# paTRICK-swk/D3DP

Hardware: AMD Instinct MI355X
Metric: pose-hypotheses/sec (H x clips) at F=243, J=17, H=20, K=10 (higher is better)
Workload: dtype f16x2-split operands on fp16 MFMA, f32 accumulate (fp32-class: meets 1e-3 mm)

## Files before the change

d3dp_amd/csrc/capi_train.hip:

```cpp
#include <optional>

#include "ctx.h"

namespace {

#define TP(cls, call) { Scope ps_(pc, cls, st); LAUNCH_TRY(call); }

const float* mask_ptr(const float* masks, const d3dp_cfg& g, int B, int blk, int branch) {
  if (!masks) return nullptr;
  const size_t smax = (size_t)B * std::max(g.frames, g.joints);
  return masks + ((size_t)blk * 2 + branch) * smax;
}

struct Reducer {
  float* base;
  size_t cap, used = 0;
  hipStream_t st;
  std::vector<D3dpReduceItem> items{};
  int rc = 0;
  float* take(size_t n) {
    n = (n + 63) / 64 * 64;
    if (used + n > cap) { rc = -1; return nullptr; }
    float* p = base + used;
    used += n;
    return p;
  }
  void add(const float* part, float* dst, size_t n, size_t count, size_t stride, bool accumulate = false) {
    if (!part || !dst || rc) { rc = rc ? rc : -1; return; }
    items.push_back(D3dpReduceItem{part, dst, (unsigned)n, (unsigned)count, (unsigned)stride, accumulate ? 1u : 0u});
  }
  void flush() {
    for (size_t i = 0; i < items.size() && rc == 0; i += D3DP_REDUCE_MAX) {
      D3dpReduceTable tb{};
      tb.count = (int)std::min<size_t>(D3DP_REDUCE_MAX, items.size() - i);
      for (int j = 0; j < tb.count; ++j) tb.it[j] = items[i + j];
      rc = d3dp_train_reduce_many(tb, st);
    }
    items.clear();
  }
};

int lin32(const float* A, const float* W, const float* bias, float* out, int M, int N, int K, hipStream_t st) {
  return d3dp_launch_linear_f32(EPI_BIAS, A, W, bias, out, M, N, K, st);
}

const float* lin_w(const BlockDev& w, int j) { return (const float*)(j == kQkv ? w.qkv_w : j == kProj ? w.proj_w : j == kFc1 ? w.fc1_w : w.fc2_w); }
const float* lin_b(const BlockDev& w, int j) { return j == kQkv ? w.qkv_b : j == kProj ? w.proj_b : j == kFc1 ? w.fc1_b : w.fc2_b; }

struct X2Train {
  hipStream_t st;
  float* ws;
  const TrainLayout& L;
  const TrainPlan& P;
  d3dp_ctx* pc;
  hipStream_t st_w = nullptr;
  X2Train(d3dp_ctx* c, const TrainLayout& L_, const TrainPlan& P_, float* ws_, hipStream_t st_)
      : st(st_), ws(ws_), L(L_), P(P_), pc(c->prof ? c : nullptr) {
    use_set(0);
  }
  size_t o_a = 0, o_at = 0, o_part = 0, set_base = 0, set_used = 0;
  void use_set(int s) {
    set_base = o_a = s ? L.op_a2 : L.op_a; set_used = 0; n_def = 0;
    o_at = s ? L.op_at2 : L.op_at; o_part = s ? L.part2 : L.part;
  }
  int n_def = 0;
  D3dpTnProduct def[D3DP_TN_MAX];
  float* def_dw[D3DP_TN_MAX];
  int flush_wgrads() {
    if (!n_def) return 0;
    hipStream_t sw = st_w ? st_w : st;
    Scope ps(pc, T_WGRAD, sw);
    int r = d3dp_launch_linear_f16x2_tn_many(def, n_def, P.mTp, P.mZ, sw, P.passes, P.rows_hi);
    if (r) return r;
    D3dpSumTable tb{};
    tb.n = n_def; tb.Z = P.mZ;
    for (int i = 0; i < n_def; ++i) { tb.part[i] = def[i].out; tb.out[i] = def_dw[i]; tb.n4[i] = (size_t)def[i].N * def[i].K / 4; }
    d3dp_launch_sum_partials_many(tb, sw);
    n_def = 0;
    return 0;
  }
  static constexpr int kBwdSlot0 = kTrainBwdSlot0;
  static constexpr int kQkvSlot0 = kTrainQkvSlot0;
  static constexpr int kPmaxSlot0 = kTrainPmaxSlot0;
  int next = 0;
  unsigned* amax() const { return reinterpret_cast<unsigned*>(ws + L.slots); }
  float* uns() const { return ws + L.slots + kTrainSlots; }
  unsigned* qkv_amax(int blk) const { return P.path.attn_x2(blk & 1) ? amax() + kQkvSlot0 + blk : nullptr; }
  int begin(bool forward_pass) {
    next = forward_pass ? 0 : kBwdSlot0;
    return hipMemsetAsync(ws + L.slots + next, 0, (size_t)kBwdSlot0 * 4, st) == hipSuccess ? 0 : -3;
  }
  int take() { return (next < kBwdSlot0 || next >= kTrainSlots) ? -1 : next++; }
  int slot_for(const float* src, size_t n) {
    if (next < kBwdSlot0 || next >= kTrainSlots) return -1;
    d3dp_launch_absmax(src, n, amax() + next, st);
    return next++;
  }
  void rows(const float* src, int R, int C, void* dst, int slot) {
    d3dp_launch_split2_dyn(src, dst, R, C, C, amax() + slot, uns() + slot, st);
  }
  void cols(const float* src, int R, int C, int Rpad, void* dst, int slot) {
    d3dp_launch_split2_t_dyn(src, dst, R, C, Rpad, amax() + slot, uns() + slot, st);
  }
  size_t xoff(int l) const { return (size_t)(l >> 2) * L.x_block + (size_t)(l & 3) * L.C * L.Tp_max; }
  size_t woff(int l) const {
    const size_t CC = L.C * L.C, j = (size_t)(l & 3);
    return (size_t)(l >> 2) * L.w_block + (j == 0 ? 0 : j == 1 ? 3 * CC : j == 2 ? 4 * CC : 4 * CC + L.Hd * L.C);
  }
  float* x_op(int l) const { return ws + L.x_cols + xoff(l); }
  int prepare_weights(const d3dp_ctx* c) {
    if (!P.batched) return 0;
    const int nl = 8 * c->cfg.depth;
    D3dpWPrepTable tb{};
    tb.n = nl;
    for (int l = 0; l < nl; ++l) {
      const int blk = l >> 2, j = l & 3;
      const BlockDev& w = (blk & 1) ? c->tte[blk >> 1] : c->ste[blk >> 1];
      tb.it[l] = D3dpWPrepItem{lin_w(w, j), P.lin[j].N, P.lin[j].K, 2 * l + 1, 0, woff(l)};
    }
    return d3dp_launch_wprep(tb, ws + L.w_rows, ws + L.w_cols, amax(), uns(), st, P.rows_hi);
  }
  int gemm(TrainTail tail, const float* A2, const float* W2, const float* bias, const float* ua, const float* uw, float* out, int N,
           int K, unsigned* out_amax = nullptr, int amax_pos = 0) {
    Scope ps(pc, T_LINEAR, st);
    const int T = P.T, passes = P.passes;
    if (tail.form != TrainTailForm::SPLIT_REM)
      return d3dp_launch_linear_f16x2_dyn(A2, W2, bias, ua, uw, out, T, N, K, 1, st, out_amax, amax_pos,
                                          tail.form == TrainTailForm::REM_BLOCKS ? 1 : 0, passes, P.rows_hi);
    if (P.rows_hi) return -1;
    const int q = T / 256, rem = T - q * 256;
    int r = d3dp_launch_linear_f16x2_dyn(A2, W2, bias, ua, uw, out, q * 256, N, K, 1, st, out_amax, amax_pos, 0, passes);
    if (r) return r;
    r = d3dp_launch_linear_f16x2_dyn(A2 + (size_t)q * 256 * K, W2, nullptr, ua, uw, ws + L.part_rem, rem, N, K, tail.Z, st, nullptr, 0, 0, passes);
    if (r) return r;
    d3dp_launch_sum_partials_bias(ws + L.part_rem, bias, out + (size_t)q * 256 * N, (size_t)rem * N, N, tail.Z, st, out_amax, amax_pos);
    return 0;
  }
  int forward(int blk, TrainLinearId j, const float* A, const BlockDev& w, float ln_eps, float* out) {
    const TrainLinear& p = P.lin[j];
    const int l = 4 * blk + j, sa = 2 * l, sw = 2 * l + 1, T = P.T, N = p.N, K = p.K;
    if (sw >= kBwdSlot0) return -1;
    const float* W = lin_w(w, j);
    const bool pmax = j == kFc1 && P.gelu_operand;
    unsigned* out_amax = j == kQkv ? qkv_amax(blk) : pmax ? amax() + kPmaxSlot0 + blk : nullptr;
    const TrainOperand src = P.source(blk, j);
    const float* a2 = x_op(l);
    if (P.rows_hi && (src == TrainOperand::ROWS_T || !P.batched)) return -1;
    if (src != TrainOperand::PRODUCER) {
      Scope ps(pc, T_OPERAND, st);
      if (j == kProj && (blk & 1) && P.attn_t_f32_mfma) d3dp_launch_absmax(A, (size_t)T * K, amax() + sa, st);
      const int Tp = p.pad_rows;
      int r;
      if (src == TrainOperand::LN_INPUT)
        r = d3dp_launch_rowprep_ln(A, j == kQkv ? w.n1w : w.n2w, j == kQkv ? w.n1b : w.n2b, ln_eps, x_op(l), T, Tp, K, amax() + sa, uns() + sa, st, P.rows_hi);
      else if (src == TrainOperand::ROWS)
        r = d3dp_launch_rowprep(A, x_op(l), nullptr, nullptr, T, Tp, K, amax() + sa, uns() + sa, st, nullptr, 0, 1, 1, nullptr, P.rows_hi);
      else {
        a2 = ws + o_a;
        r = d3dp_launch_dyprep(A, ws + o_a, x_op(l), nullptr, T, K, Tp, amax() + sa, uns() + sa, st);
      }
      if (r) return r;
    }
    const float* w2 = ws + L.op_w;
    if (P.batched) w2 = ws + L.w_rows + woff(l);
    else {
      Scope ps(pc, T_OPERAND, st);
      d3dp_launch_absmax(W, (size_t)N * K, amax() + sw, st);
      rows(W, N, K, ws + L.op_w, sw);
    }
    return gemm(p.fwd_tail, a2, w2, lin_b(w, j), uns() + sa, uns() + sw, out, N, K, out_amax, pmax ? 1 : 0);
  }
  int gelu_operand(int blk, const float* hpre) {
    const int l = 4 * blk + kFc2;
    Scope ps(pc, T_OPERAND, st);
    return d3dp_launch_gelu_rowprep(hpre, x_op(l), P.T, P.lin[kFc2].pad_rows, P.lin[kFc2].K, amax() + kPmaxSlot0 + blk, amax() + 2 * l, uns() + 2 * l, st, P.rows_hi);
  }
  int dgrad(int blk, TrainLinearId j, int sdy, const float* W, float* dX, unsigned* out_amax = nullptr) {
    const TrainLinear& p = P.lin[j];
    const int l = 4 * blk + j, sw = 2 * l + 1;
    {
      Scope ps(pc, T_OPERAND, st);
      if (!P.batched) cols(W, p.N, p.K, p.N, ws + L.op_w, sw);
    }
    const float* wt = ws + L.op_w;
    if (P.batched) wt = ws + L.w_cols + woff(l);
    return gemm(p.dgrad_tail, ws + o_a, wt, nullptr, uns() + sdy, uns() + sw, dX, p.K, p.N, out_amax);
  }
  int prep_dy(TrainLinearId j, const float* dY, int sdy, float* bias_part, int* bias_rows, const float* mask = nullptr, int axis = 0,
              int F = 1, int J = 1, const float* gelu_pre = nullptr) {
    const TrainLinear& p = P.lin[j];
    if (P.merged) {
      if (set_used + L.Tp_max * (size_t)p.N > L.dy_set_floats) return -1;
      o_a = set_base + set_used;
      set_used += L.Tp_max * (size_t)p.N;
    }
    Scope ps(pc, T_OPERAND, st);
    if (p.tn)
      return d3dp_launch_rowprep(dY, ws + o_a, bias_part, bias_rows, P.T, p.pad_rows, p.N, amax() + sdy, uns() + sdy, st, mask, axis, F, J,
                                 gelu_pre, P.rows_hi);
    if (P.rows_hi) return -1;
    *bias_rows = D3DP_DYPREP_ROWS;
    return d3dp_launch_dyprep(dY, ws + o_a, ws + o_at, bias_part, P.T, p.N, p.pad_rows, amax() + sdy, uns() + sdy, st);
  }
  int wgrad(int blk, TrainLinearId j, int sdy, float* dW) {
    const TrainLinear& p = P.lin[j];
    const int l = 4 * blk + j, sx = 2 * l, N = p.N, K = p.K;
    if (P.merged) {
      if (n_def >= D3DP_TN_MAX) return -1;
      size_t po = 0;
      for (int i = 0; i < n_def; ++i) po += (size_t)P.mZ * def[i].N * def[i].K;
      def[n_def] = D3dpTnProduct{ws + o_a, x_op(l), uns() + sdy, uns() + sx, ws + o_part + po, N, K, 0, 0};
      def_dw[n_def++] = dW;
      return 0;
    }
    int r;
    hipStream_t sw = st_w ? st_w : st;
    Scope ps(pc, T_WGRAD, sw);
    if (p.tn)
      r = d3dp_launch_linear_f16x2_tn(ws + o_a, x_op(l), uns() + sdy, uns() + sx, ws + o_part, N, K, p.Tp, p.Z, sw, P.passes, P.rows_hi);
    else
      r = d3dp_launch_linear_f16x2_dyn(ws + o_at, x_op(l), nullptr, uns() + sdy, uns() + sx, ws + o_part, N, K, p.Tp, p.Z, sw, nullptr, 0, 0, P.passes);
    if (r) return r;
    d3dp_launch_sum_partials(ws + o_part, dW, (size_t)N * K, p.Z, sw);
    return 0;
  }
};

}

extern "C" {

int d3dp_train_workspace_bytes(const d3dp_ctx* c, int32_t B, size_t* bytes) {
  if (!c || !bytes || B < 1) return d3dp_fail(D3DP_EINVAL, "d3dp_train_workspace_bytes: bad argument");
  *bytes = train_layout(c->cfg, B).total_floats * 4;
  return D3DP_OK;
}

int d3dp_train_forward(d3dp_ctx* c, const float* x2d, const float* x3d, const int64_t* t, const float* masks, float* out,
                       int32_t B, void* workspace, size_t workspace_bytes, void* stream) {
  if (!c || !x2d || !x3d || !t || !out || !workspace || B < 1) return d3dp_fail(D3DP_EINVAL, "d3dp_train_forward: bad argument");
  if (!c->train()) return d3dp_fail(D3DP_ESTATE, "d3dp_train_forward needs a D3DP_MODE_TRAIN context");
  if (!c->weights_set) return d3dp_fail(D3DP_ESTATE, "weights not set");
  const d3dp_cfg& g = c->cfg;
  const TrainLayout L = train_layout(g, B);
  const TrainPlan P = plan_train_step(*c, g, B, c->n_cu);
  if (g.frames > 256 && !(P.path.attn_x2(0) && P.path.attn_x2(1)) && !P.attn_bwd_chunked)
    return d3dp_fail(D3DP_ENOTSUP, "frames=%d > 256: the training step runs such clips on its split-fp16 attention kernels only, which take "
                              "head dims 64, 32 and 16 -- 24, 40, 48 and 56 under D3DP_TRAIN_IMPL=f16x2 -- (channels=%d heads=%d is head dim %d) and are switched off by the cross-check "
                              "switches D3DP_TRAIN_IMPL=f32 and D3DP_TRAIN_ATTN=f32|x2t; the fp32 attention holds a whole sequence "
                              "in LDS (<= 256 frames)", g.frames, g.channels, g.heads, g.channels / g.heads);
  if (workspace_bytes < L.total_floats * 4) return d3dp_fail(D3DP_ESTATE, "train workspace too small");
  if (P.use_x2 && !P.rows_fit) return d3dp_fail(D3DP_EINVAL, "d3dp_train_forward: an operand's padded rows exceed the workspace's");
  hipStream_t st = (hipStream_t)stream;
  float* ws = (float*)workspace;
  const int T = P.T, C = g.channels, F = g.frames, J = g.joints, Hd = g.hidden;
  float *xn = ws + L.xn, *y = ws + L.y, *hid = ws + L.hid;
  d3dp_ctx* const pc = c->prof ? c : nullptr;
  std::optional<X2Train> x2s;
  if (P.use_x2) x2s.emplace(c, L, P, ws, st);
  X2Train* const x2 = P.use_x2 ? &*x2s : nullptr;
  if (x2) {
    Scope ps_(pc, T_OTHER, st);
    LAUNCH_TRY(x2->begin(true));
    LAUNCH_TRY(x2->prepare_weights(c));
  }
  auto lin = [&](int blk, TrainLinearId j, const float* src, float* out) -> int {
    const BlockDev& w = (blk & 1) ? c->tte[blk >> 1] : c->ste[blk >> 1];
    if (x2) return x2->forward(blk, j, src, w, g.eps_block, out);
    Scope ps_(pc, T_LINEAR, st);
    return lin32(src, lin_w(w, j), lin_b(w, j), out, T, P.lin[j].N, P.lin[j].K, st);
  };
  const bool ln_fused = P.ln_fused, ln_direct = P.ln_direct;
  TP(T_OTHER, d3dp_train_time_mlp(t, c->freq, c->t1w, c->t1b, c->t3w, c->t3b, ws + L.dtemb, ws + L.temb, B, C, st));
  float* slab0 = ws + L.saved0;
  TP(T_LN_FWD, d3dp_launch_embed_ln(0, x2d, x3d, ws + L.temb, c->ew, c->eb, c->spos, c->ste[0].n1w, c->ste[0].n1b,
                                    g.eps_block, slab0 + L.o_xin, xn, 0, B, 1, F, J, C, st));
  auto slot = [&](int l) -> unsigned* { return x2 ? x2->amax() + 2 * l : nullptr; };
  if (x2) { Scope ps_(pc, T_OTHER, st); d3dp_launch_absmax(xn, (size_t)T * C, slot(0), st); }
  for (int blk = 0; blk < 2 * g.depth; ++blk) {
    const int kind = blk & 1, d = blk >> 1;
    const BlockDev& w = kind ? c->tte[d] : c->ste[d];
    float* S = ws + L.saved0 + (size_t)blk * L.saved_stride;
    const bool ax2 = P.path.attn_x2(kind);
    LAUNCH_TRY(lin(blk, kQkv, ln_fused ? S + L.o_xin : xn, S + L.o_qkv));
    const bool att_direct = P.att_direct(kind);
    void* att_op = att_direct ? x2->x_op(4 * blk + 1) : nullptr;
    const int att_tp = att_direct ? P.lin[kProj].pad_rows : 0;
    float* att_un = att_direct ? x2->uns() + 2 * (4 * blk + 1) : nullptr;
    const int n_seq = kind ? B * J : B * F;
    const SeqMap map = kind ? temporal_map(F, J) : spatial_map(F, J);
    auto attention = [&]() -> int {
      if (ax2)
        return d3dp_train_attn_x2_fwd(S + L.o_qkv, S + L.o_att, ws + L.stats_x2 + (size_t)blk * L.stats_x2_stride, n_seq, map, C,
                                      g.heads, x2->qkv_amax(blk), slot(4 * blk + 1), st, att_op, T, att_tp, att_un, P.attn_passes, P.rows_hi);
      if (kind == 1 && P.attn_t_f32_mfma)
        return d3dp_launch_attn_temporal_f32(0, S + L.o_qkv, S + L.o_att, n_seq, map, C, g.heads, st);
      return d3dp_launch_attn_rows(0, S + L.o_qkv, S + L.o_att, n_seq, map, C, g.heads, st, slot(4 * blk + 1));
    };
    TP(kind ? T_ATTN_FWD_T : T_ATTN_FWD_S, attention());
    LAUNCH_TRY(lin(blk, kProj, S + L.o_att, y));
    if (ln_direct)
      TP(T_LN_FWD, d3dp_train_add_mask_ln(S + L.o_xin, y, mask_ptr(masks, g, B, blk, 0), kind, F, J, w.n2w, w.n2b, g.eps_block,
                                          S + L.o_xmid, nullptr, slot(4 * blk + 2), T, C, st, x2->x_op(4 * blk + 2),
                                          P.lin[kFc1].pad_rows, x2->uns() + 2 * (4 * blk + 2), P.rows_hi))
    else
      TP(T_LN_FWD, d3dp_train_add_mask_ln(S + L.o_xin, y, mask_ptr(masks, g, B, blk, 0), kind, F, J, w.n2w, w.n2b, g.eps_block,
                                          S + L.o_xmid, ln_fused ? nullptr : xn, slot(4 * blk + 2), T, C, st));
    LAUNCH_TRY(lin(blk, kFc1, ln_fused ? S + L.o_xmid : xn, S + L.o_hpre));
    if (P.gelu_operand) {
      LAUNCH_TRY(x2->gelu_operand(blk, S + L.o_hpre));
      LAUNCH_TRY(lin(blk, kFc2, nullptr, y));
    } else {
      TP(T_OPERAND, d3dp_train_gelu_fwd(S + L.o_hpre, hid, (size_t)T * Hd, slot(4 * blk + 3), st));
      LAUNCH_TRY(lin(blk, kFc2, hid, y));
    }
    const bool last = blk == 2 * g.depth - 1;
    float* x_next = last ? ws + L.x_final : S + L.saved_stride + L.o_xin;
    const float *nw = c->hnw, *nb = c->hnb;
    if (!last) { const BlockDev& wn = kind ? c->ste[d + 1] : c->tte[d]; nw = wn.n1w; nb = wn.n1b; }
    TP(T_LN_FWD, d3dp_train_add_mask_ln2(S + L.o_xmid, y, mask_ptr(masks, g, B, blk, 1), kind, F, J, kind ? c->tnw : c->snw,
                                         kind ? c->tnb : c->snb, g.eps_block, (kind == 0 && d == 0) ? c->tpos : nullptr, nw, nb,
                                         last ? g.eps_head : g.eps_block, S + L.o_xout, x_next,
                                         last ? ws + L.z : (ln_fused ? nullptr : xn), last ? nullptr : slot(4 * (blk + 1)), T, C, st,
                                         (ln_direct && !last) ? x2->x_op(4 * (blk + 1)) : nullptr,
                                         (ln_direct && !last) ? P.lin[kQkv].pad_rows : 0,
                                         (ln_direct && !last) ? x2->uns() + 2 * 4 * (blk + 1) : nullptr, P.rows_hi));
  }
  TP(T_OTHER, d3dp_train_head_linear(ws + L.z, c->hw, c->hb, out, T, C, st));
  HIP_TRY(hipGetLastError());
  return D3DP_OK;
}

int d3dp_train_backward(d3dp_ctx* c, const float* x2d, const float* x3d, const int64_t* t, const float* masks,
                        const float* grad_out, const d3dp_weights* grads, int32_t B, void* workspace,
                        size_t workspace_bytes, void* stream) {
  if (!c || !x2d || !x3d || !t || !grad_out || !grads || !grads->ste || !grads->tte || !workspace || B < 1)
    return d3dp_fail(D3DP_EINVAL, "d3dp_train_backward: bad argument");
  if (!c->train()) return d3dp_fail(D3DP_ESTATE, "d3dp_train_backward needs a D3DP_MODE_TRAIN context");
  const d3dp_cfg& g = c->cfg;
  const TrainLayout L = train_layout(g, B);
  const TrainPlan P = plan_train_step(*c, g, B, c->n_cu);
  if (workspace_bytes < L.total_floats * 4) return d3dp_fail(D3DP_ESTATE, "train workspace too small");
  if (P.use_x2 && !(P.rows_fit && P.parts_fit))
    return d3dp_fail(D3DP_EINVAL, "d3dp_train_backward: an operand's padded rows or a weight gradient's partial products exceed the workspace's");
  hipStream_t st = (hipStream_t)stream;
  float* ws = (float*)workspace;
  const int T = P.T, Tp = (int)L.Tpad, C = g.channels, F = g.frames, J = g.joints, Hd = g.hidden;
  auto G = [](const float* p) { return const_cast<float*>(p); };
  D3dpZeroTable ztab{};
  auto zero = [&](const float* p, size_t n) -> hipError_t {
    if (ztab.count < D3DP_ZERO_MAX && n < ((size_t)1 << 32)) {
      ztab.p[ztab.count] = G(p); ztab.n[ztab.count] = (unsigned)n; ++ztab.count;
      return hipSuccess;
    }
    return hipMemsetAsync(G(p), 0, n * 4, st);
  };
  const size_t CC = (size_t)C * C;
  HIP_TRY(zero(grads->time1_w, 2 * CC)); HIP_TRY(zero(grads->time1_b, 2 * C));
  HIP_TRY(zero(grads->time3_w, 2 * CC)); HIP_TRY(zero(grads->time3_b, C));
  d3dp_ctx* const pc = c->prof ? c : nullptr;
  if (ztab.count) TP(T_OTHER, d3dp_train_zero_many(ztab, st));
  float *xn = ws + L.xn, *hid = ws + L.hid, *dA = ws + L.dA, *dB = ws + L.dB, *dC = ws + L.dC, *dqkv = ws + L.dqkv,
        *dh = ws + L.dh, *At = ws + L.At, *Xt = ws + L.Xt, *Wt = ws + L.Wt;

  std::optional<X2Train> x2s;
  if (P.use_x2) x2s.emplace(c, L, P, ws, st);
  X2Train* const x2 = P.use_x2 ? &*x2s : nullptr;
  if (x2) TP(T_OTHER, x2->begin(false));
  const bool overlap = P.path.needs_aux && !c->prof;
  if (overlap && !c->aux) return d3dp_fail(D3DP_ESTATE, "d3dp_train_backward: the second stream was not created (d3dp_create makes it)");
  bool pending[2] = {false, false};
  int n_wgrad = 0, cur_set = 0;
  const int n_sets = P.overlap_sets;
  auto wait_set = [&](int s) -> int {
    if (!pending[s]) return 0;
    pending[s] = false;
    return hipStreamWaitEvent(st, c->ev_done[s], 0) == hipSuccess ? 0 : -3;
  };
  auto join = [&]() -> int { int r = wait_set(0); return r ? r : wait_set(1); };
  Reducer red{ws + L.red, L.red_floats, 0, st};
  red.items.reserve(24 * (size_t)g.depth + 32);
  const int lnrows = L.ln_rows;
  auto ln_part = [&](const float* dgamma, const float* dbeta, int calls) -> float* {
    float* p = red.take((size_t)calls * lnrows * 2 * C);
    if (p) {
      red.add(p, G(dgamma), C, (size_t)calls * lnrows, 2 * (size_t)C);
      red.add(p + C, G(dbeta), C, (size_t)calls * lnrows, 2 * (size_t)C);
    }
    return p;
  };
  float* part_sn = ln_part(grads->spatial_norm_w, grads->spatial_norm_b, g.depth);
  float* part_tn = ln_part(grads->temporal_norm_w, grads->temporal_norm_b, g.depth);
  float* part_hn = ln_part(grads->head_norm_w, grads->head_norm_b, 1);
  if (red.rc) return d3dp_fail(D3DP_ESTATE, "d3dp_train_backward: partial-sum region too small");
  int sdy = -1;
  auto wgrad = [&](int blk, TrainLinearId j, const float* dY, const float* X, float* dW, float* dbias, int pre_slot = -1,
                   const float* mk = nullptr, int mk_axis = 0, const float* gelu_pre = nullptr) -> int {
    const int N = P.lin[j].N, K = P.lin[j].K;
    int r;
    if (x2) {
      sdy = pre_slot >= 0 ? pre_slot : x2->slot_for(dY, (size_t)T * N);
      if (sdy < 0) return -1;
      float* bp = red.take((size_t)L.bias_rows * N);
      int brows = 0;
      if (!bp) return -1;
      const bool first = !P.merged || j == kFc2, last = !P.merged || j == kQkv;
      if (first) {
        cur_set = overlap ? (n_wgrad++ % n_sets) : 0;
        if ((r = wait_set(cur_set))) return r;
        x2->use_set(cur_set);
      }
      if ((r = x2->prep_dy(j, dY, sdy, bp, &brows, mk, mk_axis, F, J, gelu_pre))) return r;
      red.add(bp, dbias, N, brows, N);
      if (last && overlap) {
        if (hipEventRecord(c->ev_fork, st) != hipSuccess || hipStreamWaitEvent(c->aux, c->ev_fork, 0) != hipSuccess) return -3;
        x2->st_w = c->aux;
      }
      if ((r = x2->wgrad(blk, j, sdy, dW))) return r;
      if (last && P.merged && (r = x2->flush_wgrads())) return r;
      if (last && overlap) {
        if (hipEventRecord(c->ev_done[cur_set], c->aux) != hipSuccess) return -3;
        pending[cur_set] = true;
      }
      return 0;
    }
    float* bp = red.take((size_t)D3DP_DYPREP_ROWS * N);
    int rows = 0;
    if (!bp || mk || gelu_pre) return -1;
    {
      Scope ps_(pc, T_OPERAND, st);
      if ((r = d3dp_train_colsum(dY, bp, &rows, D3DP_DYPREP_ROWS, T, N, st))) return r;
      red.add(bp, dbias, N, rows, N);
      if ((r = d3dp_train_transpose_pad(dY, At, T, N, Tp, st))) return r;
      if ((r = d3dp_train_transpose_pad(X, Xt, T, K, Tp, st))) return r;
    }
    Scope ps_(pc, T_WGRAD, st);
    return d3dp_launch_linear_f32_splitk(At, Xt, dW, N, K, Tp, st, ws + L.part, L.part_floats);
  };
  auto dgrad = [&](int blk, TrainLinearId j, const float* dY, float* dX, unsigned* out_amax = nullptr) -> int {
    const BlockDev& w = (blk & 1) ? c->tte[blk >> 1] : c->ste[blk >> 1];
    const int N = P.lin[j].N, K = P.lin[j].K;
    if (x2) return sdy < 0 ? -1 : x2->dgrad(blk, j, sdy, lin_w(w, j), dX, out_amax);
    int r;
    { Scope ps_(pc, T_OPERAND, st); if ((r = d3dp_train_transpose_pad(lin_w(w, j), Wt, N, K, N, st))) return r; }
    Scope ps_(pc, T_LINEAR, st);
    return lin32(dY, Wt, nullptr, dX, T, K, N, st);
  };
  auto fresh = [&](int& slot) -> unsigned* {
    slot = x2 ? x2->take() : -1;
    return slot >= 0 ? x2->amax() + slot : nullptr;
  };
#define D3DP_FRESH(ps, pa)                                                                              \
  int ps = -1;                                                                                          \
  unsigned* pa = fresh(ps);                                                                             \
  if (x2 && ps < 0) return d3dp_fail(D3DP_ESTATE, "d3dp_train_backward: out of operand slots");

  const int nblk = 2 * g.depth;
  {
    float* hp = red.take((size_t)L.head_rows * (3 * C + 4));
    int rows = 0;
    if (!hp) return d3dp_fail(D3DP_ESTATE, "d3dp_train_backward: partial-sum region too small");
    TP(T_OTHER, d3dp_train_head_bwd(grad_out, ws + L.z, c->hw, dC, hp, &rows, T, C, st));
    red.add(hp, G(grads->head_w), 3 * (size_t)C, rows, 3 * (size_t)C + 4);
    red.add(hp + 3 * C, G(grads->head_b), 3, rows, 3 * (size_t)C + 4);
  }
  const float* dy = nullptr;
  const float* dy_mask = nullptr;
  int ps_next = -1;
  const bool mip2 = P.mip2, mip1 = P.mip1, gip = P.gip;
  {
    const int lb = nblk - 1, lk = lb & 1;
    const float* S = ws + L.saved0 + (size_t)lb * L.saved_stride;
    const float* mk = mask_ptr(masks, g, B, lb, 1);
    D3DP_FRESH(ps, pa)
    TP(T_LN_BWD, d3dp_train_ln_bwd(dC, ws + L.x_final, c->hnw, g.eps_head, nullptr, nullptr, S + L.o_xout, lk ? c->tnw : c->snw,
                                 g.eps_block, dB, mk, lk, F, J, (mk && !mip2) ? dC : nullptr, pa, part_hn,
                                 (lk ? part_tn : part_sn) + (size_t)(lb >> 1) * lnrows * 2 * C, T, C, st));
    dy = (mk && !mip2) ? dC : dB;
    dy_mask = mip2 ? mk : nullptr;
    ps_next = ps;
  }
  for (int blk = nblk - 1; blk >= 0; --blk) {
    const int kind = blk & 1, d = blk >> 1;
    const BlockDev& w = kind ? c->tte[d] : c->ste[d];
    const d3dp_block_weights& gw = (kind ? grads->tte : grads->ste)[d];
    float* S = ws + L.saved0 + (size_t)blk * L.saved_stride;
    if (!x2) TP(T_OPERAND, d3dp_train_gelu_fwd(S + L.o_hpre, hid, (size_t)T * Hd, nullptr, st));
    LAUNCH_TRY(wgrad(blk, kFc2, dy, hid, G(gw.fc2_w), G(gw.fc2_b), ps_next, dy_mask, kind));
    {
      D3DP_FRESH(ps, pa)
      LAUNCH_TRY(dgrad(blk, kFc2, dy, dh, gip ? pa : nullptr));
      if (!gip) TP(T_OPERAND, d3dp_train_gelu_bwd(dh, S + L.o_hpre, dh, (size_t)T * Hd, pa, st));
      if (!x2) TP(T_LN_FWD, d3dp_train_ln_pos(S + L.o_xmid, w.n2w, w.n2b, g.eps_block, nullptr, F, J, xn, T, C, st));
      LAUNCH_TRY(wgrad(blk, kFc1, dh, xn, G(gw.fc1_w), G(gw.fc1_b), ps, nullptr, 0, gip ? S + L.o_hpre : nullptr));
      LAUNCH_TRY(dgrad(blk, kFc1, dh, dC));
    }
    {
      const float* mk = mask_ptr(masks, g, B, blk, 0);
      float* pn = ln_part(gw.norm2_w, gw.norm2_b, 1);
      D3DP_FRESH(ps, pa)
      if (!pn) return d3dp_fail(D3DP_ESTATE, "d3dp_train_backward: partial-sum region too small");
      TP(T_LN_BWD, d3dp_train_ln_bwd(dC, S + L.o_xmid, w.n2w, g.eps_block, dB, nullptr, nullptr, nullptr, 0.f, dA, mk, kind, F, J,
                                   (mk && !mip1) ? dC : nullptr, pa, pn, nullptr, T, C, st));
      dy = (mk && !mip1) ? dC : dA;
      LAUNCH_TRY(wgrad(blk, kProj, dy, S + L.o_att, G(gw.proj_w), G(gw.proj_b), ps, mip1 ? mk : nullptr, kind));
    }
    int ps_dqkv = -1;
    if (P.path.attn_x2(kind)) {
      D3DP_FRESH(pdo, pado)
      D3DP_FRESH(pq, paq)
      LAUNCH_TRY(dgrad(blk, kProj, dy, dB, pado));
      for (int part = pc ? 1 : 0; part <= (pc ? 2 : 0); ++part)
        TP(part == 2 ? (kind ? T_ATTN_BKV_T : T_ATTN_BKV_S) : (kind ? T_ATTN_BQ_T : T_ATTN_BQ_S),
           d3dp_train_attn_x2_bwd(S + L.o_qkv, S + L.o_att, dB, dqkv, ws + L.stats_x2 + (size_t)blk * L.stats_x2_stride,
                                  kind ? B * J : B * F, kind ? temporal_map(F, J) : spatial_map(F, J), C, g.heads,
                                  x2->qkv_amax(blk), pado, paq, st, part, P.attn_passes));
      ps_dqkv = pq;
    } else {
      LAUNCH_TRY(dgrad(blk, kProj, dy, dB));
      TP(kind ? T_ATTN_BQ_T : T_ATTN_BQ_S, d3dp_train_attn_bwd(S + L.o_qkv, S + L.o_att, dB, dqkv, ws + L.stats, kind ? B * J : B * F,
                                                             kind ? temporal_map(F, J) : spatial_map(F, J), C, g.heads, st,
                                                             P.attn_bwd_chunked));
    }
    if (!x2) TP(T_LN_FWD, d3dp_train_ln_pos(S + L.o_xin, w.n1w, w.n1b, g.eps_block, nullptr, F, J, xn, T, C, st));
    LAUNCH_TRY(wgrad(blk, kQkv, dqkv, xn, G(gw.qkv_w), G(gw.qkv_b), ps_dqkv));
    LAUNCH_TRY(dgrad(blk, kQkv, dqkv, dC));
    float* pn1 = ln_part(gw.norm1_w, gw.norm1_b, 1);
    if (!pn1) return d3dp_fail(D3DP_ESTATE, "d3dp_train_backward: partial-sum region too small");
    if (blk > 0) {
      const int pb = blk - 1, pk = pb & 1;
      const float* Sp = ws + L.saved0 + (size_t)pb * L.saved_stride;
      const float* mk = mask_ptr(masks, g, B, pb, 1);
      float* g_out = pb == 0 ? ws + L.y : nullptr;
      D3DP_FRESH(ps, pa)
      TP(T_LN_BWD, d3dp_train_ln_bwd(dC, S + L.o_xin, w.n1w, g.eps_block, dA, g_out, Sp + L.o_xout, pk ? c->tnw : c->snw, g.eps_block,
                                   dB, mk, pk, F, J, (mk && !mip2) ? dC : nullptr, pa, pn1,
                                   (pk ? part_tn : part_sn) + (size_t)(pb >> 1) * lnrows * 2 * C, T, C, st));
      if (g_out) TP(T_OTHER, d3dp_train_groupsum(g_out, G(grads->temporal_pos), T, C, 1, F, J, 1, st));
      dy = (mk && !mip2) ? dC : dB;
      dy_mask = mip2 ? mk : nullptr;
      ps_next = ps;
    } else {
      TP(T_LN_BWD, d3dp_train_ln_bwd(dC, S + L.o_xin, w.n1w, g.eps_block, dA, nullptr, nullptr, nullptr, 0.f, dB, nullptr, 0, F, J,
                                   nullptr, nullptr, pn1, nullptr, T, C, st));
    }
  }
#undef D3DP_FRESH
  LAUNCH_TRY(join());
  {
    Scope ps_(pc, T_OTHER, st);
    float* ep = red.take((size_t)D3DP_EMBED_BWD_ROWS * 5 * C);
    float* bp = red.take((size_t)L.embed_bias_rows * C);
    float* sp = red.take((size_t)L.group_slices * J * C);
    float* tp = red.take((size_t)L.group_slices * B * C);
    int rows = 0;
    if (!ep || !bp || !sp || !tp) return d3dp_fail(D3DP_ESTATE, "d3dp_train_backward: partial-sum region too small");
    LAUNCH_TRY(d3dp_train_embed_bwd(dB, x2d, x3d, ep, T, C, st));
    red.add(ep, G(grads->embed_w), 5 * (size_t)C, D3DP_EMBED_BWD_ROWS, 5 * (size_t)C);
    LAUNCH_TRY(d3dp_train_colsum(dB, bp, &rows, L.embed_bias_rows, T, C, st));
    red.add(bp, G(grads->embed_b), C, rows, C);
    LAUNCH_TRY(d3dp_train_groupsum(dB, sp, T, C, 0, F, J, L.group_slices, st));
    red.add(sp, G(grads->spatial_pos), (size_t)J * C, L.group_slices, (size_t)J * C);
    LAUNCH_TRY(d3dp_train_groupsum(dB, tp, T, C, 2, F, J, L.group_slices, st));
    red.add(tp, ws + L.dtemb, (size_t)B * C, L.group_slices, (size_t)B * C);
    red.flush();
  }
  if (red.rc) return d3dp_fail(D3DP_EHIP, "d3dp_train_backward: the gradient reduction failed");
  TP(T_OTHER, d3dp_train_time_mlp_bwd(t, c->freq, c->t1w, c->t1b, c->t3w, ws + L.dtemb, G(grads->time1_w),
                                      G(grads->time1_b), G(grads->time3_w), G(grads->time3_b), B, C, st));
  for (int i = 0; pc && i < 8; ++i) { Scope ps_(pc, P_EMPTY, st); }
  HIP_TRY(hipGetLastError());
  return D3DP_OK;
}

}
#undef TP
```

d3dp_amd/csrc/ctx_plan.h:

```cpp
#pragma once
#include <algorithm>
#include <cstdlib>
#include <cstring>

#include "../../include/d3dp_hip.h"

int d3dp_fail(int code, const char* fmt, ...) __attribute__((format(printf, 2, 3)));

struct CtxEnv {
  const char *exact_impl = nullptr, *long_attn = nullptr, *no_fold = nullptr, *defer_norm = nullptr, *train_impl = nullptr,
             *train_overlap = nullptr, *train_gelu = nullptr, *train_wgrad = nullptr, *train_ln_operand = nullptr, *train_tail = nullptr,
             *train_attn = nullptr, *train_passes = nullptr, *fast_impl = nullptr, *fast16_range = nullptr, *x2_skew = nullptr,
             *x2_pp = nullptr, *x2_wide = nullptr, *seq_pad = nullptr, *fold_ln = nullptr, *train_long_attn = nullptr,
             *train_attn_passes = nullptr, *train_rows = nullptr;
  static CtxEnv from_process() {
    CtxEnv e;
    e.exact_impl = getenv("D3DP_EXACT_IMPL");
    e.long_attn = getenv("D3DP_LONG_ATTN");
    e.no_fold = getenv("D3DP_NO_FOLD");
    e.defer_norm = getenv("D3DP_DEFER_NORM");
    e.train_impl = getenv("D3DP_TRAIN_IMPL");
    e.train_overlap = getenv("D3DP_TRAIN_OVERLAP");
    e.train_gelu = getenv("D3DP_TRAIN_GELU");
    e.train_wgrad = getenv("D3DP_TRAIN_WGRAD");
    e.train_ln_operand = getenv("D3DP_TRAIN_LN_OPERAND");
    e.train_tail = getenv("D3DP_TRAIN_TAIL");
    e.train_attn = getenv("D3DP_TRAIN_ATTN");
    e.train_passes = getenv("D3DP_TRAIN_PASSES");
    e.fast_impl = getenv("D3DP_FAST_IMPL");
    e.fast16_range = getenv("D3DP_FAST16_RANGE");
    e.x2_skew = getenv("D3DP_X2_SKEW");
    e.x2_pp = getenv("D3DP_X2_PP");
    e.x2_wide = getenv("D3DP_X2_WIDE");
    e.seq_pad = getenv("D3DP_SEQ_PAD");
    e.fold_ln = getenv("D3DP_FOLD_LN");
    e.train_long_attn = getenv("D3DP_TRAIN_LONG_ATTN");
    e.train_attn_passes = getenv("D3DP_TRAIN_ATTN_PASSES");
    e.train_rows = getenv("D3DP_TRAIN_ROWS");
    return e;
  }
};

struct CtxPlan {
  int hdp = 0;
  bool fast16_scale = false;
  int train_passes = 3;
  int train_attn_passes = 3;
  bool train_rows_hi = false;
  int exact_impl_req = 0;
  bool long_rows = false;
  bool fold = true;
  bool defer = true;
  bool train_x2 = true;
  bool train_overlap = true;
  int train_overlap_sets = 2;
  bool train_gelu_in_prep = true;
  bool train_wgrad_merged = true;
  bool train_ln_direct = true;
  bool train_tail_blocks = true;
  int train_attn_x2 = 2;
  bool train_long_attn = false;
  int skew_d = 0;
  int pingpong = 0;
  int pad_override = -1;
  bool fold_ln_on = false;
};

inline bool env_is(const char* v, const char* s) { return v && !strcmp(v, s); }
inline int env_digit(const char* v, const char* allowed, int dflt) {
  return v && v[0] && !v[1] && strchr(allowed, v[0]) ? v[0] - '0' : dflt;
}
inline bool mfma_head_dim(int hd) { return hd == 64 || hd == 32 || hd == 16; }

inline bool instantiated_width(const d3dp_cfg& g) {
  const int hd = g.channels / g.heads;
  return (g.channels == 64 || g.channels == 128 || g.channels == 256 || g.channels == 512) &&
         (hd == 8 || hd == 16 || hd == 32 || hd == 64) && g.hidden >= 64 && g.hidden % 64 == 0;
}
inline bool optin_width(int c) { return c == 192 || c == 320 || c == 384 || c == 448; }
inline int padded_head_dim(int hd) { return hd <= 32 ? 32 : 64; }
inline bool x2_optin_shape(const d3dp_cfg& g) {
  const int hd = g.channels / g.heads;
  return optin_width(g.channels) && hd % 8 == 0 && hd <= 64 && g.hidden >= 64 && g.hidden % 64 == 0;
}
inline bool fast_optin_shape(const d3dp_cfg& g) {
  const int hd = g.channels / g.heads;
  return optin_width(g.channels) && (hd == 24 || hd == 32 || hd == 40 || hd == 48 || hd == 56 || hd == 64) && g.hidden == 2 * g.channels;
}
constexpr int D3DP_TN_TILE_N = 256, D3DP_TN_TILE_K = 128;
constexpr int D3DP_WPREP_MAX = 64;
inline bool d3dp_tn_applies(int N, int K) { return N % D3DP_TN_TILE_N == 0 && K % D3DP_TN_TILE_K == 0; }
inline bool train_linears_split(const CtxPlan& p, const d3dp_cfg& g) { return p.train_x2 && g.channels % 32 == 0 && g.hidden % 32 == 0; }

inline int plan_context(const d3dp_cfg& g, const CtxEnv& e, bool variants_built, CtxPlan* out) {
  if (g.frames < 1 || g.frames > 1024) return d3dp_fail(D3DP_ENOTSUP, "frames=%d not in [1,1024]", g.frames);
  if (g.joints < 1 || g.joints > 256) return d3dp_fail(D3DP_ENOTSUP, "joints=%d not in [1,256]", g.joints);
  if (g.heads < 1 || g.channels < 1 || g.channels % g.heads) return d3dp_fail(D3DP_EINVAL, "heads=%d does not divide channels=%d", g.heads, g.channels);
  if (g.depth < 1) return d3dp_fail(D3DP_EINVAL, "depth=%d", g.depth);
  if (g.mode != D3DP_MODE_EXACT && g.mode != D3DP_MODE_FAST && g.mode != D3DP_MODE_TRAIN && g.mode != D3DP_MODE_FAST16)
    return d3dp_fail(D3DP_EINVAL, "mode=%d", g.mode);
  const int hd = g.channels / g.heads;
  const bool inst = instantiated_width(g), train = g.mode == D3DP_MODE_TRAIN, fast16 = g.mode == D3DP_MODE_FAST16;
  CtxPlan p;
  p.long_rows = env_is(e.long_attn, "rows");
  if (env_is(e.exact_impl, "f16x2") && !inst) {
    if (!x2_optin_shape(g) || g.mode != D3DP_MODE_EXACT)
      return d3dp_fail(D3DP_ENOTSUP, "D3DP_EXACT_IMPL=f16x2 outside the instantiated widths exists for D3DP_MODE_EXACT contexts with channels in "
                                "{192,320,384,448}, head dim a multiple of 8 up to 64 and hidden a multiple of 64; channels=%d heads=%d "
                                "hidden=%d mode=%d is not one (unset the switch: such a context runs the fp32 implementation)",
                  g.channels, g.heads, g.hidden, g.mode);
    if (p.long_rows)
      return d3dp_fail(D3DP_ENOTSUP, "D3DP_LONG_ATTN=rows with D3DP_EXACT_IMPL=f16x2 at channels=%d: the run-time-head-dim row attention has no "
                                "split-fp16 output form", g.channels);
    p.hdp = padded_head_dim(hd);
  }
  const bool train_widths = train && !inst && env_is(e.train_impl, "f16x2");
  if (train_widths && !x2_optin_shape(g))
    return d3dp_fail(D3DP_ENOTSUP, "D3DP_TRAIN_IMPL=f16x2 outside the instantiated widths exists for D3DP_MODE_TRAIN contexts with channels in "
                              "{192,320,384,448}, head dim a multiple of 8 up to 64 and hidden a multiple of 64; channels=%d heads=%d "
                              "hidden=%d is not one (unset the switch: such a context trains on the fp32 path)",
                g.channels, g.heads, g.hidden);
  if ((g.mode == D3DP_MODE_FAST || fast16) && e.fast_impl) {
    if (strcmp(e.fast_impl, "mfma"))
      return d3dp_fail(D3DP_ENOTSUP, "D3DP_FAST_IMPL=%.32s: the one value a FAST / FAST16 context takes is D3DP_FAST_IMPL=mfma (channels=%d)",
                  e.fast_impl, g.channels);
    if (!inst) {
      if (!fast_optin_shape(g))
        return d3dp_fail(D3DP_ENOTSUP, "D3DP_FAST_IMPL=mfma outside the instantiated widths exists for FAST / FAST16 contexts with channels in "
                                  "{192,320,384,448}, head dim in {24,32,40,48,56,64} and hidden = 2 x channels; channels=%d heads=%d "
                                  "hidden=%d is not one (such a width runs in D3DP_MODE_EXACT / D3DP_MODE_TRAIN)",
                    g.channels, g.heads, g.hidden);
      if (p.long_rows)
        return d3dp_fail(D3DP_ENOTSUP, "D3DP_LONG_ATTN=rows with D3DP_FAST_IMPL=mfma at channels=%d: the row attention kernel would take the padded "
                                  "head dim for its exponent", g.channels);
      p.hdp = padded_head_dim(hd);
    }
  }
  if (fast16 && e.fast16_range) {
    if (strcmp(e.fast16_range, "scale"))
      return d3dp_fail(D3DP_ENOTSUP, "D3DP_FAST16_RANGE=%.32s: the one value a FAST16 context takes is D3DP_FAST16_RANGE=scale", e.fast16_range);
    if (p.hdp)
      return d3dp_fail(D3DP_ENOTSUP, "D3DP_FAST16_RANGE=scale with D3DP_FAST_IMPL=mfma at channels=%d: the padded-head kernels have no scaled "
                                "form", g.channels);
    if (inst && !mfma_head_dim(hd))
      return d3dp_fail(D3DP_ENOTSUP, "D3DP_FAST16_RANGE=scale at head dim %d (channels=%d heads=%d): the scaled attention kernels exist at head "
                                "dims 64, 32 and 16", hd, g.channels, g.heads);
    if (inst && p.long_rows)
      return d3dp_fail(D3DP_ENOTSUP, "D3DP_FAST16_RANGE=scale with D3DP_LONG_ATTN=rows: the row attention kernel has no scaled form");
    const int k = g.hidden;
    if (inst && !(k == 64 || k == 128 || k == 256 || k == 512 || k == 1024))
      return d3dp_fail(D3DP_ENOTSUP, "D3DP_FAST16_RANGE=scale with hidden=%d: the scaled streaming Linear exists at k-depths 64, 128, 256, 512 "
                                "and 1024", g.hidden);
    p.fast16_scale = inst;
  }
  if (train && e.train_long_attn) {
    if (strcmp(e.train_long_attn, "chunked"))
      return d3dp_fail(D3DP_ENOTSUP, "D3DP_TRAIN_LONG_ATTN=%.32s: the one value a TRAIN context takes is D3DP_TRAIN_LONG_ATTN=chunked (the fp32 "
                                "attention backward passes its rows through LDS in chunks and takes any sequence length)", e.train_long_attn);
    p.train_long_attn = true;
  }
  const bool width_inst = inst || p.hdp != 0;
  if (!width_inst) {
    if (g.mode == D3DP_MODE_FAST)
      return d3dp_fail(D3DP_ENOTSUP, "channels=%d heads=%d hidden=%d: FAST contexts exist for channels in {64,128,256,512} with head dim in "
                                "{8,16,32,64} and hidden a multiple of 64; other widths run in D3DP_MODE_EXACT / D3DP_MODE_TRAIN (fp32 implementation)",
                  g.channels, g.heads, g.hidden);
    if (fast16)
      return d3dp_fail(D3DP_ENOTSUP, "channels=%d heads=%d hidden=%d: FAST16 contexts exist for the shapes FAST contexts exist for -- channels in "
                                "{64,128,256,512} with head dim in {8,16,32,64} and hidden a multiple of 64; other widths run in D3DP_MODE_EXACT / "
                                "D3DP_MODE_TRAIN (fp32 implementation)",
                  g.channels, g.heads, g.hidden);
    if (g.channels > 1024 || g.channels % 4 || hd % 4 || hd > 128 || g.hidden < 4 || g.hidden % 4)
      return d3dp_fail(D3DP_ENOTSUP, "channels=%d heads=%d hidden=%d: the fp32 implementation takes channels <= 1024, head dim a multiple of 4 up to 128 "
                                "and hidden a multiple of 4", g.channels, g.heads, g.hidden);
    const int nmax = std::max(g.frames, g.joints), cap = hd <= 16 ? 16 : hd <= 32 ? 32 : hd <= 64 ? 64 : 128;
    if (train && !train_widths && !p.train_long_attn && (nmax > 256 || (size_t)nmax * (8 * (cap + 4) + 12) > 160 * 1024))
      return d3dp_fail(D3DP_ENOTSUP, "channels=%d heads=%d frames=%d joints=%d: training at a width outside {64,128,256,512} runs the fp32 attention "
                                "backward, which holds a whole sequence in LDS (<= 256 tokens; <= 153 at head dims above 64)",
                  g.channels, g.heads, g.frames, g.joints);
  }
  const bool train_f32 = env_is(e.train_impl, "f32");
  p.fold = !(e.no_fold && e.no_fold[0] == '1');
  p.defer = !(e.defer_norm && e.defer_norm[0] == '0');
  p.train_x2 = !train_f32 && (width_inst || train_widths);
  p.train_overlap = !(e.train_overlap && e.train_overlap[0] == '0');
  p.train_overlap_sets = (e.train_overlap && e.train_overlap[0] == '1') ? 1 : 2;
  p.train_gelu_in_prep = !env_is(e.train_gelu, "pass");
  p.train_wgrad_merged = !env_is(e.train_wgrad, "each");
  p.train_ln_direct = !env_is(e.train_ln_operand, "pass");
  p.train_tail_blocks = !env_is(e.train_tail, "split");
  p.train_attn_x2 = env_is(e.train_attn, "f32") ? 0 : env_is(e.train_attn, "x2t") ? 1 : 2;
  const bool superseded = !p.train_gelu_in_prep || !p.train_wgrad_merged || !p.train_tail_blocks || !p.train_ln_direct;
  if (train && e.train_passes) {
    if (strcmp(e.train_passes, "1") && strcmp(e.train_passes, "3"))
      return d3dp_fail(D3DP_ENOTSUP, "D3DP_TRAIN_PASSES=%.32s: the values a TRAIN context takes are D3DP_TRAIN_PASSES=1 (one fp16-MFMA pass per "
                                "product of the split-fp16 training Linears) and 3 (the default)", e.train_passes);
    if (e.train_passes[0] == '1') {
      if (!train_linears_split(p, g))
        return d3dp_fail(D3DP_ENOTSUP, "D3DP_TRAIN_PASSES=1 exists for the split-fp16 training Linears; channels=%d%s trains on the fp32 path "
                                  "(fp32-MFMA Linears have no one-pass form)", g.channels, train_f32 ? " under D3DP_TRAIN_IMPL=f32" : "");
      if (superseded)
        return d3dp_fail(D3DP_ENOTSUP, "D3DP_TRAIN_PASSES=1 beside D3DP_TRAIN_WGRAD=each / D3DP_TRAIN_TAIL=split / D3DP_TRAIN_GELU=pass / "
                                  "D3DP_TRAIN_LN_OPERAND=pass: the superseded launch forms have no one-pass form");
      p.train_passes = 1;
    }
  }
  if (train && e.train_attn_passes) {
    if (strcmp(e.train_attn_passes, "1") && strcmp(e.train_attn_passes, "3"))
      return d3dp_fail(D3DP_ENOTSUP, "D3DP_TRAIN_ATTN_PASSES=%.32s: the values a TRAIN context takes are D3DP_TRAIN_ATTN_PASSES=1 (one fp16-MFMA "
                                "pass per product of the split-fp16 training attention) and 3 (the default)", e.train_attn_passes);
    if (e.train_attn_passes[0] == '1') {
      if (!train_linears_split(p, g))
        return d3dp_fail(D3DP_ENOTSUP, "D3DP_TRAIN_ATTN_PASSES=1 exists for the split-fp16 training attention; channels=%d%s trains on the fp32 "
                                  "path (its attention runs the fp32 kernels, which have no one-pass form)", g.channels,
                    train_f32 ? " under D3DP_TRAIN_IMPL=f32" : "");
      if (hd == 24 || hd == 40 || hd == 48 || hd == 56)
        return d3dp_fail(D3DP_ENOTSUP, "D3DP_TRAIN_ATTN_PASSES=1 at head dim %d (channels=%d heads=%d): the padded forms of the split-fp16 "
                                  "training attention have no one-pass form", hd, g.channels, g.heads);
      if (!mfma_head_dim(hd))
        return d3dp_fail(D3DP_ENOTSUP, "D3DP_TRAIN_ATTN_PASSES=1 at head dim %d (channels=%d heads=%d): the one-pass training attention exists at "
                                  "head dims 64, 32 and 16 (this head dim runs the fp32 attention kernels)", hd, g.channels, g.heads);
      if (p.train_attn_x2 == 0)
        return d3dp_fail(D3DP_ENOTSUP, "D3DP_TRAIN_ATTN_PASSES=1 beside D3DP_TRAIN_ATTN=f32: both axes then run the fp32 attention kernels, which "
                                  "have no one-pass form");
      p.train_attn_passes = 1;
    }
  }
  if (train && e.train_rows) {
    if (strcmp(e.train_rows, "hi") && strcmp(e.train_rows, "split"))
      return d3dp_fail(D3DP_ENOTSUP, "D3DP_TRAIN_ROWS=%.32s: the values a TRAIN context takes are D3DP_TRAIN_ROWS=hi (the one-pass training "
                                "Linears' operands as plain fp16 rows) and split (the default)", e.train_rows);
    if (e.train_rows[0] == 'h') {
      if (!train_linears_split(p, g))
        return d3dp_fail(D3DP_ENOTSUP, "D3DP_TRAIN_ROWS=hi exists for the split-fp16 training Linears; channels=%d%s trains on the fp32 path "
                                  "(fp32-MFMA Linears read no operand rows)", g.channels, train_f32 ? " under D3DP_TRAIN_IMPL=f32" : "");
      if (!inst)
        return d3dp_fail(D3DP_ENOTSUP, "D3DP_TRAIN_ROWS=hi at channels=%d under D3DP_TRAIN_IMPL=f16x2: the padded widths run an operand pass in "
                                  "front of every Linear and transposed weight-gradient operands, which have no hi-only form", g.channels);
      if (superseded)
        return d3dp_fail(D3DP_ENOTSUP, "D3DP_TRAIN_ROWS=hi beside D3DP_TRAIN_WGRAD=each / D3DP_TRAIN_TAIL=split / D3DP_TRAIN_GELU=pass / "
                                  "D3DP_TRAIN_LN_OPERAND=pass: the superseded launch forms have no hi-only form");
      if (p.train_passes != 1)
        return d3dp_fail(D3DP_ENOTSUP, "D3DP_TRAIN_ROWS=hi without D3DP_TRAIN_PASSES=1: the three-pass products read the lo halves that hi-only "
                                  "rows do not store");
      const int C = g.channels, Hd = g.hidden;
      if (C % 256 != 0 || !d3dp_tn_applies(3 * C, C) || !d3dp_tn_applies(C, C) || !d3dp_tn_applies(Hd, C) || !d3dp_tn_applies(C, Hd))
        return d3dp_fail(D3DP_ENOTSUP, "D3DP_TRAIN_ROWS=hi at channels=%d hidden=%d: the hi-only route exists where no operand of the step is "
                                  "transposed and the LayerNorm kernels write the qkv / fc1 operand rows -- channels a multiple of 256 "
                                  "and hidden a multiple of 256 (`-cs` 256 and 512); narrower widths use transposed operands", C, Hd);
      if (hd == 16 && p.train_attn_x2 != 0)
        return d3dp_fail(D3DP_ENOTSUP, "D3DP_TRAIN_ROWS=hi at head dim 16 (channels=%d heads=%d): the split-fp16 training attention writes "
                                  "hi-only proj operand rows at head dims 64 and 32", g.channels, g.heads);
      if (8 * g.depth > D3DP_WPREP_MAX)
        return d3dp_fail(D3DP_ENOTSUP, "D3DP_TRAIN_ROWS=hi at depth=%d: the hi-only weight operands are written by the batched weight preparation "
                                  "(depth <= %d); the per-weight preparation of deeper models has no hi-only form", g.depth, D3DP_WPREP_MAX / 8);
      p.train_rows_hi = true;
    }
  }
  p.exact_impl_req = env_is(e.exact_impl, "bf16x3") ? 1 : env_is(e.exact_impl, "f32") ? 2 : 0;
  if (!width_inst) {
    if (p.exact_impl_req == 1)
      return d3dp_fail(D3DP_ENOTSUP, "D3DP_EXACT_IMPL=bf16x3 exists for channels in {64,128,256,512}; channels=%d runs the fp32 implementation", g.channels);
    p.exact_impl_req = 2;
  }
  if (superseded && !variants_built)
    return d3dp_fail(D3DP_ENOTSUP, "D3DP_TRAIN_WGRAD=each / D3DP_TRAIN_TAIL=split / D3DP_TRAIN_GELU=pass / D3DP_TRAIN_LN_OPERAND=pass select superseded launch forms of the "
                              "training step that only the variants build honours (make -C d3dp_amd/csrc variants; "
                              "D3DP_LIB=d3dp_amd/lib/variants/libd3dp_variants.so)");
  p.skew_d = env_digit(e.x2_skew, "0124", 0);
  p.pingpong = env_is(e.x2_wide, "1") ? 2 : env_digit(e.x2_pp, "01", 0);
  p.pad_override = env_digit(e.seq_pad, "01", -1);
  p.fold_ln_on = e.fold_ln && e.fold_ln[0] == '1';
  if ((p.skew_d || p.pingpong || p.pad_override > 0 || p.fold_ln_on) && !variants_built)
    return d3dp_fail(D3DP_ENOTSUP, "D3DP_X2_SKEW / D3DP_X2_PP / D3DP_X2_WIDE / D3DP_SEQ_PAD / D3DP_FOLD_LN select experiment kernels that this "
                              "library was built without (make -C d3dp_amd/csrc variants; D3DP_LIB=d3dp_amd/lib/variants/libd3dp_variants.so)");
  *out = p;
  return D3DP_OK;
}
```

d3dp_amd/csrc/gemm_x2_train.hip:

```cpp
#include <cstdlib>
#include <cstring>

#include "common.h"
#include "gemm_x2_tile.h"
#include "kernels.h"

namespace {

template <int PASSES, bool HI = false>
__global__ __launch_bounds__(768) void gemm_f16x2_dyn_kernel(const f16* __restrict__ A2, const f16* __restrict__ W2,
                                                             const float* __restrict__ bias, const float* __restrict__ dynA,
                                                             const float* __restrict__ dynW, float* __restrict__ out, int M,
                                                             int N, int Kfull, int NKz, int tiles_n, int tiles_per_z,
                                                             int total_items, unsigned* __restrict__ amax_out, int amax_pos,
                                                             int rem_m0) {
  static_assert(PASSES == 1 || PASSES == 3, "one pass (hi x hi) or the three-pass split scheme");
  static_assert(!HI || PASSES == 1, "hi-only rows hold no lo halves");
  constexpr int RS = HI ? 1 : 2;
  extern __shared__ __attribute__((aligned(16))) char smem[];
  const int G = gridDim.x;
  const int L = xcd_remap(blockIdx.x, G);
  const int n_my = (total_items - L + G - 1) / G;
  const int NS = HI ? NKz >> 1 : NKz;
  const int gtot = n_my * NS;
  const int tid = threadIdx.x, lane = tid & 63;
  const int wave = __builtin_amdgcn_readfirstlane(tid >> 6);
  if (gtot <= 0) return;
  const int rem_cg = (N + 63) >> 6;
  const int rem_blocks = rem_m0 > 0 ? ((M - rem_m0 + 15) >> 4) * rem_cg : 0;

  if (wave >= XNCW) {
    const int lw = wave - XNCW;
    const int lr = lane >> 3, lq = lane & 7;
    int ti = 0, ks = 0, slot = 0;
    const f16* pa[8];
    const f16* pw[4];
    auto issue = [&]() {
      if (ks == 0) {
        const int item = L + ti * G;
        const int z = item / tiles_per_z, t = item - z * tiles_per_z;
        const int m0 = (t / tiles_n) * XBM, n0 = (t % tiles_n) * XBN;
        const size_t k0 = (size_t)z * NS * (2 * XBK);
#pragma unroll
        for (int i = 0; i < 8; ++i) {
          const int row = (lw * 8 + i) * 8 + lr;
          pa[i] = A2 + (size_t)min(m0 + row, M - 1) * (RS * Kfull) + k0 + swz128(row, lq) * 8;
        }
#pragma unroll
        for (int i = 0; i < 4; ++i) {
          const int row = (lw * 4 + i) * 8 + lr;
          const int wrow = (row & 64) + colperm(row & 63);
          pw[i] = W2 + (size_t)min(n0 + wrow, N - 1) * (RS * Kfull) + k0 + swz128(row, lq) * 8;
        }
      }
      char* base = smem + slot * XSTAGE;
      const int ko = ks * (2 * XBK);
#pragma unroll
      for (int i = 0; i < 8; ++i) __builtin_amdgcn_global_load_lds(GPTR(pa[i] + ko), LPTR(base + (lw * 8 + i) * 1024), 16, 0, 0);
#pragma unroll
      for (int i = 0; i < 4; ++i)
        __builtin_amdgcn_global_load_lds(GPTR(pw[i] + ko), LPTR(base + XA_BYTES + (lw * 4 + i) * 1024), 16, 0, 0);
      if (++ks == NS) { ks = 0; ++ti; }
      slot = (slot == XNSTAGE - 1) ? 0 : slot + 1;
    };
    issue();
    if (gtot > 1) issue();
    for (int b = L; b < rem_blocks; b += G) { X2_BARRIER(); X2_BARRIER(); }
    for (int g = 0; g < gtot; ++g) {
      if (g + 1 < gtot) asm volatile("s_waitcnt vmcnt(12)" ::: "memory");
      else asm volatile("s_waitcnt vmcnt(0)" ::: "memory");
      X2_BARRIER();
      if (g + 2 < gtot) issue();
    }
    if (amax_out) X2_BARRIER();
    return;
  }

  const int wr = wave >> 1, wc = wave & 1;
  const int fi = lane & 15, fg = lane >> 4;
  const int offA = (wr * 64 + fi) * 128 + swz128(fi, fg) * 16, offAl = offA ^ 64;
  const int offW = XA_BYTES + (wc * 64 + fi) * 128 + swz128(fi, fg) * 16, offWl = offW ^ 64;
  const float unscale = dynA[0] * dynW[0];
  __builtin_amdgcn_s_setprio(1);
  float am = 0.f;
  int slot = 0;
  if (rem_blocks > 0) {
    const int ksw = NKz / XNCW;
    f32x4* xch = reinterpret_cast<f32x4*>(smem + (XNSTAGE - 1) * XSTAGE);
#pragma unroll 1
    for (int b = L; b < rem_blocks; b += G) {
      const int m0 = rem_m0 + (b / rem_cg) * 16, nb0 = (b % rem_cg) * 64;
      const size_t kofs = (size_t)wave * ksw * (RS * XBK) + fg * 8;
      const f16* ap = A2 + (size_t)min(m0 + fi, M - 1) * (RS * Kfull) + kofs;
      const f16* wp[4];
#pragma unroll
      for (int ni = 0; ni < 4; ++ni) wp[ni] = W2 + (size_t)min(nb0 + 4 * fi + ni, N - 1) * (RS * Kfull) + kofs;
      f32x4 pacc[4];
#pragma unroll
      for (int ni = 0; ni < 4; ++ni) pacc[ni] = (f32x4){0.f, 0.f, 0.f, 0.f};
#pragma unroll 1
      for (int ks = 0; ks < ksw; ks += 2) {
        f16x8 ah[2], al[2], wh[2][4], wl[2][4];
#pragma unroll
        for (int u = 0; u < 2; ++u) {
          const int o = (ks + u) * (RS * XBK);
          ah[u] = *reinterpret_cast<const f16x8*>(ap + o);
          if constexpr (PASSES == 3) al[u] = *reinterpret_cast<const f16x8*>(ap + o + XBK);
#pragma unroll
          for (int ni = 0; ni < 4; ++ni) {
            wh[u][ni] = *reinterpret_cast<const f16x8*>(wp[ni] + o);
            if constexpr (PASSES == 3) wl[u][ni] = *reinterpret_cast<const f16x8*>(wp[ni] + o + XBK);
          }
        }
#pragma unroll
        for (int u = 0; u < 2; ++u) {
          if constexpr (PASSES == 3) {
#pragma unroll
            for (int ni = 0; ni < 4; ++ni) pacc[ni] = __builtin_amdgcn_mfma_f32_16x16x32_f16(ah[u], wl[u][ni], pacc[ni], 0, 0, 0);
#pragma unroll
            for (int ni = 0; ni < 4; ++ni) pacc[ni] = __builtin_amdgcn_mfma_f32_16x16x32_f16(al[u], wh[u][ni], pacc[ni], 0, 0, 0);
          }
#pragma unroll
          for (int ni = 0; ni < 4; ++ni) pacc[ni] = __builtin_amdgcn_mfma_f32_16x16x32_f16(ah[u], wh[u][ni], pacc[ni], 0, 0, 0);
        }
      }
      X2_BARRIER();
#pragma unroll
      for (int ni = 0; ni < 4; ++ni) xch[(wave * 4 + ni) * 64 + lane] = pacc[ni];
      asm volatile("s_waitcnt lgkmcnt(0)" ::: "memory");
      X2_BARRIER();
      if (wave == 0) {
        f32x4 sum[4];
#pragma unroll
        for (int ni = 0; ni < 4; ++ni) {
          sum[ni] = xch[ni * 64 + lane];
#pragma unroll
          for (int w = 1; w < XNCW; ++w) sum[ni] += xch[(w * 4 + ni) * 64 + lane];
        }
        const int nb = nb0 + 4 * fi;
        if (nb < N) {
          float4 bz = {0.f, 0.f, 0.f, 0.f};
          if (bias != nullptr) bz = *reinterpret_cast<const float4*>(bias + nb);
#pragma unroll
          for (int r = 0; r < 4; ++r) {
            const int m = m0 + 4 * fg + r;
            if (m < M) {
              const f32x4 v = {fmaf(sum[0][r], unscale, bz.x), fmaf(sum[1][r], unscale, bz.y), fmaf(sum[2][r], unscale, bz.z),
                               fmaf(sum[3][r], unscale, bz.w)};
              *reinterpret_cast<f32x4*>(out + (size_t)m * N + nb) = v;
              am = amax_pos ? fmaxf(am, fmaxf(fmaxf(v[0], v[1]), fmaxf(v[2], v[3])))
                            : fmaxf(am, fmaxf(fmaxf(fabsf(v[0]), fabsf(v[1])), fmaxf(fabsf(v[2]), fabsf(v[3]))));
            }
          }
        }
      }
    }
  }
#pragma unroll 1
  for (int ti = 0; ti < n_my; ++ti) {
    f32x4 acc[4][4];
#pragma unroll
    for (int i = 0; i < 4; ++i)
#pragma unroll
      for (int j = 0; j < 4; ++j) acc[i][j] = (f32x4){0.f, 0.f, 0.f, 0.f};
#pragma unroll 1
    for (int ks = 0; ks < NS; ++ks) {
      asm volatile("s_waitcnt lgkmcnt(0)" ::: "memory");
      X2_BARRIER();
      const char* sb = smem + slot * XSTAGE;
      slot = (slot == XNSTAGE - 1) ? 0 : slot + 1;
      f16x8 wf[4][2];
#pragma unroll
      for (int ni = 0; ni < 4; ++ni)
#pragma unroll
        for (int pl = 0; pl < (PASSES == 3 || HI ? 2 : 1); ++pl)
          wf[ni][pl] = *reinterpret_cast<const f16x8*>(sb + (pl ? offWl : offW) + ni * 2048);
#pragma unroll
      for (int mi = 0; mi < 4; ++mi) {
        const f16x8 ah = *reinterpret_cast<const f16x8*>(sb + offA + mi * 2048);
        if constexpr (HI) {
          const f16x8 a2 = *reinterpret_cast<const f16x8*>(sb + offAl + mi * 2048);
#pragma unroll
          for (int ni = 0; ni < 4; ++ni) acc[mi][ni] = __builtin_amdgcn_mfma_f32_16x16x32_f16(ah, wf[ni][0], acc[mi][ni], 0, 0, 0);
#pragma unroll
          for (int ni = 0; ni < 4; ++ni) acc[mi][ni] = __builtin_amdgcn_mfma_f32_16x16x32_f16(a2, wf[ni][1], acc[mi][ni], 0, 0, 0);
          continue;
        }
        if constexpr (PASSES == 3) {
          const f16x8 al = *reinterpret_cast<const f16x8*>(sb + offAl + mi * 2048);
#pragma unroll
          for (int ni = 0; ni < 4; ++ni) acc[mi][ni] = __builtin_amdgcn_mfma_f32_16x16x32_f16(ah, wf[ni][1], acc[mi][ni], 0, 0, 0);
#pragma unroll
          for (int ni = 0; ni < 4; ++ni) acc[mi][ni] = __builtin_amdgcn_mfma_f32_16x16x32_f16(al, wf[ni][0], acc[mi][ni], 0, 0, 0);
        }
#pragma unroll
        for (int ni = 0; ni < 4; ++ni) acc[mi][ni] = __builtin_amdgcn_mfma_f32_16x16x32_f16(ah, wf[ni][0], acc[mi][ni], 0, 0, 0);
      }
    }
    const int item = L + ti * G;
    const int z = item / tiles_per_z, t = item - z * tiles_per_z;
    const int pm0 = (t / tiles_n) * XBM + wr * 64 + 4 * fg, nb = (t % tiles_n) * XBN + wc * 64 + 4 * fi;
    if (nb < N) {
      float4 bz = {0.f, 0.f, 0.f, 0.f};
      if (bias != nullptr) bz = *reinterpret_cast<const float4*>(bias + nb);
      float* o = out + (size_t)z * M * N + nb;
#pragma unroll
      for (int mi = 0; mi < 4; ++mi)
#pragma unroll
        for (int r = 0; r < 4; ++r) {
          const int m = pm0 + mi * 16 + r;
          if (m < M) {
            const f32x4 v = {fmaf(acc[mi][0][r], unscale, bz.x), fmaf(acc[mi][1][r], unscale, bz.y),
                             fmaf(acc[mi][2][r], unscale, bz.z), fmaf(acc[mi][3][r], unscale, bz.w)};
            *reinterpret_cast<f32x4*>(o + (size_t)m * N) = v;
            am = amax_pos ? fmaxf(am, fmaxf(fmaxf(v[0], v[1]), fmaxf(v[2], v[3])))
                          : fmaxf(am, fmaxf(fmaxf(fabsf(v[0]), fabsf(v[1])), fmaxf(fabsf(v[2]), fabsf(v[3]))));
          }
        }
    }
  }
  if (amax_out) {
    float* part = reinterpret_cast<float*>(smem + XNSTAGE * XSTAGE);
    am = wave_max(am);
    if (lane == 0) part[wave] = am;
    asm volatile("s_waitcnt lgkmcnt(0)" ::: "memory");
    X2_BARRIER();
    if (wave == 0 && lane == 0) {
      float m = part[0];
#pragma unroll
      for (int w = 1; w < XNCW; ++w) m = fmaxf(m, part[w]);
      atomicMax(amax_out, __float_as_uint(m));
    }
  }
}

__device__ __forceinline__ int tn_find(const D3dpTnTable& tb, int t) {
  int i = 0;
#pragma unroll
  for (int j = 1; j < D3DP_TN_MAX; ++j)
    if (j < tb.n && t >= tb.p[j].tile0) i = j;
  return i;
}
constexpr int XTN_HI_A = 32 * 512, XTN_HI_STAGE = XTN_HI_A + 32 * 256;
template <int PASSES, bool HI = false>
__global__ __launch_bounds__(768) void gemm_f16x2_tn_kernel(D3dpTnTable tb, int NKz, int tiles_per_z, int total_items) {
  static_assert(PASSES == 1 || PASSES == 3, "one pass (hi x hi) or the three-pass split scheme");
  static_assert(!HI || PASSES == 1, "hi-only rows hold no lo halves");
  constexpr int STAGE = HI ? XTN_HI_STAGE : XSTAGE, A_BYTES = HI ? XTN_HI_A : XA_BYTES, A_ROW = HI ? 512 : 1024, W_ROW = HI ? 256 : 512;
  extern __shared__ __attribute__((aligned(16))) char smem[];
  const int G = gridDim.x;
  const int L = xcd_remap(blockIdx.x, G);
  const int n_my = (total_items - L + G - 1) / G;
  const int gtot = n_my * NKz;
  const int tid = threadIdx.x, lane = tid & 63;
  const int wave = __builtin_amdgcn_readfirstlane(tid >> 6);
  if (gtot <= 0) return;

  if (wave >= XNCW) {
    const int lw = wave - XNCW;
    int ti = 0, ks = 0, slot = 0;
    const f16* pa;
    const f16* pw;
    size_t a_row = 0, w_row = 0;
    auto issue = [&]() {
      if (ks == 0) {
        const int item = L + ti * G;
        const int z = item / tiles_per_z, tt = item - z * tiles_per_z;
        const D3dpTnProduct& P = tb.p[tn_find(tb, tt)];
        const int t = tt - P.tile0;
        const int n0 = (t / P.tiles_k) * XBM, k0 = (t % P.tiles_k) * XBN;
        const size_t t0 = (size_t)z * NKz * XBK;
        a_row = (size_t)(HI ? 1 : 2) * P.N; w_row = (size_t)(HI ? 1 : 2) * P.K;
        pa = (const f16*)P.A2 + (t0 + lw * 8) * a_row + (size_t)n0 * (HI ? 1 : 2);
        pw = (const f16*)P.W2 + (t0 + lw * 8) * w_row + (size_t)k0 * (HI ? 1 : 2);
      }
      char* base = smem + slot * STAGE;
      const size_t ro = (size_t)ks * XBK;
      if constexpr (HI) {
#pragma unroll
        for (int i = 0; i < 4; ++i) {
          const int rr = 2 * i + (lane >> 5);
          __builtin_amdgcn_global_load_lds(GPTR(pa + (ro + rr) * a_row + (((lane & 31) ^ (rr << 1)) << 3)),
                                           LPTR(base + (lw * 8 + 2 * i) * 512), 16, 0, 0);
        }
#pragma unroll
        for (int i = 0; i < 2; ++i) {
          const int rr = 4 * i + (lane >> 4);
          __builtin_amdgcn_global_load_lds(GPTR(pw + (ro + rr) * w_row + (((lane & 15) ^ (rr << 1)) << 3)),
                                           LPTR(base + A_BYTES + (lw * 8 + 4 * i) * 256), 16, 0, 0);
        }
      } else {
#pragma unroll
      for (int i = 0; i < 8; ++i) {
        const int r = lw * 8 + i;
        __builtin_amdgcn_global_load_lds(GPTR(pa + (ro + i) * a_row + ((lane ^ (i << 1)) << 3)), LPTR(base + r * 1024), 16, 0, 0);
      }
#pragma unroll
      for (int i = 0; i < 4; ++i) {
        const int r = lw * 8 + 2 * i + (lane >> 5);
        const int l32 = lane & 31;
        __builtin_amdgcn_global_load_lds(GPTR(pw + (ro + 2 * i + (lane >> 5)) * w_row + ((l32 ^ ((r & 7) << 1)) << 3)),
                                         LPTR(base + XA_BYTES + (lw * 8 + 2 * i) * 512), 16, 0, 0);
      }
      }
      if (++ks == NKz) { ks = 0; ++ti; }
      slot = (slot == XNSTAGE - 1) ? 0 : slot + 1;
    };
    issue();
    if (gtot > 1) issue();
    for (int g = 0; g < gtot; ++g) {
      if (g + 1 < gtot) { if constexpr (HI) asm volatile("s_waitcnt vmcnt(6)" ::: "memory"); else asm volatile("s_waitcnt vmcnt(12)" ::: "memory"); }
      else asm volatile("s_waitcnt vmcnt(0)" ::: "memory");
      X2_BARRIER();
      if (g + 2 < gtot) issue();
    }
    return;
  }

  const int wr = wave >> 1, wc = wave & 1;
  const int fi = lane & 15, fg = lane >> 4;
  const int j = fi >> 2, qd = fi & 3, row = 4 * fg + j;
  auto a_off = [&](int mi, int pl) {
    if constexpr (HI) return row * 512 + (((((wr * 2 + (mi >> 1)) << 2) | ((mi & 1) << 1) | (qd >> 1)) ^ ((row & 7) << 1)) << 4) + ((qd & 1) << 3);
    else return row * 1024 + (((((wr * 2 + (mi >> 1)) << 3) | (pl << 2) | ((mi & 1) << 1) | (qd >> 1)) ^ ((row & 7) << 1)) << 4) + ((qd & 1) << 3);
  };
  auto w_off = [&](int ni, int pl) {
    if constexpr (HI) return A_BYTES + row * 256 + (((((wc * 2 + (ni >> 1)) << 2) | ((ni & 1) << 1) | (qd >> 1)) ^ ((row & 7) << 1)) << 4) + ((qd & 1) << 3);
    else return XA_BYTES + row * 512 + (((((wc * 2 + (ni >> 1)) << 3) | (pl << 2) | ((ni & 1) << 1) | (qd >> 1)) ^ ((row & 7) << 1)) << 4) + ((qd & 1) << 3);
  };
  typedef __bf16 v4bf __attribute__((ext_vector_type(4)));
  typedef __bf16 v8bf __attribute__((ext_vector_type(8)));
  auto tr8 = [&](const char* p, int second) {
    const v4bf a = __builtin_amdgcn_ds_read_tr16_b64_v4bf16((__attribute__((address_space(3))) v4bf*)(p));
    const v4bf b = __builtin_amdgcn_ds_read_tr16_b64_v4bf16((__attribute__((address_space(3))) v4bf*)(p + second));
    return __builtin_bit_cast(f16x8, (v8bf){a[0], a[1], a[2], a[3], b[0], b[1], b[2], b[3]});
  };
  int offA[4][2], offW[4][2];
#pragma unroll
  for (int m = 0; m < 4; ++m)
#pragma unroll
    for (int pl = 0; pl < 2; ++pl) { offA[m][pl] = a_off(m, pl); offW[m][pl] = w_off(m, pl); }
  __builtin_amdgcn_s_setprio(1);
  int slot = 0;
#pragma unroll 1
  for (int ti = 0; ti < n_my; ++ti) {
    f32x4 acc[4][4];
#pragma unroll
    for (int i = 0; i < 4; ++i)
#pragma unroll
      for (int jj = 0; jj < 4; ++jj) acc[i][jj] = (f32x4){0.f, 0.f, 0.f, 0.f};
#pragma unroll 1
    for (int ks = 0; ks < NKz; ++ks) {
      asm volatile("s_waitcnt lgkmcnt(0)" ::: "memory");
      X2_BARRIER();
      const char* sb = smem + slot * STAGE;
      slot = (slot == XNSTAGE - 1) ? 0 : slot + 1;
      f16x8 wf[4][2];
#pragma unroll
      for (int ni = 0; ni < 4; ++ni)
#pragma unroll
        for (int pl = 0; pl < (PASSES == 3 ? 2 : 1); ++pl) wf[ni][pl] = tr8(sb + offW[ni][pl], 16 * W_ROW);
#pragma unroll
      for (int mi = 0; mi < 4; ++mi) {
        const f16x8 ah = tr8(sb + offA[mi][0], 16 * A_ROW);
        if constexpr (PASSES == 3) {
          const f16x8 al = tr8(sb + offA[mi][1], 16 * A_ROW);
#pragma unroll
// ... 325 lines not shown
      const size_t i = i0 + u * stride;
      if (i < n) {
        const size_t r = i / G8;
        const int c = (int)(i - r * G8) * 8;
        const float v[8] = {a[u].x, a[u].y, a[u].z, a[u].w, b[u].x, b[u].y, b[u].z, b[u].w};
        f16x8 hi, lo;
#pragma unroll
        for (int e = 0; e < 8; ++e) {
          const float g = r < (size_t)R ? gelu_erf_rational(v[e]) : 0.f;
          f16 h, l;
          split2h_scaled(g * sc, h, l);
          hi[e] = h; lo[e] = l;
        }
        f16* row = HI ? drow + r * (size_t)C + c : drow + r * 2 * (size_t)C + h2i_col(c);
        *reinterpret_cast<f16x8*>(row) = hi;
        if constexpr (!HI) *reinterpret_cast<f16x8*>(row + kH2iLo) = lo;
      }
    }
  }
}

__global__ __launch_bounds__(256) void wprep_absmax_kernel(D3dpWPrepTable tb, unsigned* __restrict__ amax) {
  __shared__ float part[4];
  const D3dpWPrepItem it = tb.it[blockIdx.y];
  const size_t n4 = (size_t)it.N * it.K / 4, stride = (size_t)gridDim.x * blockDim.x;
  const float4* s4 = reinterpret_cast<const float4*>(it.w);
  float m = 0.f;
  for (size_t i = (size_t)blockIdx.x * blockDim.x + threadIdx.x; i < n4; i += stride) {
    const float4 v = s4[i];
    m = fmaxf(m, fmaxf(fmaxf(fabsf(v.x), fabsf(v.y)), fmaxf(fabsf(v.z), fabsf(v.w))));
  }
  m = wave_max(m);
  if ((threadIdx.x & 63) == 0) part[threadIdx.x >> 6] = m;
  __syncthreads();
  if (threadIdx.x == 0) atomicMax(amax + it.slot, __float_as_uint(fmaxf(fmaxf(part[0], part[1]), fmaxf(part[2], part[3]))));
}
template <bool HI = false>
__global__ __launch_bounds__(256) void wprep_rows_kernel(D3dpWPrepTable tb, f16* __restrict__ base, const unsigned* __restrict__ amax,
                                                         float* __restrict__ unscale) {
  const D3dpWPrepItem it = tb.it[blockIdx.y];
  const float sc = dyn_scale(amax[it.slot]);
  if (blockIdx.x == 0 && threadIdx.x == 0) unscale[it.slot] = 1.0f / sc;
  f16* d = base + 2 * it.off;
  const int G8 = it.K / 8;
  const size_t n = (size_t)it.N * G8;
  for (size_t i = (size_t)blockIdx.x * blockDim.x + threadIdx.x; i < n; i += (size_t)gridDim.x * blockDim.x) {
    const size_t r = i / G8;
    const int c = (int)(i - r * G8) * 8;
    const float4 a = *reinterpret_cast<const float4*>(it.w + r * it.K + c), b = *reinterpret_cast<const float4*>(it.w + r * it.K + c + 4);
    const float v[8] = {a.x, a.y, a.z, a.w, b.x, b.y, b.z, b.w};
    f16x8 hi, lo;
#pragma unroll
    for (int e = 0; e < 8; ++e) { f16 h, l; split2h_scaled(v[e] * sc, h, l); hi[e] = h; lo[e] = l; }
    f16* row = HI ? d + r * (size_t)it.K + c : d + r * 2 * (size_t)it.K + h2i_col(c);
    *reinterpret_cast<f16x8*>(row) = hi;
    if constexpr (!HI) *reinterpret_cast<f16x8*>(row + kH2iLo) = lo;
  }
}
template <bool HI = false>
__global__ __launch_bounds__(256) void wprep_cols_kernel(D3dpWPrepTable tb, f16* __restrict__ base, const unsigned* __restrict__ amax) {
  __shared__ float tile[32][33];
  const D3dpWPrepItem it = tb.it[blockIdx.y];
  const float sc = dyn_scale(amax[it.slot]);
  f16* d = base + 2 * it.off;
  const int tr = it.N / 32, tc = it.K / 32;
  const int tx = threadIdx.x & 31, ty = threadIdx.x >> 5;
  for (int tI = blockIdx.x; tI < tr * tc; tI += gridDim.x) {
    const int r0 = (tI / tc) * 32, c0 = (tI % tc) * 32;
    __syncthreads();
    for (int k = ty; k < 32; k += 8) tile[k][tx] = it.w[(size_t)(r0 + k) * it.K + c0 + tx] * sc;
    __syncthreads();
    for (int k = ty; k < 32; k += 8) {
      f16 a, b;
      split2h_scaled(tile[tx][k], a, b);
      if constexpr (HI) {
        d[(size_t)(c0 + k) * it.N + r0 + tx] = a;
      } else {
        f16* blk = d + (size_t)(c0 + k) * 2 * it.N + (size_t)(r0 / 32) * 64;
        blk[tx] = a;
        blk[32 + tx] = b;
      }
    }
  }
}

__global__ __launch_bounds__(256) void sum_partials_kernel(const float4* __restrict__ part, float4* __restrict__ out, size_t n4, int Z) {
  for (size_t i = (size_t)blockIdx.x * blockDim.x + threadIdx.x; i < n4; i += (size_t)gridDim.x * blockDim.x) {
    const float4* p = part + i;
    float4 a = p[0];
    int z = 1;
    for (; z + 8 <= Z; z += 8) {
      float4 v[8];
#pragma unroll
      for (int u = 0; u < 8; ++u) v[u] = p[(size_t)(z + u) * n4];
#pragma unroll
      for (int u = 0; u < 8; ++u) { a.x += v[u].x; a.y += v[u].y; a.z += v[u].z; a.w += v[u].w; }
    }
    for (; z < Z; ++z) {
      const float4 v = p[(size_t)z * n4];
      a.x += v.x; a.y += v.y; a.z += v.z; a.w += v.w;
    }
    out[i] = a;
  }
}

__global__ __launch_bounds__(256) void sum_partials_many_kernel(D3dpSumTable tb) {
  const float4* part = reinterpret_cast<const float4*>(tb.part[blockIdx.y]);
  float4* out = reinterpret_cast<float4*>(tb.out[blockIdx.y]);
  const size_t n4 = tb.n4[blockIdx.y];
  const int Z = tb.Z;
  for (size_t i = (size_t)blockIdx.x * 256 + threadIdx.x; i < n4; i += (size_t)gridDim.x * 256) {
    const float4* p = part + i;
    float4 a = p[0];
    int z = 1;
    for (; z + 4 <= Z; z += 4) {
      float4 v[4];
#pragma unroll
      for (int u = 0; u < 4; ++u) v[u] = p[(size_t)(z + u) * n4];
#pragma unroll
      for (int u = 0; u < 4; ++u) { a.x += v[u].x; a.y += v[u].y; a.z += v[u].z; a.w += v[u].w; }
    }
    for (; z < Z; ++z) {
      const float4 v = p[(size_t)z * n4];
      a.x += v.x; a.y += v.y; a.z += v.z; a.w += v.w;
    }
    out[i] = a;
  }
}

__global__ __launch_bounds__(256) void sum_partials_bias_kernel(const float* __restrict__ part, const float* __restrict__ bias,
                                                                float* __restrict__ out, size_t n, int N, int Z,
                                                                unsigned* __restrict__ amax, int amax_pos) {
  __shared__ float pm[4];
  float m = 0.f;
  for (size_t i = (size_t)blockIdx.x * blockDim.x + threadIdx.x; i < n; i += (size_t)gridDim.x * blockDim.x) {
    float a = part[i];
    for (int z = 1; z < Z; ++z) a += part[(size_t)z * n + i];
    a = bias ? a + bias[i % N] : a;
    out[i] = a;
    m = fmaxf(m, amax_pos ? a : fabsf(a));
  }
  if (amax) {
    m = wave_max(m);
    if ((threadIdx.x & 63) == 0) pm[threadIdx.x >> 6] = m;
    __syncthreads();
    if (threadIdx.x == 0) atomicMax(amax, __float_as_uint(fmaxf(fmaxf(pm[0], pm[1]), fmaxf(pm[2], pm[3]))));
  }
}

}

int d3dp_launch_linear_f16x2_dyn(const void* A2, const void* W2, const float* bias, const float* dynA, const float* dynW,
                                 float* out, int M, int N, int Kfull, int Z, hipStream_t st, unsigned* amax_out, int amax_pos,
                                 int rem_blocks, int passes, int rows_hi) {
  if (M <= 0 || N % 4 != 0 || Z < 1 || Kfull % (XBK * Z) != 0 || (amax_out && Z != 1) || (passes != 1 && passes != 3)) return -1;
  if (rows_hi && (passes != 1 || Kfull % (2 * XBK * Z) != 0)) return -1;
  const int NKz = Kfull / XBK / Z;
  const bool rem = rem_blocks && Z == 1 && M > XBM && M % XBM != 0 && NKz % (2 * XNCW) == 0;
  const int tm = rem ? M / XBM : (M + XBM - 1) / XBM, tn = (N + XBN - 1) / XBN;
  static PerDeviceOnce once, once1, once_hi;
  const auto kern = rows_hi ? gemm_f16x2_dyn_kernel<1, true> : passes == 1 ? gemm_f16x2_dyn_kernel<1> : gemm_f16x2_dyn_kernel<3>;
  const int cus = (rows_hi ? once_hi : passes == 1 ? once1 : once).get([&](int dev) {
    return d3dp_lds_opt_in(reinterpret_cast<const void*>(kern), XNSTAGE * XSTAGE + 64) < 0 ? -3 : d3dp_cu_count(dev);
  });
  if (cus < 0) return -3;
  const int items = tm * tn * Z, grid = items < cus ? items : cus;
  hipLaunchKernelGGL(kern, dim3(grid), dim3((XNCW + 4) * 64), XNSTAGE * XSTAGE + 64, st, (const f16*)A2,
                     (const f16*)W2, bias, dynA, dynW, out, M, N, Kfull, NKz, tn, tm * tn, items, amax_out, amax_pos,
                     rem ? tm * XBM : 0);
  return 0;
}

void d3dp_launch_split2_dyn(const float* src, void* dst, int R, int C, int Cpad, const unsigned* amax, float* unscale,
                            hipStream_t st, int rows_hi) {
  const size_t n = (size_t)R * (Cpad / 8);
  const unsigned blocks = (unsigned)((n + 255) / 256 < 4096 ? (n + 255) / 256 : 4096);
  hipLaunchKernelGGL((rows_hi ? split2h_dyn_kernel<true> : split2h_dyn_kernel<false>), dim3(blocks ? blocks : 1), dim3(256), 0, st, src, (f16*)dst, R, C, Cpad, amax, unscale);
}

void d3dp_launch_split2_t_dyn(const float* src, void* dst, int R, int C, int Rpad, const unsigned* amax, float* unscale,
                              hipStream_t st) {
  hipLaunchKernelGGL(split2h_t_dyn_kernel, dim3(Rpad / 32, (C + 31) / 32), dim3(256), 0, st, src, (f16*)dst, R, C, Rpad, amax,
                     unscale);
}

int d3dp_launch_dyprep(const float* src, void* drow, void* dcol, float* colpart, int R, int C, int Rpad, const unsigned* amax,
                       float* unscale, hipStream_t st) {
  if (C % 32 != 0 || Rpad % 32 != 0 || Rpad < R) return -1;
  hipLaunchKernelGGL(dyprep_kernel, dim3(D3DP_DYPREP_ROWS, C / 32), dim3(256), 0, st, src, (f16*)drow, (f16*)dcol, colpart, R, C, Rpad, amax, unscale);
  return 0;
}

int d3dp_launch_rowprep_ln(const float* src, const float* w, const float* b, float eps, void* drow, int R, int Rpad, int C,
                           const unsigned* amax, float* unscale, hipStream_t st, int rows_hi) {
  if (C % 32 != 0 || C > 512 || Rpad < R || !w || !b) return -1;
  int g = (Rpad + 3) / 4;
  if (g > 1024) g = 1024;
  hipLaunchKernelGGL((rows_hi ? rowprep_ln_kernel<true> : rowprep_ln_kernel<false>), dim3(g), dim3(256), 0, st, src, w, b, eps, (f16*)drow, R, Rpad, C, amax, unscale);
  return 0;
}

int d3dp_launch_rowprep(const float* src, void* drow, float* colpart, int* rows, int R, int Rpad, int C, const unsigned* amax,
                        float* unscale, hipStream_t st, const float* mask, int axis, int F, int J, const float* gelu_pre, int rows_hi) {
  if (C % 32 != 0 || Rpad < R || C > 1536) return -1;
  int g = (Rpad + 3) / 4;
  const int cap = colpart ? D3DP_ROWPREP_ROWS : 1024;
  if (g > cap) g = cap;
  if (rows) *rows = g;
  const int P = (C + 511) / 512;
  f16* d = (f16*)drow;
  if (mask && (J < 1 || F < 1)) return -1;
#define D3DP_ROWPREP(PP, GG) hipLaunchKernelGGL((rows_hi ? rowprep_kernel<PP, GG, true> : rowprep_kernel<PP, GG, false>), dim3(g), dim3(256), 0, st, src, d, colpart, R, Rpad, C, amax, unscale, mask, axis, F, J, gelu_pre)
  if (gelu_pre) {
    if (P == 1) D3DP_ROWPREP(1, true); else if (P == 2) D3DP_ROWPREP(2, true); else D3DP_ROWPREP(3, true);
  } else {
    if (P == 1) D3DP_ROWPREP(1, false); else if (P == 2) D3DP_ROWPREP(2, false); else D3DP_ROWPREP(3, false);
  }
#undef D3DP_ROWPREP
  return 0;
}

int d3dp_launch_gelu_rowprep(const float* src, void* drow, int R, int Rpad, int C, const unsigned* pmax, unsigned* amax_out,
                             float* unscale, hipStream_t st, int rows_hi) {
  if (C % 32 != 0 || Rpad < R) return -1;
  const size_t n = (size_t)Rpad * (C / 8);
  const unsigned blocks = (unsigned)((n + 511) / 512 < 2048 ? (n + 511) / 512 : 2048);
  hipLaunchKernelGGL((rows_hi ? gelu_rowprep_kernel<true> : gelu_rowprep_kernel<false>), dim3(blocks ? blocks : 1), dim3(256), 0, st, src, (f16*)drow, R, Rpad, C, pmax, amax_out, unscale);
  return 0;
}

static_assert(XBM == D3DP_TN_TILE_N && XBN == D3DP_TN_TILE_K, "train_plan.h: the tile d3dp_tn_applies asks whole multiples of");
int d3dp_launch_linear_f16x2_tn_many(const D3dpTnProduct* prods, int n, int Tp, int Z, hipStream_t st, int passes, int rows_hi) {
  if (n < 1 || n > D3DP_TN_MAX || Z < 1 || Tp % (XBK * Z) != 0 || (passes != 1 && passes != 3) || (rows_hi && passes != 1)) return -1;
  D3dpTnTable tb{};
  tb.n = n;
  int tiles = 0;
  for (int i = 0; i < n; ++i) {
    tb.p[i] = prods[i];
    if (!d3dp_tn_applies(tb.p[i].N, tb.p[i].K)) return -1;
    tb.p[i].tiles_k = tb.p[i].K / XBN;
    tb.p[i].tile0 = tiles;
    tiles += (tb.p[i].N / XBM) * tb.p[i].tiles_k;
  }
  const int NKz = Tp / XBK / Z;
  static PerDeviceOnce once, once1, once_hi;
  const auto kern = rows_hi ? gemm_f16x2_tn_kernel<1, true> : passes == 1 ? gemm_f16x2_tn_kernel<1> : gemm_f16x2_tn_kernel<3>;
  const int lds = XNSTAGE * (rows_hi ? XTN_HI_STAGE : XSTAGE);
  const int cus = (rows_hi ? once_hi : passes == 1 ? once1 : once).get([&](int dev) {
    return d3dp_lds_opt_in(reinterpret_cast<const void*>(kern), lds) < 0 ? -3 : d3dp_cu_count(dev);
  });
  if (cus < 0) return -3;
  const int items = tiles * Z, grid = items < cus ? items : cus;
  hipLaunchKernelGGL(kern, dim3(grid), dim3((XNCW + 4) * 64), lds, st, tb, NKz, tiles, items);
  return 0;
}
int d3dp_launch_linear_f16x2_tn(const void* A2, const void* W2, const float* dynA, const float* dynW, float* out, int N, int K,
                                int Tp, int Z, hipStream_t st, int passes, int rows_hi) {
  const D3dpTnProduct one{A2, W2, dynA, dynW, out, N, K, 0, 0};
  return d3dp_launch_linear_f16x2_tn_many(&one, 1, Tp, Z, st, passes, rows_hi);
}

int d3dp_launch_wprep(const D3dpWPrepTable& tb, void* rows_base, void* cols_base, unsigned* amax, float* unscale, hipStream_t st,
                      int rows_hi) {
  if (tb.n < 1 || tb.n > D3DP_WPREP_MAX) return -1;
  for (int i = 0; i < tb.n; ++i)
    if (tb.it[i].N % 32 != 0 || tb.it[i].K % 32 != 0) return -1;
  hipLaunchKernelGGL(wprep_absmax_kernel, dim3(16, tb.n), dim3(256), 0, st, tb, amax);
  hipLaunchKernelGGL((rows_hi ? wprep_rows_kernel<true> : wprep_rows_kernel<false>), dim3(32, tb.n), dim3(256), 0, st, tb, (f16*)rows_base, (const unsigned*)amax, unscale);
  hipLaunchKernelGGL((rows_hi ? wprep_cols_kernel<true> : wprep_cols_kernel<false>), dim3(32, tb.n), dim3(256), 0, st, tb, (f16*)cols_base, (const unsigned*)amax);
  return 0;
}

void d3dp_launch_sum_partials_bias(const float* part, const float* bias, float* out, size_t n, int N, int Z, hipStream_t st,
                                   unsigned* amax, int amax_pos) {
  const unsigned cap = amax ? 256 : 2048;
  const unsigned blocks = (unsigned)((n + 255) / 256 < cap ? (n + 255) / 256 : cap);
  hipLaunchKernelGGL(sum_partials_bias_kernel, dim3(blocks ? blocks : 1), dim3(256), 0, st, part, bias, out, n, N, Z, amax, amax_pos);
}
void d3dp_launch_sum_partials_many(const D3dpSumTable& tb, hipStream_t st) {
  size_t most = 0;
  for (int i = 0; i < tb.n; ++i) most = tb.n4[i] > most ? tb.n4[i] : most;
  const unsigned blocks = (unsigned)((most + 255) / 256 < 1024 ? (most + 255) / 256 : 1024);
  hipLaunchKernelGGL(sum_partials_many_kernel, dim3(blocks ? blocks : 1, tb.n), dim3(256), 0, st, tb);
}
void d3dp_launch_sum_partials(const float* part, float* out, size_t n, int Z, hipStream_t st) {
  const size_t n4 = n / 4;
  const unsigned blocks = (unsigned)((n4 + 255) / 256 < 2048 ? (n4 + 255) / 256 : 2048);
  hipLaunchKernelGGL(sum_partials_kernel, dim3(blocks ? blocks : 1), dim3(256), 0, st, reinterpret_cast<const float4*>(part),
                     reinterpret_cast<float4*>(out), n4, Z);
}
```

d3dp_amd/csrc/kernels.h:

```cpp
#pragma once
#include <hip/hip_runtime.h>
#include <stdint.h>

#include <mutex>

#include "train_plan.h"

struct PerDeviceOnce {
  static constexpr int kMaxDev = 64;
  std::mutex mu;
  int val[kMaxDev] = {0};
  template <class F> int get(F&& fn) {
    int dev = 0;
    if (hipGetDevice(&dev) != hipSuccess || dev < 0 || dev >= kMaxDev) return -3;
    std::lock_guard<std::mutex> lock(mu);
    if (val[dev] <= 0) {
      const int v = fn(dev);
      if (v <= 0) return v < 0 ? v : -3;
      val[dev] = v;
    }
    return val[dev];
  }
};
inline int d3dp_cu_count(int dev) {
  hipDeviceProp_t prop;
  if (hipGetDeviceProperties(&prop, dev) != hipSuccess || prop.multiProcessorCount < 1) return -3;
  return prop.multiProcessorCount;
}
inline int d3dp_lds_opt_in(const void* kern, int bytes) {
  return hipFuncSetAttribute(kern, hipFuncAttributeMaxDynamicSharedMemorySize, bytes) == hipSuccess ? 1 : -3;
}

enum { EPI_BIAS = 0, EPI_GELU = 1, EPI_RESID = 2, EPI_PARTIAL = 3, EPI_QKV_PACK = 4, EPI_RESID_LN = 5, EPI_GELU_LN = 6,
       EPI_RESID_NORM = 7 };

int d3dp_launch_linear_bf16_stream(int epi, int out_f32, const void* A, const void* W, const float* bias, void* out,
                                   int M, int N, int K, hipStream_t st, int f16 = 0);
int d3dp_linear_stream_widths(int epi, const void* A, const void* W, const float* bias, void* out, int M, int N, int K,
                              hipStream_t st, int f16);
int d3dp_linear_stream_scaled(int epi, const void* A, const void* W, const float* bias, void* out, int M, int N, int K, hipStream_t st,
                              float m_acc, float m_bias, float m_inv);
int d3dp_launch_linear_bf16x3(int epi, const void* A3, const void* W3, const float* bias, float* outf, void* out3, int M,
                              int N, int K, hipStream_t st);
void d3dp_launch_split3(const float* src, void* dst, size_t n, hipStream_t st);
int d3dp_launch_linear_f16x2(int epi, const void* A2, const void* W2, const float* bias, float unscale, float oscale,
                             float* outf, void* out2, float* aux, unsigned* flag, int M, int N, int K, hipStream_t st,
                             int skew_d = 0, int pingpong = 0);
constexpr int X2_TILES_LAST_TO_FIRST = 0x100;
bool d3dp_x2_skew_applies(int epi, int M, int N, int K, int skew_d, int n_cu);
bool d3dp_x2_variants_built();
void d3dp_launch_rowbound(const float* W, const float* gamma, const float* beta, const float* bias, int N, int K,
                          unsigned* out, hipStream_t st);
void d3dp_launch_ln_combine(const float* slices, float* rowstat, int M, int C, float eps, hipStream_t st);
void d3dp_launch_fold_ln(const float* W, const float* gamma, const float* beta, const float* bias, float* Wp, float* c12,
                         int N, int K, hipStream_t st);
void d3dp_launch_split2(const float* src, void* dst, size_t n, float scale, hipStream_t st);
void d3dp_launch_absmax(const float* src, size_t n, unsigned* out, hipStream_t st);
void d3dp_launch_nonfinite_flag(const float* x, size_t n, unsigned* flag, hipStream_t st);
int d3dp_launch_linear_f16x2_dyn(const void* A2, const void* W2, const float* bias, const float* dynA, const float* dynW,
                                 float* out, int M, int N, int Kfull, int Z, hipStream_t st, unsigned* amax_out = nullptr,
                                 int amax_pos = 0, int rem_blocks = 0, int passes = 3, int rows_hi = 0);
int d3dp_launch_gelu_rowprep(const float* src, void* drow, int R, int Rpad, int C, const unsigned* pmax, unsigned* amax_out,
                             float* unscale, hipStream_t st, int rows_hi = 0);
void d3dp_launch_split2_dyn(const float* src, void* dst, int R, int C, int Cpad, const unsigned* amax, float* unscale,
                            hipStream_t st, int rows_hi = 0);
void d3dp_launch_split2_t_dyn(const float* src, void* dst, int R, int C, int Rpad, const unsigned* amax, float* unscale,
                              hipStream_t st);
int d3dp_launch_dyprep(const float* src, void* drow, void* dcol, float* colpart, int R, int C, int Rpad, const unsigned* amax,
                       float* unscale, hipStream_t st);
int d3dp_launch_rowprep(const float* src, void* drow, float* colpart, int* rows, int R, int Rpad, int C, const unsigned* amax,
                        float* unscale, hipStream_t st, const float* mask = nullptr, int axis = 0, int F = 1, int J = 1,
                        const float* gelu_pre = nullptr, int rows_hi = 0);
int d3dp_launch_rowprep_ln(const float* src, const float* w, const float* b, float eps, void* drow, int R, int Rpad, int C,
                           const unsigned* amax, float* unscale, hipStream_t st, int rows_hi = 0);
int d3dp_launch_linear_f16x2_tn(const void* A2, const void* W2, const float* dynA, const float* dynW, float* out, int N, int K,
                                int Tp, int Z, hipStream_t st, int passes = 3, int rows_hi = 0);
struct D3dpTnProduct {
  const void* A2; const void* W2;
  const float* dynA; const float* dynW;
  float* out;
  int N, K;
  int tiles_k, tile0;
};
struct D3dpTnTable { D3dpTnProduct p[D3DP_TN_MAX]; int n; };
int d3dp_launch_linear_f16x2_tn_many(const D3dpTnProduct* prods, int n, int Tp, int Z, hipStream_t st, int passes = 3, int rows_hi = 0);
struct D3dpSumTable { const float* part[D3DP_TN_MAX]; float* out[D3DP_TN_MAX]; size_t n4[D3DP_TN_MAX]; int Z; int n; };
void d3dp_launch_sum_partials_many(const D3dpSumTable& tb, hipStream_t st);
struct D3dpWPrepItem { const float* w; int N, K, slot, pad; size_t off; };
struct D3dpWPrepTable { D3dpWPrepItem it[D3DP_WPREP_MAX]; int n; };
int d3dp_launch_wprep(const D3dpWPrepTable& tb, void* rows_base, void* cols_base, unsigned* amax, float* unscale, hipStream_t st,
                      int rows_hi = 0);
void d3dp_launch_sum_partials(const float* part, float* out, size_t n, int Z, hipStream_t st);
void d3dp_launch_sum_partials_bias(const float* part, const float* bias, float* out, size_t n, int N, int Z, hipStream_t st,
                                   unsigned* amax = nullptr, int amax_pos = 0);
int d3dp_launch_linear_f32_splitk(const float* A, const float* W, float* out, int M, int N, int K, hipStream_t st, float* part,
                                  size_t part_floats);
int d3dp_launch_linear_f32(int epi, const float* A, const float* W, const float* bias, float* out, int M, int N,
                           int K, hipStream_t st);

struct SeqMap { int n_tok, inner, outer_stride, inner_stride, tok_stride; };
int d3dp_launch_attn_rows(int act_bf16, const void* qkv, void* out, int n_seq, SeqMap map, int C, int heads,
                          hipStream_t st, unsigned* amax = nullptr);
int d3dp_launch_attn_temporal_f32(int act, const void* qkv, void* out, int n_seq, SeqMap map, int C, int heads,
                                  hipStream_t st);
int d3dp_launch_attn_temporal_bf16(const void* qkv, void* out, int n_seq, SeqMap map, int C, int heads,
                                   hipStream_t st, int f16 = 0, int hd_true = 0);
int d3dp_launch_attn_spatial_bf16(const void* qkv, void* out, int n_seq, SeqMap map, int C, int heads, hipStream_t st,
                                  int f16 = 0, int hd_true = 0);
int d3dp_attn_fast_padded(int axis, const void* qkv, void* out, int n_seq, SeqMap map, int C, int heads, hipStream_t st, int f16,
                          int hd_true);
int d3dp_attn_fast_scaled(int axis, const void* qkv, void* out, int n_seq, SeqMap map, int C, int heads, hipStream_t st, float emul);
int d3dp_launch_attn_x2(int act, int axis, const void* qkv, void* out, int n_seq, SeqMap map, int C, int heads,
                        float act_scale, hipStream_t st, int hd_true = 0);
void d3dp_launch_qkv_pack_x2(const float* src, void* dst, size_t T, int C, float act_scale, hipStream_t st);

int d3dp_launch_time_mlp(const int64_t* t, const float* freq, const float* w1, const float* b1, const float* w2,
                         const float* b2, float* temb, int B, int C, hipStream_t st);
int d3dp_launch_embed_ln(int act_bf16, const float* x2d, const float* x3d, const float* temb, const float* ew,
                         const float* eb, const float* spos, const float* lnw, const float* lnb, float eps, float* x,
                         void* xn, int seq0, int n_seq, int H, int F, int J, int C, hipStream_t st, int SP = 0);
int d3dp_launch_ln(int act_bf16, float* x, const void* yadd, int write_x, const float* w, const float* b, float eps,
                   void* xn, int T, int C, hipStream_t st);
int d3dp_launch_ln2(int act_bf16, float* x, const void* yadd0, const void* yadd, const float* wa, const float* ba, const float* pos,
                    const float* wb, const float* bb, float eps, void* xn, int T, int C, int F, int J, hipStream_t st,
                    int SP = 0);
int d3dp_launch_ln2_defer(int act_bf16, const float* x, const float* wa, const float* ba, const float* wb, const float* bb, float eps,
                          void* xn, float* stat, int T, int C, hipStream_t st);
int d3dp_rows2_embed_ln(int act, const float* x2d, const float* x3d, const float* temb, const float* ew, const float* eb,
                        const float* spos, const float* lnw, const float* lnb, float eps, float* x, void* xn, int seq0, int n_seq,
                        int H, int F, int J, int C, hipStream_t st, int SP);
int d3dp_rows2_ln(int act, float* x, const void* yadd, int write_x, const float* w, const float* b, float eps, void* xn, int T, int C,
                  hipStream_t st);
int d3dp_rows2_ln2(int act, float* x, const void* yadd0, const void* yadd, const float* wa, const float* ba, const float* pos,
                   const float* wb, const float* bb, float eps, void* xn, int T, int C, int F, int J, hipStream_t st, int SP);
int d3dp_rows2_head(int act, const float* x, const void* yadd0, const void* yadd, const float* wa, const float* ba, float eps_a,
                    const float* wh, const float* bh, float eps_h, const float* w, const float* b, float* out, int T, int C,
                    hipStream_t st, int FJ, int SP);
int d3dp_launch_ln_scaled(const float* x, const void* yadd, float m, const float* w, const float* b, float eps, void* xn, int T, int C,
                          hipStream_t st);
int d3dp_launch_ln2_scaled(float* x, const void* yadd0, float m0, const void* yadd, float m, const float* wa, const float* ba,
                           const float* pos, const float* wb, const float* bb, float eps, void* xn, int T, int C, int F, int J,
                           hipStream_t st, int SP);
int d3dp_launch_head_scaled(const float* x, const void* yadd0, float m0, const void* yadd, float m, const float* wa, const float* ba,
                            float eps_a, const float* wh, const float* bh, float eps_h, const float* w, const float* b, float* out, int T,
                            int C, hipStream_t st, int FJ, int SP);
int d3dp_launch_head(int act_bf16, const float* x, const void* yadd0, const void* yadd, const float* wa, const float* ba, float eps_a, const float* wh,
                     const float* bh, float eps_h, const float* w, const float* b, float* out, int T, int C,
                     hipStream_t st, int FJ = 0, int SP = 0);

int d3dp_launch_ddim_pre(const float* img, float* xt2, const int* perm, float scale, int B, int per_b, int J,
                         hipStream_t st);
int d3dp_launch_ddim_post(const float* pred2, const float* img, const float* noise, const int* perm, float scale,
                          double sqrt_recip, double sqrt_recipm1, float c_xstart, float c_noise, float sigma,
                          int last, float* x_start, size_t xs_bstride, float* img_next, int B, int per_b, int J,
                          hipStream_t st);
int d3dp_launch_q_sample(const float* x0, const float* noise, const double* a, const double* b, float scale,
                         float* out, int B, int per_b, hipStream_t st);

int d3dp_launch_jpma(const float* pred, const float* traj, const float* cam, const float* gt2d, const float* gt3d,
                     float* agg, int* sel, float* err_sel, float* err_min, float* win, float* jbest, float* mean,
                     int h_offset, int B, int K, int H, int F, int J, int root_joint, int linear, hipStream_t st,
                     int h_inner = 0, size_t outer_stride = 0);

void d3dp_launch_to_bf16(const float* s, void* d, size_t n, hipStream_t st, int f16 = 0);
void d3dp_launch_to_bf16_pad(const float* s, void* d, int rows, int cols, int src_cols, int pad_rows, int hd, int hdp, int heads,
                             hipStream_t st, int f16);

int d3dp_set_error(int code, const char* msg);
int d3dp_check_launch(const char* what);
extern "C" int d3dp_clip_count(int32_t n, int32_t F);

int d3dp_train_add_mask_ln(const float* x_in, const float* y, const float* mask, int axis, int F, int J, const float* w,
                           const float* b, float eps, float* x_out, float* xn, unsigned* amax, int T, int C, hipStream_t st,
                           void* op = nullptr, int Tp = 0, float* op_unscale = nullptr, int op_hi = 0);
int d3dp_train_add_mask_ln2(const float* x_in, const float* y, const float* mask, int axis, int F, int J, const float* wa,
                            const float* ba, float eps_a, const float* pos, const float* wb, const float* bb, float eps_b,
                            float* x_out, float* x_next, float* xn, unsigned* amax, int T, int C, hipStream_t st, void* op = nullptr,
                            int Tp = 0, float* op_unscale = nullptr, int op_hi = 0);
int d3dp_train_ln_pos(const float* x, const float* w, const float* b, float eps, const float* pos, int F, int J, float* y,
                      int T, int C, hipStream_t st);
int d3dp_train_ln_bwd(const float* dy, const float* xb, const float* wb, float eps_b, const float* dres, float* g_out,
                      const float* xa, const float* wa, float eps_a, float* dx, const float* mask, int axis, int F, int J,
                      float* dxm, unsigned* amax, float* part_b, float* part_a, int T, int C, hipStream_t st);
constexpr int D3DP_REDUCE_MAX = 80;
struct D3dpReduceItem { const float* part; float* dst; unsigned n, count, stride, accumulate; };
struct D3dpReduceTable { D3dpReduceItem it[D3DP_REDUCE_MAX]; int count; };
int d3dp_train_reduce_many(const D3dpReduceTable& tb, hipStream_t st);
int d3dp_train_gelu_fwd(const float* x, float* y, size_t n, unsigned* amax, hipStream_t st);
int d3dp_train_gelu_bwd(const float* dh, const float* x, float* dpre, size_t n, unsigned* amax, hipStream_t st);
int d3dp_train_colsum(const float* in, float* part, int* rows, int max_rows, int T, int C, hipStream_t st);
constexpr int D3DP_ZERO_MAX = 192;
struct D3dpZeroTable { float* p[D3DP_ZERO_MAX]; unsigned n[D3DP_ZERO_MAX]; int count; };
int d3dp_train_zero_many(const D3dpZeroTable& tb, hipStream_t st);
int d3dp_train_groupsum(const float* in, float* out, int T, int C, int mode, int F, int J, int slices, hipStream_t st);
int d3dp_train_transpose_pad(const float* in, float* out, int R, int C, int Rpad, hipStream_t st);
int d3dp_train_attn_bwd(const float* qkv, const float* o, const float* dout, float* dqkv, void* stats, int n_seq,
                        SeqMap map, int C, int heads, hipStream_t st, bool chunked = false);
int d3dp_train_attn_x2_fwd(const float* qkv, float* out, void* stats, int n_seq, SeqMap map, int C, int heads,
                           const unsigned* amax_qkv, unsigned* amax_out, hipStream_t st, void* op = nullptr, int T = 0, int Tp = 0,
                           float* op_unscale = nullptr, int passes = 3, int op_hi = 0);
int d3dp_train_attn_x2_bwd(const float* qkv, const float* o, const float* dout, float* dqkv, void* stats, int n_seq, SeqMap map,
                           int C, int heads, const unsigned* amax_qkv, const unsigned* amax_do, unsigned* amax_out,
                           hipStream_t st, int part = 0, int passes = 3);
int d3dp_train_attn_x2_padded(int which, const float* qkv, const float* o, const float* dout, float* out, float* dqkv, void* stats,
                              int n_seq, SeqMap map, int C, int heads, const unsigned* amax_qkv, const unsigned* amax_do,
                              unsigned* amax_out, hipStream_t st);
int d3dp_train_attn_x2_1p(int which, const float* qkv, const float* o, const float* dout, float* out, float* dqkv, void* stats,
                          int n_seq, SeqMap map, int C, int heads, const unsigned* amax_qkv, const unsigned* amax_do,
                          unsigned* amax_out, hipStream_t st, void* op, int T, int Tp, float* op_unscale);
int d3dp_train_attn_x2_fwd_hi(int passes, const float* qkv, float* out, void* stats, int n_seq, SeqMap map, int C, int heads,
                              const unsigned* amax_qkv, unsigned* amax_out, hipStream_t st, void* op, int T, int Tp, float* op_unscale);
int d3dp_train_embed_bwd(const float* dx, const float* x2d, const float* x3d, float* part, int T, int C, hipStream_t st);
int d3dp_train_head_linear(const float* z, const float* w, const float* b, float* out, int T, int C, hipStream_t st);
int d3dp_train_head_bwd(const float* g, const float* z, const float* w, float* dz, float* part, int* rows, int T, int C,
                        hipStream_t st);
int d3dp_train_time_mlp(const int64_t* t, const float* freq, const float* w1, const float* b1, const float* w2, const float* b2,
                        float* hidden, float* temb, int B, int C, hipStream_t st);
int d3dp_train_time_mlp_bwd(const int64_t* t, const float* freq, const float* w1, const float* b1, const float* w2,
                            const float* dtemb, float* dw1, float* db1, float* dw2, float* db2, int B, int C,
                            hipStream_t st);

inline bool d3dp_width_instantiated(int C) { return C == 64 || C == 128 || C == 256 || C == 512; }
int d3dp_train_g_add_mask_ln(const float* x_in, const float* y, const float* mask, int axis, int F, int J, const float* w,
                             const float* b, float eps, float* x_out, float* xn, unsigned* amax, int T, int C, hipStream_t st);
int d3dp_train_g_add_mask_ln2(const float* x_in, const float* y, const float* mask, int axis, int F, int J, const float* wa,
                              const float* ba, float eps_a, const float* pos, const float* wb, const float* bb, float eps_b,
                              float* x_out, float* x_next, float* xn, unsigned* amax, int T, int C, hipStream_t st);
int d3dp_train_g_ln_pos(const float* x, const float* w, const float* b, float eps, const float* pos, int F, int J, float* y, int T,
                        int C, hipStream_t st);
int d3dp_train_g_ln_bwd(const float* dy, const float* xb, const float* wb, float eps_b, const float* dres, float* g_out,
                        const float* xa, const float* wa, float eps_a, float* dx, const float* mask, int axis, int F, int J,
                        float* dxm, unsigned* amax, float* part_b, float* part_a, int T, int C, int blocks, hipStream_t st);
int d3dp_train_g_head_linear(const float* z, const float* w, const float* b, float* out, int T, int C, hipStream_t st);
int d3dp_train_g_time_mlp_bwd(const int64_t* t, const float* freq, const float* w1, const float* b1, const float* w2,
                              const float* dtemb, float* dw1, float* db1, float* dw2, float* db2, int B, int C, hipStream_t st);
```

d3dp_amd/csrc/train_attn.hip:

```cpp
#include "common.h"
#include "kernels.h"
#include "ta_common.h"

namespace {

struct TAStat { float L, D; };

template <int NW>
__device__ __forceinline__ void ta_block_amax(float am, unsigned* amax, float* part) {
  am = wave_max(am);
  if ((threadIdx.x & 63) == 0) part[threadIdx.x >> 6] = am;
  __syncthreads();
  if (threadIdx.x == 0 && amax) {
    float m = part[0];
#pragma unroll
    for (int w = 1; w < NW; ++w) m = fmaxf(m, part[w]);
    atomicMax(amax, __float_as_uint(m));
  }
}

template <int NKT, int NW, int NKC, int HD, bool PAD = false, int PASSES = 3, bool OPHI = false>
__global__ __launch_bounds__(NW * 64, 4) void tattn_fwd_kernel(const float* __restrict__ qkv, float* __restrict__ out,
                                                           TAStat* __restrict__ stats, SeqMap map, int C, int heads, int groups,
                                                           int n_work, const unsigned* __restrict__ amax_qkv,
// ... 443 lines not shown
        row_op(fgr, wave, gh, gl);
        const float2 ld_ = st[row];
        f32x4 a, b, c, d;
        ta_rows_pair<PLANE, HD, PASSES>(fk, 0, qh, ql, a, b);
        ta_rows_pair<PLANE, HD, PASSES>(fv, 0, gh, gl, c, d);
        float ds[8];
#pragma unroll
        for (int r = 0; r < 4; ++r) {
          const float pa = __builtin_amdgcn_exp2f(fmaf(a[r], cexp, -ld_.x)), pb = __builtin_amdgcn_exp2f(fmaf(b[r], cexp, -ld_.x));
          ds[r] = pa * (fmaf(c[r], cdp, -ld_.y)) * scale;
          ds[4 + r] = pb * (fmaf(d[r], cdp, -ld_.y)) * scale;
          if (4 * fg + r >= n) ds[r] = 0.f;
          if (16 + 4 * fg + r >= n) ds[4 + r] = 0.f;
        }
        const int eb = max(20, ta_exp_of_max(ds));
        f16x8 sh, sl;
        ta_split_run<PASSES>(ds, eb, sh, sl);
        f32x4 dq[ND];
#pragma unroll
        for (int dn = 0; dn < ND; ++dn) dq[dn] = (f32x4){0.f, 0.f, 0.f, 0.f};
        ta_tr_chunk<PLANE, HD, PASSES>(fk, 0, sh, sl, dq);
        if (live) {
          const float un = 1.0f / sq;
          float* dst = dqkv + tok * ld + head * hd + fg * 4;
#pragma unroll
          for (int dn = 0; dn < ND; ++dn) {
            if constexpr (PAD) { if (dn * 16 + fg * 4 >= hd) continue; }
            const float4 r4 = make_float4(ldexpf(dq[dn][0], eb - 140) * un, ldexpf(dq[dn][1], eb - 140) * un,
                                          ldexpf(dq[dn][2], eb - 140) * un, ldexpf(dq[dn][3], eb - 140) * un);
            am = fmaxf(am, fmaxf(fmaxf(fabsf(r4.x), fabsf(r4.y)), fmaxf(fabsf(r4.z), fabsf(r4.w))));
            *reinterpret_cast<float4*>(dst + dn * 16) = r4;
          }
        }
      }
      {
        frag kh[NQ], kl[NQ], vh[NQ], vl[NQ];
        row_op(fk, wave, kh, kl);
        row_op(fv, wave, vh, vl);
        f32x4 a, b, c, d;
        ta_rows_pair<PLANE, HD, PASSES>(fq, 0, kh, kl, a, b);
        ta_rows_pair<PLANE, HD, PASSES>(fgr, 0, vh, vl, c, d);
        float ds[8];
        f16x8 ph, pl;
#pragma unroll
        for (int r = 0; r < 4; ++r) {
          const float2 sa = st[4 * fg + r], sb = st[16 + 4 * fg + r];
          float pa = __builtin_amdgcn_exp2f(fmaf(a[r], cexp, -sa.x)), pb = __builtin_amdgcn_exp2f(fmaf(b[r], cexp, -sb.x));
          if (!live) { pa = 0.f; pb = 0.f; }
          ds[r] = pa * (fmaf(c[r], cdp, -sa.y)) * scale;
          ds[4 + r] = pb * (fmaf(d[r], cdp, -sb.y)) * scale;
          if constexpr (PASSES == 1) {
            ph[r] = (f16)(pa * 1024.0f); ph[4 + r] = (f16)(pb * 1024.0f);
          } else {
          const float ya = ta_opaque(pa * 1024.0f), yb = ta_opaque(pb * 1024.0f);
          const f16 ha = (f16)ya, hb = (f16)yb;
          ph[r] = ha; pl[r] = (f16)(ya - (float)ha);
          ph[4 + r] = hb; pl[4 + r] = (f16)(yb - (float)hb);
          }
        }
        f32x4 dk[ND], dv[ND];
#pragma unroll
        for (int dn = 0; dn < ND; ++dn) { dk[dn] = (f32x4){0.f, 0.f, 0.f, 0.f}; dv[dn] = dk[dn]; }
        ta_tr_chunk<PLANE, HD, PASSES>(fgr, 0, ph, PASSES == 1 ? ph : pl, dv);
        const int eb = max(20, ta_exp_of_max(ds));
        f16x8 sh, sl;
        ta_split_run<PASSES>(ds, eb, sh, sl);
        ta_tr_chunk<PLANE, HD, PASSES>(fq, 0, sh, sl, dk);
        if (live) {
          const float uk = 1.0f / sq, uv = 1.0f / (sg * 1024.0f);
          float* dst = dqkv + tok * ld + C + head * hd + fg * 4;
#pragma unroll
          for (int dn = 0; dn < ND; ++dn) {
            if constexpr (PAD) { if (dn * 16 + fg * 4 >= hd) continue; }
            const float4 k4 = make_float4(ldexpf(dk[dn][0], eb - 140) * uk, ldexpf(dk[dn][1], eb - 140) * uk,
                                          ldexpf(dk[dn][2], eb - 140) * uk, ldexpf(dk[dn][3], eb - 140) * uk);
            const float4 v4 = make_float4(dv[dn][0] * uv, dv[dn][1] * uv, dv[dn][2] * uv, dv[dn][3] * uv);
            am = fmaxf(am, fmaxf(fmaxf(fabsf(k4.x), fabsf(k4.y)), fmaxf(fabsf(k4.z), fabsf(k4.w))));
            am = fmaxf(am, fmaxf(fmaxf(fabsf(v4.x), fabsf(v4.y)), fmaxf(fabsf(v4.z), fabsf(v4.w))));
            *reinterpret_cast<float4*>(dst + dn * 16) = k4;
            *reinterpret_cast<float4*>(dst + C + dn * 16) = v4;
          }
        }
      }
    }
  }
  if (amax_out) ta_block_amax<NW>(am, amax_out, part);
}

struct TAOperand { f16* op; int T, Tp; float* unscale; };
template <int NKT, int HD, bool PAD = false, int PASSES = 3, bool OPHI = false>
int ta_launch(int which, const float* qkv, const float* o, const float* dout, float* out, float* dqkv, void* stats, int n_seq,
              SeqMap map, int C, int heads, const unsigned* amax_qkv, const unsigned* amax_do, unsigned* amax_out,
              hipStream_t st, TAOperand po = {nullptr, 0, 0, nullptr}) {
  constexpr int NK = 16 * NKT, NW = NKT <= 2 ? 2 : (NKT <= 4 ? 4 : 8);
  constexpr int NKC = NKT > 8 ? 8 : NKT;
  static_assert(!PAD || PASSES == 3, "padded heads: no one-pass form");
  if (PAD && po.op) return -1;
  constexpr int NKC_KV = (NKT > 16 || (HD < 64 && NKT > 8)) ? 8 : NKT;
  constexpr int WPE_KV = HD < 64 ? 4 : 2;
  constexpr int ROWB = 2 * HD;
  constexpr int NPL = ta_planes(PASSES);
  const size_t lds = (size_t)2 * NPL * NKC * 16 * ROWB + 64, lds_kv = (size_t)2 * NPL * NKC_KV * 16 * ROWB + NKC_KV * 16 * 8 + 64, lds_fwd = lds;
  (void)NK;
  if constexpr (OPHI) {
    static_assert(!PAD, "padded heads write no operand rows");
    if (which != 0 || !po.op) return -1;
    static PerDeviceOnce once_hi;
    if (once_hi.get([&](int) {
          return d3dp_lds_opt_in(reinterpret_cast<const void*>(tattn_fwd_kernel<NKT, NW, NKC, HD, false, PASSES, true>), 160 * 1024);
        }) < 0) return -3;
    const int tiles = (map.n_tok + 15) / 16, groups = (tiles + NW - 1) / NW;
    const int n_work = n_seq * heads * groups;
    hipLaunchKernelGGL((tattn_fwd_kernel<NKT, NW, NKC, HD, false, PASSES, true>), dim3(n_work < 2048 ? n_work : 2048), dim3(NW * 64), lds_fwd, st, qkv, out,
                       reinterpret_cast<TAStat*>(stats), map, C, heads, groups, n_work, amax_qkv, amax_out, po.op, po.T, po.Tp, po.unscale);
    return 0;
  } else {
  static PerDeviceOnce once;
  if (once.get([&](int) {
        return d3dp_lds_opt_in(reinterpret_cast<const void*>(tattn_fwd_kernel<NKT, NW, NKC, HD, PAD, PASSES>), 160 * 1024) < 0 ? -3
               : d3dp_lds_opt_in(reinterpret_cast<const void*>(tattn_bwd_q_kernel<NKT, NW, NKC, 4, HD, PAD, PASSES>), 160 * 1024) < 0 ? -3
               : d3dp_lds_opt_in(reinterpret_cast<const void*>(tattn_bwd_kv_kernel<NKT, NW, NKC_KV, WPE_KV, HD, PAD, PASSES>), 160 * 1024);
      }) < 0) return -3;
  const int tiles = (map.n_tok + 15) / 16, groups = (tiles + NW - 1) / NW;
  const int n_work = n_seq * heads * groups;
  const dim3 grid(n_work < 2048 ? n_work : 2048), blk(NW * 64);
  TAStat* s = reinterpret_cast<TAStat*>(stats);
  if (which == 0)
    hipLaunchKernelGGL((tattn_fwd_kernel<NKT, NW, NKC, HD, PAD, PASSES>), grid, blk, lds_fwd, st, qkv, out, s, map, C, heads, groups, n_work, amax_qkv, amax_out,
                       po.op, po.T, po.Tp, po.unscale);
  else if (NKT == 2) {
    if (which != 3) {
      const dim3 g2(n_seq * heads < 4096 ? n_seq * heads : 4096);
      hipLaunchKernelGGL((tattn_bwd_small_kernel<HD, PAD, PASSES>), g2, dim3(128), 0, st, qkv, o, dout, dqkv, (const TAStat*)s, map, C, heads, n_seq * heads,
                         amax_qkv, amax_do, amax_out);
    }
  } else {
    if (which != 3)
      hipLaunchKernelGGL((tattn_bwd_q_kernel<NKT, NW, NKC, 4, HD, PAD, PASSES>), grid, blk, lds, st, qkv, o, dout, dqkv, s, map, C, heads, groups, n_work,
                         amax_qkv, amax_do, amax_out);
    if (which != 2)
      hipLaunchKernelGGL((tattn_bwd_kv_kernel<NKT, NW, NKC_KV, WPE_KV, HD, PAD, PASSES>), grid, blk, lds_kv, st, qkv, dout, dqkv, (const TAStat*)s, map, C, heads, groups,
                         n_work, amax_qkv, amax_do, amax_out);
  }
  return 0;
  }
}

#ifdef D3DP_TA_HI_TU
#define TA_CASE(NKT_, HD_)                                                                                                                      \
  return passes == 1 ? ta_launch<NKT_, HD_, false, 1, true>(0, qkv, nullptr, nullptr, out, nullptr, stats, n_seq, map, C, heads, amax_qkv, nullptr, amax_out, st, po) \
                     : ta_launch<NKT_, HD_, false, 3, true>(0, qkv, nullptr, nullptr, out, nullptr, stats, n_seq, map, C, heads, amax_qkv, nullptr, amax_out, st, po);
#elif defined(D3DP_TA_PAD_TU)
#define TA_CASE(NKT_, HD_) return ta_launch<NKT_, HD_, true>(which, qkv, o, dout, out, dqkv, stats, n_seq, map, C, heads, amax_qkv, amax_do, amax_out, st);
#elif defined(D3DP_TA_1P_TU)
#define TA_CASE(NKT_, HD_) return ta_launch<NKT_, HD_, false, 1>(which, qkv, o, dout, out, dqkv, stats, n_seq, map, C, heads, amax_qkv, amax_do, amax_out, st, po);
#else
#define TA_CASE(NKT_, HD_) return ta_launch<NKT_, HD_>(which, qkv, o, dout, out, dqkv, stats, n_seq, map, C, heads, amax_qkv, amax_do, amax_out, st, po);
#endif
#define TA_LENGTHS(HD_)              \
  if (n <= 32) { TA_CASE(2, HD_) }   \
  if (n <= 64) { TA_CASE(4, HD_) }   \
  if (n <= 128) { TA_CASE(8, HD_) }  \
  if (n <= 256) { TA_CASE(16, HD_) } \
  if (n <= 512) { TA_CASE(32, HD_) } \
  TA_CASE(64, HD_)

#if !defined(D3DP_TA_PAD_TU) && !defined(D3DP_TA_1P_TU) && !defined(D3DP_TA_HI_TU)
int ta_dispatch(int which, const float* qkv, const float* o, const float* dout, float* out, float* dqkv, void* stats, int n_seq,
                SeqMap map, int C, int heads, const unsigned* amax_qkv, const unsigned* amax_do, unsigned* amax_out,
                hipStream_t st, int passes, TAOperand po = {nullptr, 0, 0, nullptr}, int op_hi = 0) {
  const int n = map.n_tok;
  if (passes != 1 && passes != 3) return -1;
  if (heads < 1 || C % heads != 0 || C % 4 != 0 || n < 1 || n > 1024 || !amax_qkv || !stats) return -2;
  if (po.op && (po.Tp < po.T || !po.unscale || C % 32 != 0)) return -1;
  if (po.op && op_hi) {
    if (which != 0) return -1;
    return d3dp_train_attn_x2_fwd_hi(passes, qkv, out, stats, n_seq, map, C, heads, amax_qkv, amax_out, st, po.op, po.T, po.Tp, po.unscale);
  }
  if (passes == 1) {
    const int hd1 = C / heads;
    if (hd1 != 64 && hd1 != 32 && hd1 != 16) return -2;
    return d3dp_train_attn_x2_1p(which, qkv, o, dout, out, dqkv, stats, n_seq, map, C, heads, amax_qkv, amax_do, amax_out, st, po.op, po.T,
                                 po.Tp, po.unscale);
  }
  switch (C / heads) {
    case 64: { TA_LENGTHS(64) }
    case 32: { TA_LENGTHS(32) }
    case 16: { TA_LENGTHS(16) }
    case 56: case 48: case 40: case 24:
      if (po.op) return -1;
      return d3dp_train_attn_x2_padded(which, qkv, o, dout, out, dqkv, stats, n_seq, map, C, heads, amax_qkv, amax_do, amax_out, st);
    default: return -2;
  }
}
#endif

}

#ifdef D3DP_TA_HI_TU
int d3dp_train_attn_x2_fwd_hi(int passes, const float* qkv, float* out, void* stats, int n_seq, SeqMap map, int C, int heads,
                              const unsigned* amax_qkv, unsigned* amax_out, hipStream_t st, void* op, int T, int Tp, float* op_unscale) {
  const int n = map.n_tok, hd = heads > 0 ? C / heads : 0;
  if (heads < 1 || hd * heads != C || n < 1 || n > 1024 || !amax_qkv || !stats || !op || (passes != 1 && passes != 3)) return -2;
  const TAOperand po{(f16*)op, T, Tp, op_unscale};
  if (hd == 64) { TA_LENGTHS(64) }
  if (hd == 32) { TA_LENGTHS(32) }
  return -2;
}
#elif defined(D3DP_TA_PAD_TU)
int d3dp_train_attn_x2_padded(int which, const float* qkv, const float* o, const float* dout, float* out, float* dqkv, void* stats,
                              int n_seq, SeqMap map, int C, int heads, const unsigned* amax_qkv, const unsigned* amax_do,
                              unsigned* amax_out, hipStream_t st) {
  const int n = map.n_tok, hd = heads > 0 ? C / heads : 0;
  if (heads < 1 || hd * heads != C || n < 1 || n > 1024 || !amax_qkv || !stats) return -2;
  if (hd == 24) { TA_LENGTHS(32) }
  if (hd == 40 || hd == 48 || hd == 56) {
    if (n <= 32) { TA_CASE(2, 64) }
    if (n <= 128) { TA_CASE(8, 64) }
    if (n <= 256) { TA_CASE(16, 64) }
    if (n <= 512) { TA_CASE(32, 64) }
    TA_CASE(64, 64)
  }
  return -2;
}
#elif defined(D3DP_TA_1P_TU)
int d3dp_train_attn_x2_1p(int which, const float* qkv, const float* o, const float* dout, float* out, float* dqkv, void* stats,
                          int n_seq, SeqMap map, int C, int heads, const unsigned* amax_qkv, const unsigned* amax_do,
                          unsigned* amax_out, hipStream_t st, void* op, int T, int Tp, float* op_unscale) {
  const int n = map.n_tok, hd = heads > 0 ? C / heads : 0;
  if (heads < 1 || hd * heads != C || n < 1 || n > 1024 || !amax_qkv || !stats) return -2;
  const TAOperand po{(f16*)op, T, Tp, op_unscale};
  if (hd == 64) { TA_LENGTHS(64) }
  if (hd == 32) { TA_LENGTHS(32) }
  if (hd == 16) { TA_LENGTHS(16) }
  return -2;
}
#else
static_assert(sizeof(TAStat) == D3DP_TRAIN_ATTN_X2_STAT_BYTES, "train_plan.h: d3dp_train_attn_x2_stats_bytes");

int d3dp_train_attn_x2_fwd(const float* qkv, float* out, void* stats, int n_seq, SeqMap map, int C, int heads,
                           const unsigned* amax_qkv, unsigned* amax_out, hipStream_t st, void* op, int T, int Tp,
                           float* op_unscale, int passes, int op_hi) {
  if (!qkv || !out) return -1;
  return ta_dispatch(0, qkv, nullptr, nullptr, out, nullptr, stats, n_seq, map, C, heads, amax_qkv, nullptr, amax_out, st, passes,
                     TAOperand{(f16*)op, T, Tp, op_unscale}, op_hi);
}
int d3dp_train_attn_x2_bwd(const float* qkv, const float* o, const float* dout, float* dqkv, void* stats, int n_seq, SeqMap map,
                           int C, int heads, const unsigned* amax_qkv, const unsigned* amax_do, unsigned* amax_out,
                           hipStream_t st, int part, int passes) {
  if (!qkv || !o || !dout || !dqkv || !amax_do || part < 0 || part > 2) return -1;
  return ta_dispatch(1 + part, qkv, o, dout, nullptr, dqkv, stats, n_seq, map, C, heads, amax_qkv, amax_do, amax_out, st, passes);
}
#endif
#undef TA_LENGTHS
#undef TA_CASE
```

d3dp_amd/csrc/train_plan.h:

```cpp
#pragma once
#include <cstddef>

#include "ctx_plan.h"

constexpr int D3DP_DYPREP_ROWS = 96;
constexpr int D3DP_ROWPREP_ROWS = 512;
constexpr int D3DP_LN_BWD_BLOCKS = 512;
constexpr int D3DP_EMBED_BWD_ROWS = 64;
constexpr int D3DP_TN_MAX = 4;
constexpr size_t D3DP_TRAIN_ATTN_STAT_BYTES = 12;
constexpr size_t D3DP_TRAIN_ATTN_X2_STAT_BYTES = 8;
inline int d3dp_train_ln_bwd_blocks(int T) { return (T + 3) / 4 < D3DP_LN_BWD_BLOCKS ? (T + 3) / 4 : D3DP_LN_BWD_BLOCKS; }
inline size_t d3dp_train_attn_stats_bytes(int n_seq, int n_tok, int heads) { return (size_t)n_seq * heads * n_tok * D3DP_TRAIN_ATTN_STAT_BYTES; }
inline size_t d3dp_train_attn_x2_stats_bytes(int n_seq, int n_tok, int heads) { return (size_t)n_seq * heads * n_tok * D3DP_TRAIN_ATTN_X2_STAT_BYTES; }

constexpr int kTrainSlots = 8192, kTrainBwdSlot0 = 4096, kTrainQkvSlot0 = 2048, kTrainPmaxSlot0 = 3072;

struct TrainLayout {
  size_t T, Tpad, C, Hd, unit;
  size_t temb, x_final, saved0, saved_stride;
  size_t o_xin, o_qkv, o_att, o_xmid, o_hpre, o_xout;
  size_t xn, y, hid, dA, dB, dC, dqkv, dh, z, At, Xt, Wt, dtemb, stats;
  size_t op_a, op_w, op_at, part, part_rem, slots;
  size_t dy_set_floats;
  size_t part_floats;
  size_t part_rem_floats;
  size_t op_a2, op_at2, part2;
  size_t x_cols, x_block;
  size_t w_rows, w_cols, w_block;
  size_t Tp_max;
  size_t stats_x2, stats_x2_stride;
  size_t red, red_floats;
  int ln_rows;
  int bias_rows;
  int head_rows, embed_bias_rows;
  int group_slices;
  size_t total_floats;
};

inline TrainLayout train_layout(const d3dp_cfg& g, int B) {
  TrainLayout L{};
  L.T = (size_t)B * g.frames * g.joints;
  L.Tpad = (L.T + 15) / 16 * 16;
  L.C = g.channels; L.Hd = g.hidden; L.unit = L.T * L.C;
  L.ln_rows = d3dp_train_ln_bwd_blocks((int)L.T);
  L.bias_rows = std::max(D3DP_DYPREP_ROWS, D3DP_ROWPREP_ROWS);
  L.head_rows = 512; L.embed_bias_rows = 512; L.group_slices = 32;
  size_t off = 0;
  auto take = [&](size_t n) { size_t o = off; off += (n + 63) / 64 * 64; return o; };
  L.temb = take((size_t)B * L.C);
  L.x_final = take(L.unit);
  L.o_xin = 0; L.o_qkv = L.unit; L.o_att = 4 * L.unit; L.o_xmid = 5 * L.unit; L.o_hpre = 6 * L.unit;
  L.o_xout = 6 * L.unit + L.T * L.Hd;
  L.saved_stride = (7 * L.unit + L.T * L.Hd + 63) / 64 * 64;
  L.saved0 = take(L.saved_stride * 2 * g.depth);
  L.xn = take(L.unit); L.y = take(L.unit); L.hid = take(L.T * L.Hd);
  L.dA = take(L.unit); L.dB = take(L.unit); L.dC = take(L.unit);
  L.dqkv = take(3 * L.unit); L.dh = take(L.T * L.Hd); L.z = take(L.unit);
  const size_t wide = std::max<size_t>(3 * L.C, L.Hd);
  L.At = take(wide * L.Tpad); L.Xt = take(wide * L.Tpad); L.Wt = take(wide * wide);
  L.dtemb = take((size_t)B * 2 * L.C);
  L.stats = take(d3dp_train_attn_stats_bytes(B * std::max(g.frames, g.joints), std::max(g.frames, g.joints), g.heads) / 4 + 64);
  {
    const size_t fmax = std::max<size_t>(3 * L.C, L.Hd), kmax = std::max<size_t>(L.C, L.Hd);
    L.Tp_max = ((L.T + 31) / 32 + 64) * 32;
    const size_t dy_all = 5 * L.C + L.Hd;
    L.dy_set_floats = L.Tp_max * dy_all;
    L.op_a = take(L.dy_set_floats);
    L.op_w = take(fmax * kmax);
    L.op_at = take(fmax * L.Tp_max);
    L.part_floats = (size_t)(1024 + 64) * 256 * 128;
    L.part = take(L.part_floats);
    L.op_a2 = take(L.dy_set_floats); L.op_at2 = take(fmax * L.Tp_max); L.part2 = take(L.part_floats);
    L.part_rem_floats = (size_t)16 * 256 * fmax;
    L.part_rem = take(L.part_rem_floats);
    L.slots = take(2 * kTrainSlots);
    L.w_block = 4 * L.C * L.C + 2 * L.Hd * L.C;
    L.x_block = (3 * L.C + L.Hd) * L.Tp_max;
    L.x_cols = take(L.x_block * 2 * g.depth);
    L.w_rows = take(L.w_block * 2 * g.depth);
    L.w_cols = take(L.w_block * 2 * g.depth);
  }
  L.stats_x2_stride = (d3dp_train_attn_x2_stats_bytes(B * g.joints, g.frames, g.heads) / 4 + 63) / 64 * 64;
  L.stats_x2 = take(L.stats_x2_stride * 2 * g.depth);
  {
    const size_t lnb = (size_t)D3DP_LN_BWD_BLOCKS * 2 * L.C;
    L.red_floats = (size_t)(6 * g.depth + 2) * lnb
                   + (size_t)2 * g.depth * L.bias_rows * (5 * L.C + L.Hd + 256)
                   + (size_t)L.head_rows * (3 * L.C + 4) + (size_t)D3DP_EMBED_BWD_ROWS * 5 * L.C + (size_t)L.embed_bias_rows * L.C
                   + (size_t)L.group_slices * (g.joints + (size_t)B) * L.C + 4096;
    L.red = take(L.red_floats);
  }
  L.total_floats = off;
  return L;
}

inline bool train_attn_head_dim(int hd) { return mfma_head_dim(hd) || hd == 24 || hd == 40 || hd == 48 || hd == 56; }

struct TrainPath {
  bool use_x2, attn_x2_t, attn_x2_s, needs_aux;
  bool attn_x2(int axis) const { return axis == 1 ? attn_x2_t : attn_x2_s; }
};
inline TrainPath plan_train_path(const CtxPlan& c, const d3dp_cfg& g) {
  TrainPath p{};
  p.use_x2 = train_linears_split(c, g);
  p.attn_x2_t = p.use_x2 && c.train_attn_x2 > 0 && train_attn_head_dim(g.channels / g.heads) && g.frames <= 1024;
  p.attn_x2_s = p.attn_x2_t && c.train_attn_x2 > 1;
  p.needs_aux = g.mode == D3DP_MODE_TRAIN && p.use_x2 && c.train_overlap;
  return p;
}

enum TrainLinearId { kQkv = 0, kProj = 1, kFc1 = 2, kFc2 = 3 };

enum class TrainOperand {
  ROWS,
  ROWS_T,
  LN_INPUT,
  PRODUCER
};
enum class TrainTailForm {
  WHOLE_TILES,
  REM_BLOCKS,
  SPLIT_REM
};
struct TrainTail { TrainTailForm form; int Z; };
inline TrainTail train_tail(int T, int N, int K, int n_cu, bool tail_blocks, size_t part_rem_floats) {
  const int tn = (N + 127) / 128, q = T / 256, rem = T - q * 256;
  const int rounds_all = ((q + (rem ? 1 : 0)) * tn + n_cu - 1) / n_cu, rounds_full = (q * tn + n_cu - 1) / n_cu;
  const int nk = K / 32;
  int Z = 1;
  for (int z = 2; z <= 16; ++z)
    if (nk % z == 0) Z = z;
  if (tail_blocks && rem && q && rounds_all > rounds_full && nk % 16 == 0) return {TrainTailForm::REM_BLOCKS, 1};
  if (rem == 0 || q == 0 || rounds_all == rounds_full || Z == 1 || nk < 32 || (size_t)Z * rem * N > part_rem_floats)
    return {TrainTailForm::WHOLE_TILES, 1};
  return {TrainTailForm::SPLIT_REM, Z};
}

struct TrainLinear {
  int N, K;
  bool tn;
  int Z, Tp;
  int pad_rows;
  TrainOperand src;
  TrainTail fwd_tail, dgrad_tail;
};

struct TrainPlan {
  TrainPath path;
  bool use_x2;
  int T, passes, overlap_sets;
  int attn_passes;
  bool rows_hi;
  bool attn_bwd_chunked;
  TrainLinear lin[4];
  bool ln_fused;
  bool ln_direct;
  TrainOperand qkv_src0;
  bool att_direct_s, att_direct_t;
  bool att_direct(int axis) const { return axis == 1 ? att_direct_t : att_direct_s; }
  bool attn_t_f32_mfma;
  bool gelu_operand;
  bool gip;
  bool mip1, mip2;
  bool batched;
  bool merged;
  int mZ, mTp;
  bool rows_fit;
  bool parts_fit;

  TrainOperand source(int blk, int j) const {
    if (j == kQkv && blk == 0) return qkv_src0;
    if (j == kProj && att_direct(blk & 1)) return TrainOperand::PRODUCER;
    return lin[j].src;
  }
};

inline TrainPlan plan_train_step(const CtxPlan& c, const d3dp_cfg& g, int B, int n_cu) {
  TrainPlan P{};
  const TrainLayout L = train_layout(g, B);
  const int T = (int)L.T, C = g.channels, Hd = g.hidden;
  P.path = plan_train_path(c, g);
  P.use_x2 = P.path.use_x2;
  P.T = T; P.passes = c.train_passes; P.overlap_sets = c.train_overlap_sets;
  P.attn_passes = c.train_attn_passes;
  P.attn_bwd_chunked = c.train_long_attn;
  P.rows_hi = c.train_rows_hi && P.path.use_x2;
  const int shape[4][2] = {{3 * C, C}, {C, C}, {Hd, C}, {C, Hd}};
  for (int j = 0; j < 4; ++j) { P.lin[j].N = shape[j][0]; P.lin[j].K = shape[j][1]; }
  if (!P.use_x2) return P;
  const int nk = (T + 31) / 32;
  {
    int tiles = 0;
    bool ok = c.train_wgrad_merged;
    size_t nk_sum = 0;
    for (int j = 3; j >= 0; --j) {
      const int N = shape[j][0], K = shape[j][1];
      ok = ok && d3dp_tn_applies(N, K); tiles += ((N + 255) / 256) * ((K + 127) / 128); nk_sum += (size_t)N * K;
    }
    P.mZ = std::max(1, std::min(std::min(n_cu / std::max(tiles, 1), 64), nk / 4));
    P.mTp = P.mZ * ((nk + P.mZ - 1) / P.mZ) * 32;
    P.merged = ok && (size_t)P.mTp <= L.Tp_max && (size_t)P.mZ * nk_sum <= L.part_floats;
  }
  auto ln_operand_applies = [](int N, int K) { return d3dp_tn_applies(N, K) && K <= 512; };
  P.ln_fused = ln_operand_applies(3 * C, C) && ln_operand_applies(Hd, C);
  P.ln_direct = P.ln_fused && c.train_ln_direct && C % 256 == 0;
  P.gelu_operand = d3dp_tn_applies(C, Hd);
  P.att_direct_s = P.path.attn_x2(0) && P.ln_direct && d3dp_tn_applies(C, C);
  P.att_direct_t = P.path.attn_x2(1) && P.ln_direct && d3dp_tn_applies(C, C);
  P.attn_t_f32_mfma = !P.path.attn_x2(1) && C / g.heads == 64 && g.frames <= 256;
  P.gip = c.train_gelu_in_prep && d3dp_tn_applies(Hd, C) && Hd <= 1536;
  P.mip2 = d3dp_tn_applies(C, Hd); P.mip1 = d3dp_tn_applies(C, C);
  P.batched = 8 * g.depth <= D3DP_WPREP_MAX;
  P.rows_fit = P.parts_fit = true;
  for (int j = 0; j < 4; ++j) {
    TrainLinear& p = P.lin[j];
    p.tn = d3dp_tn_applies(p.N, p.K);
    {
      const int tiles = ((p.N + 255) / 256) * ((p.K + 127) / 128);
      p.Z = std::max(1, std::min(std::min(n_cu / tiles, 64), nk / 4));
      const int nkz = (nk + p.Z - 1) / p.Z;
      p.Tp = p.Z * nkz * 32;
    }
    p.pad_rows = P.merged ? std::max(p.Tp, P.mTp) : p.Tp;
    const TrainOperand pass = p.tn ? TrainOperand::ROWS : TrainOperand::ROWS_T;
    p.src = j == kFc2 ? (P.gelu_operand ? TrainOperand::PRODUCER : pass)
          : j == kProj ? pass
          : P.ln_direct ? TrainOperand::PRODUCER : P.ln_fused ? TrainOperand::LN_INPUT : pass;
    p.fwd_tail = train_tail(T, p.N, p.K, n_cu, c.train_tail_blocks, L.part_rem_floats);
    p.dgrad_tail = train_tail(T, p.K, p.N, n_cu, c.train_tail_blocks, L.part_rem_floats);
    P.rows_fit = P.rows_fit && (size_t)p.pad_rows <= L.Tp_max;
    P.parts_fit = P.parts_fit && (size_t)p.Tp <= L.Tp_max && (size_t)p.Z * p.N * p.K <= L.part_floats;
  }
  P.qkv_src0 = P.ln_fused ? TrainOperand::LN_INPUT : P.lin[kQkv].src;
  return P;
}
```

Measured before the change: 51.74.

## Emit pre-split f16 q/k/v planes from QKV GEMM epilogue for temporal attention

The QKV linear epilogue now writes fp16 hi/lo split planes of q/k/v, scaled by a static bound computed once from the weights, LayerNorm gamma/beta and bias. The temporal x2 attention forward and backward kernels then read these planes directly instead of re-splitting the fp32 qkv rows, and with long sequences the fp32 qkv store is skipped. The aim is to cut the per-kernel absmax/split work and memory traffic in attention. In exchange the saved-activation workspace grows, a new bound kernel is added, and the weight-derived bound may be loose, which costs fp16 precision headroom.

```diff
diff --git a/d3dp_amd/csrc/capi_train.hip b/d3dp_amd/csrc/capi_train.hip
--- a/d3dp_amd/csrc/capi_train.hip
+++ b/d3dp_amd/csrc/capi_train.hip
@@ -86,6 +86,7 @@
   unsigned* amax() const { return reinterpret_cast<unsigned*>(ws + L.slots); }
   float* uns() const { return ws + L.slots + kTrainSlots; }
   unsigned* qkv_amax(int blk) const { return P.path.attn_x2(blk & 1) ? amax() + kQkvSlot0 + blk : nullptr; }
+  unsigned* qkv_scale(int blk) const { return P.presplit(blk) ? amax() + kTrainQkvBoundSlot0 + blk : qkv_amax(blk); }
   int begin(bool forward_pass) {
     next = forward_pass ? 0 : kBwdSlot0;
     return hipMemsetAsync(ws + L.slots + next, 0, (size_t)kBwdSlot0 * 4, st) == hipSuccess ? 0 : -3;
@@ -118,16 +119,25 @@
       const BlockDev& w = (blk & 1) ? c->tte[blk >> 1] : c->ste[blk >> 1];
       tb.it[l] = D3dpWPrepItem{lin_w(w, j), P.lin[j].N, P.lin[j].K, 2 * l + 1, 0, woff(l)};
     }
-    return d3dp_launch_wprep(tb, ws + L.w_rows, ws + L.w_cols, amax(), uns(), st, P.rows_hi);
+    const int r = d3dp_launch_wprep(tb, ws + L.w_rows, ws + L.w_cols, amax(), uns(), st, P.rows_hi);
+    if (r || !P.qkv_presplit) return r;
+    D3dpQkvBoundTable qb{};
+    for (int blk = 0; blk < 2 * c->cfg.depth; ++blk) {
+      if (!P.presplit(blk)) continue;
+      if (qb.n >= D3DP_QKV_BOUND_MAX) return -1;
+      const BlockDev& w = (blk & 1) ? c->tte[blk >> 1] : c->ste[blk >> 1];
+      qb.it[qb.n++] = D3dpQkvBoundItem{lin_w(w, kQkv), w.n1w, w.n1b, lin_b(w, kQkv), P.lin[kQkv].N, P.lin[kQkv].K, kTrainQkvBoundSlot0 + blk, 0};
+    }
+    return qb.n ? d3dp_launch_qkv_bound(qb, amax(), st) : 0;
   }
   int gemm(TrainTail tail, const float* A2, const float* W2, const float* bias, const float* ua, const float* uw, float* out, int N,
-           int K, unsigned* out_amax = nullptr, int amax_pos = 0) {
+           int K, unsigned* out_amax = nullptr, int amax_pos = 0, void* pk = nullptr, const unsigned* pk_bound = nullptr) {
     Scope ps(pc, T_LINEAR, st);
     const int T = P.T, passes = P.passes;
     if (tail.form != TrainTailForm::SPLIT_REM)
       return d3dp_launch_linear_f16x2_dyn(A2, W2, bias, ua, uw, out, T, N, K, 1, st, out_amax, amax_pos,
-                                          tail.form == TrainTailForm::REM_BLOCKS ? 1 : 0, passes, P.rows_hi);
-    if (P.rows_hi) return -1;
+                                          tail.form == TrainTailForm::REM_BLOCKS ? 1 : 0, passes, P.rows_hi, pk, pk_bound, pk && P.qkv_planes_only);
+    if (P.rows_hi || pk) return -1;
     const int q = T / 256, rem = T - q * 256;
     int r = d3dp_launch_linear_f16x2_dyn(A2, W2, bias, ua, uw, out, q * 256, N, K, 1, st, out_amax, amax_pos, 0, passes);
     if (r) return r;
@@ -136,7 +146,7 @@
     d3dp_launch_sum_partials_bias(ws + L.part_rem, bias, out + (size_t)q * 256 * N, (size_t)rem * N, N, tail.Z, st, out_amax, amax_pos);
     return 0;
   }
-  int forward(int blk, TrainLinearId j, const float* A, const BlockDev& w, float ln_eps, float* out) {
+  int forward(int blk, TrainLinearId j, const float* A, const BlockDev& w, float ln_eps, float* out, void* pk = nullptr) {
     const TrainLinear& p = P.lin[j];
     const int l = 4 * blk + j, sa = 2 * l, sw = 2 * l + 1, T = P.T, N = p.N, K = p.K;
     if (sw >= kBwdSlot0) return -1;
@@ -168,7 +178,7 @@
       d3dp_launch_absmax(W, (size_t)N * K, amax() + sw, st);
       rows(W, N, K, ws + L.op_w, sw);
     }
-    return gemm(p.fwd_tail, a2, w2, lin_b(w, j), uns() + sa, uns() + sw, out, N, K, out_amax, pmax ? 1 : 0);
+    return gemm(p.fwd_tail, a2, w2, lin_b(w, j), uns() + sa, uns() + sw, out, N, K, out_amax, pmax ? 1 : 0, pk, pk ? qkv_scale(blk) : nullptr);
   }
   int gelu_operand(int blk, const float* hpre) {
     const int l = 4 * blk + kFc2;
@@ -264,9 +274,9 @@
     LAUNCH_TRY(x2->begin(true));
     LAUNCH_TRY(x2->prepare_weights(c));
   }
-  auto lin = [&](int blk, TrainLinearId j, const float* src, float* out) -> int {
+  auto lin = [&](int blk, TrainLinearId j, const float* src, float* out, void* pk = nullptr) -> int {
     const BlockDev& w = (blk & 1) ? c->tte[blk >> 1] : c->ste[blk >> 1];
-    if (x2) return x2->forward(blk, j, src, w, g.eps_block, out);
+    if (x2) return x2->forward(blk, j, src, w, g.eps_block, out, pk);
     Scope ps_(pc, T_LINEAR, st);
     return lin32(src, lin_w(w, j), lin_b(w, j), out, T, P.lin[j].N, P.lin[j].K, st);
   };
@@ -282,7 +292,8 @@
     const BlockDev& w = kind ? c->tte[d] : c->ste[d];
     float* S = ws + L.saved0 + (size_t)blk * L.saved_stride;
     const bool ax2 = P.path.attn_x2(kind);
-    LAUNCH_TRY(lin(blk, kQkv, ln_fused ? S + L.o_xin : xn, S + L.o_qkv));
+    void* const qkv_pk = P.presplit(blk) ? S + L.o_qkv_pk : nullptr;
+    LAUNCH_TRY(lin(blk, kQkv, ln_fused ? S + L.o_xin : xn, S + L.o_qkv, qkv_pk));
     const bool att_direct = P.att_direct(kind);
     void* att_op = att_direct ? x2->x_op(4 * blk + 1) : nullptr;
     const int att_tp = att_direct ? P.lin[kProj].pad_rows : 0;
@@ -292,7 +303,8 @@
     auto attention = [&]() -> int {
       if (ax2)
         return d3dp_train_attn_x2_fwd(S + L.o_qkv, S + L.o_att, ws + L.stats_x2 + (size_t)blk * L.stats_x2_stride, n_seq, map, C,
-                                      g.heads, x2->qkv_amax(blk), slot(4 * blk + 1), st, att_op, T, att_tp, att_un, P.attn_passes, P.rows_hi);
+                                      g.heads, x2->qkv_scale(blk), slot(4 * blk + 1), st, att_op, T, att_tp, att_un, P.attn_passes, P.rows_hi,
+                                      qkv_pk);
       if (kind == 1 && P.attn_t_f32_mfma)
         return d3dp_launch_attn_temporal_f32(0, S + L.o_qkv, S + L.o_att, n_seq, map, C, g.heads, st);
       return d3dp_launch_attn_rows(0, S + L.o_qkv, S + L.o_att, n_seq, map, C, g.heads, st, slot(4 * blk + 1));
@@ -514,7 +526,7 @@
         TP(part == 2 ? (kind ? T_ATTN_BKV_T : T_ATTN_BKV_S) : (kind ? T_ATTN_BQ_T : T_ATTN_BQ_S),
            d3dp_train_attn_x2_bwd(S + L.o_qkv, S + L.o_att, dB, dqkv, ws + L.stats_x2 + (size_t)blk * L.stats_x2_stride,
                                   kind ? B * J : B * F, kind ? temporal_map(F, J) : spatial_map(F, J), C, g.heads,
-                                  x2->qkv_amax(blk), pado, paq, st, part, P.attn_passes));
+                                  x2->qkv_scale(blk), pado, paq, st, part, P.attn_passes, P.presplit(blk) ? S + L.o_qkv_pk : nullptr));
       ps_dqkv = pq;
     } else {
       LAUNCH_TRY(dgrad(blk, kProj, dy, dB));
diff --git a/d3dp_amd/csrc/ctx_plan.h b/d3dp_amd/csrc/ctx_plan.h
--- a/d3dp_amd/csrc/ctx_plan.h
+++ b/d3dp_amd/csrc/ctx_plan.h
@@ -12,7 +12,7 @@
              *train_overlap = nullptr, *train_gelu = nullptr, *train_wgrad = nullptr, *train_ln_operand = nullptr, *train_tail = nullptr,
              *train_attn = nullptr, *train_passes = nullptr, *fast_impl = nullptr, *fast16_range = nullptr, *x2_skew = nullptr,
              *x2_pp = nullptr, *x2_wide = nullptr, *seq_pad = nullptr, *fold_ln = nullptr, *train_long_attn = nullptr,
-             *train_attn_passes = nullptr, *train_rows = nullptr;
+             *train_attn_passes = nullptr, *train_rows = nullptr, *train_qkv = nullptr;
   static CtxEnv from_process() {
     CtxEnv e;
     e.exact_impl = getenv("D3DP_EXACT_IMPL");
@@ -37,6 +37,7 @@
     e.train_long_attn = getenv("D3DP_TRAIN_LONG_ATTN");
     e.train_attn_passes = getenv("D3DP_TRAIN_ATTN_PASSES");
     e.train_rows = getenv("D3DP_TRAIN_ROWS");
+    e.train_qkv = getenv("D3DP_TRAIN_QKV");
     return e;
   }
 };
@@ -47,6 +48,7 @@
   int train_passes = 3;
   int train_attn_passes = 3;
   bool train_rows_hi = false;
+  bool train_qkv_presplit = true;
   int exact_impl_req = 0;
   bool long_rows = false;
   bool fold = true;
@@ -89,6 +91,7 @@
 }
 constexpr int D3DP_TN_TILE_N = 256, D3DP_TN_TILE_K = 128;
 constexpr int D3DP_WPREP_MAX = 64;
+constexpr int D3DP_QKV_BOUND_MAX = 16;
 inline bool d3dp_tn_applies(int N, int K) { return N % D3DP_TN_TILE_N == 0 && K % D3DP_TN_TILE_K == 0; }
 inline bool train_linears_split(const CtxPlan& p, const d3dp_cfg& g) { return p.train_x2 && g.channels % 32 == 0 && g.hidden % 32 == 0; }
 
@@ -257,6 +260,12 @@
       p.train_rows_hi = true;
     }
   }
+  if (train && e.train_qkv) {
+    if (strcmp(e.train_qkv, "fp32") && strcmp(e.train_qkv, "presplit"))
+      return d3dp_fail(D3DP_ENOTSUP, "D3DP_TRAIN_QKV=%.32s: the values a TRAIN context takes are D3DP_TRAIN_QKV=fp32 (the training attention "
+                                "stages q / k / v from the fp32 qkv rows) and presplit (the default)", e.train_qkv);
+    p.train_qkv_presplit = e.train_qkv[0] != 'f';
+  }
   p.exact_impl_req = env_is(e.exact_impl, "bf16x3") ? 1 : env_is(e.exact_impl, "f32") ? 2 : 0;
   if (!width_inst) {
     if (p.exact_impl_req == 1)
diff --git a/d3dp_amd/csrc/gemm_x2_train.hip b/d3dp_amd/csrc/gemm_x2_train.hip
--- a/d3dp_amd/csrc/gemm_x2_train.hip
+++ b/d3dp_amd/csrc/gemm_x2_train.hip
@@ -7,15 +7,16 @@
 
 namespace {
 
-template <int PASSES, bool HI = false>
+template <int PASSES, bool HI = false, int PK = 0>
 __global__ __launch_bounds__(768) void gemm_f16x2_dyn_kernel(const f16* __restrict__ A2, const f16* __restrict__ W2,
                                                              const float* __restrict__ bias, const float* __restrict__ dynA,
                                                              const float* __restrict__ dynW, float* __restrict__ out, int M,
                                                              int N, int Kfull, int NKz, int tiles_n, int tiles_per_z,
                                                              int total_items, unsigned* __restrict__ amax_out, int amax_pos,
-                                                             int rem_m0) {
+                                                             int rem_m0, f16* __restrict__ pk, const unsigned* __restrict__ pk_bound) {
   static_assert(PASSES == 1 || PASSES == 3, "one pass (hi x hi) or the three-pass split scheme");
   static_assert(!HI || PASSES == 1, "hi-only rows hold no lo halves");
+  static_assert(!PK || (PASSES == 3 && !HI), "packed q / k / v rows: the three-pass product on split rows");
   constexpr int RS = HI ? 1 : 2;
   extern __shared__ __attribute__((aligned(16))) char smem[];
   const int G = gridDim.x;
@@ -81,6 +82,17 @@
   const int offA = (wr * 64 + fi) * 128 + swz128(fi, fg) * 16, offAl = offA ^ 64;
   const int offW = XA_BYTES + (wc * 64 + fi) * 128 + swz128(fi, fg) * 16, offWl = offW ^ 64;
   const float unscale = dynA[0] * dynW[0];
+  const float pk_sc = PK ? __uint_as_float(train_presplit_scale(pk_bound[0]).scale_bits) : 0.f;
+  const int pk_c = N / 3;
+  auto pk_store = [&](int m, int nb, const f32x4& v) {
+    const int sect = nb / pk_c;
+    f16* d = pk + (size_t)m * (2 * N) + sect * (2 * pk_c) + (nb - sect * pk_c);
+    f16x4 hi, lo;
+#pragma unroll
+    for (int e = 0; e < 4; ++e) { f16 h, l; split2h_scaled(v[e] * pk_sc, h, l); hi[e] = h; lo[e] = l; }
+    *reinterpret_cast<f16x4*>(d) = hi;
+    *reinterpret_cast<f16x4*>(d + pk_c) = lo;
+  };
   __builtin_amdgcn_s_setprio(1);
   float am = 0.f;
   int slot = 0;
@@ -147,7 +159,8 @@
             if (m < M) {
               const f32x4 v = {fmaf(sum[0][r], unscale, bz.x), fmaf(sum[1][r], unscale, bz.y), fmaf(sum[2][r], unscale, bz.z),
                                fmaf(sum[3][r], unscale, bz.w)};
-              *reinterpret_cast<f32x4*>(out + (size_t)m * N + nb) = v;
+              if constexpr (PK != 2) *reinterpret_cast<f32x4*>(out + (size_t)m * N + nb) = v;
+              if constexpr (PK) pk_store(m, nb, v);
               am = amax_pos ? fmaxf(am, fmaxf(fmaxf(v[0], v[1]), fmaxf(v[2], v[3])))
                             : fmaxf(am, fmaxf(fmaxf(fabsf(v[0]), fabsf(v[1])), fmaxf(fabsf(v[2]), fabsf(v[3]))));
             }
@@ -212,7 +225,8 @@
           if (m < M) {
             const f32x4 v = {fmaf(acc[mi][0][r], unscale, bz.x), fmaf(acc[mi][1][r], unscale, bz.y),
                              fmaf(acc[mi][2][r], unscale, bz.z), fmaf(acc[mi][3][r], unscale, bz.w)};
-            *reinterpret_cast<f32x4*>(o + (size_t)m * N) = v;
+            if constexpr (PK != 2) *reinterpret_cast<f32x4*>(o + (size_t)m * N) = v;
+            if constexpr (PK) pk_store(m, nb, v);
             am = amax_pos ? fmaxf(am, fmaxf(fmaxf(v[0], v[1]), fmaxf(v[2], v[3])))
                           : fmaxf(am, fmaxf(fmaxf(fabsf(v[0]), fabsf(v[1])), fmaxf(fabsf(v[2]), fabsf(v[3]))));
           }
@@ -844,22 +858,50 @@
 
 int d3dp_launch_linear_f16x2_dyn(const void* A2, const void* W2, const float* bias, const float* dynA, const float* dynW,
                                  float* out, int M, int N, int Kfull, int Z, hipStream_t st, unsigned* amax_out, int amax_pos,
-                                 int rem_blocks, int passes, int rows_hi) {
+                                 int rem_blocks, int passes, int rows_hi, void* pk, const unsigned* pk_bound, int pk_only) {
+  if (pk && (!pk_bound || passes != 3 || rows_hi || Z != 1 || N % 12 != 0)) return -1;
   if (M <= 0 || N % 4 != 0 || Z < 1 || Kfull % (XBK * Z) != 0 || (amax_out && Z != 1) || (passes != 1 && passes != 3)) return -1;
   if (rows_hi && (passes != 1 || Kfull % (2 * XBK * Z) != 0)) return -1;
   const int NKz = Kfull / XBK / Z;
   const bool rem = rem_blocks && Z == 1 && M > XBM && M % XBM != 0 && NKz % (2 * XNCW) == 0;
   const int tm = rem ? M / XBM : (M + XBM - 1) / XBM, tn = (N + XBN - 1) / XBN;
-  static PerDeviceOnce once, once1, once_hi;
-  const auto kern = rows_hi ? gemm_f16x2_dyn_kernel<1, true> : passes == 1 ? gemm_f16x2_dyn_kernel<1> : gemm_f16x2_dyn_kernel<3>;
-  const int cus = (rows_hi ? once_hi : passes == 1 ? once1 : once).get([&](int dev) {
+  static PerDeviceOnce once, once1, once_hi, once_pk, once_pk2;
+  const auto kern = pk ? (pk_only ? gemm_f16x2_dyn_kernel<3, false, 2> : gemm_f16x2_dyn_kernel<3, false, 1>)
+                       : rows_hi ? gemm_f16x2_dyn_kernel<1, true> : passes == 1 ? gemm_f16x2_dyn_kernel<1> : gemm_f16x2_dyn_kernel<3>;
+  const int cus = (pk ? (pk_only ? once_pk2 : once_pk) : rows_hi ? once_hi : passes == 1 ? once1 : once).get([&](int dev) {
     return d3dp_lds_opt_in(reinterpret_cast<const void*>(kern), XNSTAGE * XSTAGE + 64) < 0 ? -3 : d3dp_cu_count(dev);
   });
   if (cus < 0) return -3;
   const int items = tm * tn * Z, grid = items < cus ? items : cus;
   hipLaunchKernelGGL(kern, dim3(grid), dim3((XNCW + 4) * 64), XNSTAGE * XSTAGE + 64, st, (const f16*)A2,
                      (const f16*)W2, bias, dynA, dynW, out, M, N, Kfull, NKz, tn, tm * tn, items, amax_out, amax_pos,
-                     rem ? tm * XBM : 0);
+                     rem ? tm * XBM : 0, (f16*)pk, pk_bound);
+  return 0;
+}
+
+namespace {
+__global__ __launch_bounds__(256) void qkv_bound_kernel(D3dpQkvBoundTable tb, unsigned* __restrict__ amax) {
+  const D3dpQkvBoundItem it = tb.it[blockIdx.y];
+  const int lane = threadIdx.x & 63;
+  const float sq = sqrtf((float)(it.K - 1)) * 1.0001f;
+  float best = 0.f;
+  for (int n = blockIdx.x * 4 + (threadIdx.x >> 6); n < it.N; n += gridDim.x * 4) {
+    float a = 0.f;
+    for (int k = lane; k < it.K; k += 64) a = fmaf(fabsf(it.w[(size_t)n * it.K + k]), fmaf(sq, fabsf(it.gamma[k]), fabsf(it.beta[k])), a);
+    a = wave_sum(a);
+    const float v = (a + (it.bias ? fabsf(it.bias[n]) : 0.f)) * 1.001f;
+    best = v == v ? fmaxf(best, v) : INFINITY;
+  }
+  if (lane == 0) atomicMax(amax + it.slot, __float_as_uint(best));
+}
+}
+int d3dp_launch_qkv_bound(const D3dpQkvBoundTable& tb, unsigned* amax, hipStream_t st) {
+  if (tb.n < 1 || tb.n > D3DP_QKV_BOUND_MAX) return -1;
+  for (int i = 0; i < tb.n; ++i)
+    if (!tb.it[i].w || !tb.it[i].gamma || !tb.it[i].beta || tb.it[i].N < 1 || tb.it[i].K < 2 || tb.it[i].K > 2048) return -1;
+  int rows = 0;
+  for (int i = 0; i < tb.n; ++i) rows = tb.it[i].N > rows ? tb.it[i].N : rows;
+  hipLaunchKernelGGL(qkv_bound_kernel, dim3((rows + 3) / 4, tb.n), dim3(256), 0, st, tb, amax);
   return 0;
 }
 
diff --git a/d3dp_amd/csrc/kernels.h b/d3dp_amd/csrc/kernels.h
--- a/d3dp_amd/csrc/kernels.h
+++ b/d3dp_amd/csrc/kernels.h
@@ -59,7 +59,11 @@
 void d3dp_launch_nonfinite_flag(const float* x, size_t n, unsigned* flag, hipStream_t st);
 int d3dp_launch_linear_f16x2_dyn(const void* A2, const void* W2, const float* bias, const float* dynA, const float* dynW,
                                  float* out, int M, int N, int Kfull, int Z, hipStream_t st, unsigned* amax_out = nullptr,
-                                 int amax_pos = 0, int rem_blocks = 0, int passes = 3, int rows_hi = 0);
+                                 int amax_pos = 0, int rem_blocks = 0, int passes = 3, int rows_hi = 0, void* pk = nullptr,
+                                 const unsigned* pk_bound = nullptr, int pk_only = 0);
+struct D3dpQkvBoundItem { const float *w, *gamma, *beta, *bias; int N, K, slot, pad; };
+struct D3dpQkvBoundTable { D3dpQkvBoundItem it[D3DP_QKV_BOUND_MAX]; int n; };
+int d3dp_launch_qkv_bound(const D3dpQkvBoundTable& tb, unsigned* amax, hipStream_t st);
 int d3dp_launch_gelu_rowprep(const float* src, void* drow, int R, int Rpad, int C, const unsigned* pmax, unsigned* amax_out,
                              float* unscale, hipStream_t st, int rows_hi = 0);
 void d3dp_launch_split2_dyn(const float* src, void* dst, int R, int C, int Cpad, const unsigned* amax, float* unscale,
@@ -198,16 +202,19 @@
                         SeqMap map, int C, int heads, hipStream_t st, bool chunked = false);
 int d3dp_train_attn_x2_fwd(const float* qkv, float* out, void* stats, int n_seq, SeqMap map, int C, int heads,
                            const unsigned* amax_qkv, unsigned* amax_out, hipStream_t st, void* op = nullptr, int T = 0, int Tp = 0,
-                           float* op_unscale = nullptr, int passes = 3, int op_hi = 0);
+                           float* op_unscale = nullptr, int passes = 3, int op_hi = 0, const void* qkv_pk = nullptr);
 int d3dp_train_attn_x2_bwd(const float* qkv, const float* o, const float* dout, float* dqkv, void* stats, int n_seq, SeqMap map,
                            int C, int heads, const unsigned* amax_qkv, const unsigned* amax_do, unsigned* amax_out,
-                           hipStream_t st, int part = 0, int passes = 3);
+                           hipStream_t st, int part = 0, int passes = 3, const void* qkv_pk = nullptr);
 int d3dp_train_attn_x2_padded(int which, const float* qkv, const float* o, const float* dout, float* out, float* dqkv, void* stats,
                               int n_seq, SeqMap map, int C, int heads, const unsigned* amax_qkv, const unsigned* amax_do,
                               unsigned* amax_out, hipStream_t st);
 int d3dp_train_attn_x2_1p(int which, const float* qkv, const float* o, const float* dout, float* out, float* dqkv, void* stats,
                           int n_seq, SeqMap map, int C, int heads, const unsigned* amax_qkv, const unsigned* amax_do,
                           unsigned* amax_out, hipStream_t st, void* op, int T, int Tp, float* op_unscale);
+int d3dp_train_attn_x2_pre(int which, const void* pk, const float* o, const float* dout, float* out, float* dqkv, void* stats,
+                           int n_seq, SeqMap map, int C, int heads, const unsigned* bound_qkv, const unsigned* amax_do,
+                           unsigned* amax_out, hipStream_t st, void* op, int T, int Tp, float* op_unscale);
 int d3dp_train_attn_x2_fwd_hi(int passes, const float* qkv, float* out, void* stats, int n_seq, SeqMap map, int C, int heads,
                               const unsigned* amax_qkv, unsigned* amax_out, hipStream_t st, void* op, int T, int Tp, float* op_unscale);
 int d3dp_train_embed_bwd(const float* dx, const float* x2d, const float* x3d, float* part, int T, int C, hipStream_t st);
diff --git a/d3dp_amd/csrc/train_attn.hip b/d3dp_amd/csrc/train_attn.hip
--- a/d3dp_amd/csrc/train_attn.hip
+++ b/d3dp_amd/csrc/train_attn.hip
@@ -619,6 +619,8 @@
                      : ta_launch<NKT_, HD_, false, 3, true>(0, qkv, nullptr, nullptr, out, nullptr, stats, n_seq, map, C, heads, amax_qkv, nullptr, amax_out, st, po);
 #elif defined(D3DP_TA_PAD_TU)
 #define TA_CASE(NKT_, HD_) return ta_launch<NKT_, HD_, true>(which, qkv, o, dout, out, dqkv, stats, n_seq, map, C, heads, amax_qkv, amax_do, amax_out, st);
+#elif defined(D3DP_TA_PRE_TU)
+#define TA_CASE(NKT_, HD_)
 #elif defined(D3DP_TA_1P_TU)
 #define TA_CASE(NKT_, HD_) return ta_launch<NKT_, HD_, false, 1>(which, qkv, o, dout, out, dqkv, stats, n_seq, map, C, heads, amax_qkv, amax_do, amax_out, st, po);
 #else
@@ -632,14 +634,20 @@
   if (n <= 512) { TA_CASE(32, HD_) } \
   TA_CASE(64, HD_)
 
-#if !defined(D3DP_TA_PAD_TU) && !defined(D3DP_TA_1P_TU) && !defined(D3DP_TA_HI_TU)
+#if !defined(D3DP_TA_PAD_TU) && !defined(D3DP_TA_1P_TU) && !defined(D3DP_TA_HI_TU) && !defined(D3DP_TA_PRE_TU)
 int ta_dispatch(int which, const float* qkv, const float* o, const float* dout, float* out, float* dqkv, void* stats, int n_seq,
                 SeqMap map, int C, int heads, const unsigned* amax_qkv, const unsigned* amax_do, unsigned* amax_out,
-                hipStream_t st, int passes, TAOperand po = {nullptr, 0, 0, nullptr}, int op_hi = 0) {
+                hipStream_t st, int passes, TAOperand po = {nullptr, 0, 0, nullptr}, int op_hi = 0, const void* qkv_pk = nullptr) {
   const int n = map.n_tok;
   if (passes != 1 && passes != 3) return -1;
   if (heads < 1 || C % heads != 0 || C % 4 != 0 || n < 1 || n > 1024 || !amax_qkv || !stats) return -2;
   if (po.op && (po.Tp < po.T || !po.unscale || C % 32 != 0)) return -1;
+  if (qkv_pk) {
+    const int hdp = C / heads;
+    if (passes != 3 || op_hi || (hdp != 64 && hdp != 32 && hdp != 16)) return -1;
+    if (which == 0 || n > 32)
+      return d3dp_train_attn_x2_pre(which, qkv_pk, o, dout, out, dqkv, stats, n_seq, map, C, heads, amax_qkv, amax_do, amax_out, st, po.op, po.T, po.Tp, po.unscale);
+  }
   if (po.op && op_hi) {
     if (which != 0) return -1;
     return d3dp_train_attn_x2_fwd_hi(passes, qkv, out, stats, n_seq, map, C, heads, amax_qkv, amax_out, st, po.op, po.T, po.Tp, po.unscale);
@@ -690,6 +698,7 @@
   }
   return -2;
 }
+#elif defined(D3DP_TA_PRE_TU)
 #elif defined(D3DP_TA_1P_TU)
 int d3dp_train_attn_x2_1p(int which, const float* qkv, const float* o, const float* dout, float* out, float* dqkv, void* stats,
                           int n_seq, SeqMap map, int C, int heads, const unsigned* amax_qkv, const unsigned* amax_do,
@@ -707,16 +716,17 @@
 
 int d3dp_train_attn_x2_fwd(const float* qkv, float* out, void* stats, int n_seq, SeqMap map, int C, int heads,
                            const unsigned* amax_qkv, unsigned* amax_out, hipStream_t st, void* op, int T, int Tp,
-                           float* op_unscale, int passes, int op_hi) {
+                           float* op_unscale, int passes, int op_hi, const void* qkv_pk) {
   if (!qkv || !out) return -1;
   return ta_dispatch(0, qkv, nullptr, nullptr, out, nullptr, stats, n_seq, map, C, heads, amax_qkv, nullptr, amax_out, st, passes,
-                     TAOperand{(f16*)op, T, Tp, op_unscale}, op_hi);
+                     TAOperand{(f16*)op, T, Tp, op_unscale}, op_hi, qkv_pk);
 }
 int d3dp_train_attn_x2_bwd(const float* qkv, const float* o, const float* dout, float* dqkv, void* stats, int n_seq, SeqMap map,
                            int C, int heads, const unsigned* amax_qkv, const unsigned* amax_do, unsigned* amax_out,
-                           hipStream_t st, int part, int passes) {
+                           hipStream_t st, int part, int passes, const void* qkv_pk) {
   if (!qkv || !o || !dout || !dqkv || !amax_do || part < 0 || part > 2) return -1;
-  return ta_dispatch(1 + part, qkv, o, dout, nullptr, dqkv, stats, n_seq, map, C, heads, amax_qkv, amax_do, amax_out, st, passes);
+  return ta_dispatch(1 + part, qkv, o, dout, nullptr, dqkv, stats, n_seq, map, C, heads, amax_qkv, amax_do, amax_out, st, passes,
+                     TAOperand{nullptr, 0, 0, nullptr}, 0, qkv_pk);
 }
 #endif
 #undef TA_LENGTHS
diff --git a/d3dp_amd/csrc/train_attn_pre.hip b/d3dp_amd/csrc/train_attn_pre.hip
--- /dev/null
+++ b/d3dp_amd/csrc/train_attn_pre.hip
@@ -0,0 +1,494 @@
+#define D3DP_TA_PRE_TU 1
+#include <type_traits>
+
+#include "train_attn.hip"
+
+namespace {
+
+template <int NKT, int HD> struct TAPre {
+  static constexpr int NW = NKT <= 2 ? 2 : (NKT <= 4 ? 4 : 8);
+  static constexpr int NKCH = NKT <= 2 ? 2 : 4;
+  static constexpr int ROWB = 2 * HD, SL = HD / 8;
+  static constexpr int NK = 2 * NKCH * 16;
+  static constexpr int PLANE = NK * ROWB;
+  static constexpr int CHB = NKCH * 16 * ROWB;
+  static constexpr int PPP = CHB / 1024;
+  static constexpr int NP = 4 * PPP;
+  static constexpr int LDS = 4 * PLANE + 64;
+  static_assert(CHB % 1024 == 0 && NP % NW == 0, "whole 1 KiB pieces, the same number for every wave");
+};
+
+template <int NKT, int HD>
+__device__ __forceinline__ void ta_pre_issue(const f16* pkh, size_t rs, int C, int key0, int n, int buf, char* kimg, char* vimg, int wave, int lane) {
+  typedef TAPre<NKT, HD> G;
+  asm volatile("" : "+v"(lane));
+#pragma unroll
+  for (int i = 0; i < G::NP / G::NW; ++i) {
+    const int p = wave + i * G::NW, pl = p / G::PPP, q = p - pl * G::PPP;
+    const int boff = q * 1024 + lane * 16, row = boff / G::ROWB, slot = (boff % G::ROWB) >> 4;
+    const int key = min(key0 + row, n - 1);
+    const f16* src = pkh + (size_t)key * rs + (size_t)(2 + pl) * C + ((slot ^ ta_sw<HD>(row)) << 3);
+    char* dst = ((pl & 2) ? vimg : kimg) + (pl & 1) * G::PLANE + buf * G::CHB + q * 1024;
+    __builtin_amdgcn_global_load_lds(GPTR(src), LPTR(dst), 16, 0, 0);
+  }
+}
+template <int HD>
+__device__ __forceinline__ void ta_pre_row_op(const f16* row, int C, int fg, typename TAHead<HD>::frag (&h)[TAHead<HD>::NQ],
+                                              typename TAHead<HD>::frag (&l)[TAHead<HD>::NQ]) {
+  typedef typename TAHead<HD>::frag frag;
+  constexpr int W = HD == 16 ? 4 : 8;
+#pragma unroll
+  for (int half = 0; half < TAHead<HD>::NQ; ++half) {
+    h[half] = *reinterpret_cast<const frag*>(row + half * 32 + fg * W);
+    l[half] = *reinterpret_cast<const frag*>(row + C + half * 32 + fg * W);
+  }
+}
+
+template <int NKT, int HD>
+__global__ __launch_bounds__((TAPre<NKT, HD>::NW * 64), 4) void tattn_fwd_pre_kernel(const f16* __restrict__ pk, float* __restrict__ out,
+                                                                               TAStat* __restrict__ stats, SeqMap map, int C, int heads,
+                                                                               int groups, int n_work, const unsigned* __restrict__ bound_qkv,
+                                                                               unsigned* __restrict__ amax_out, f16* __restrict__ op, int T,
+                                                                               int Tp, float* __restrict__ op_unscale) {
+  typedef TAPre<NKT, HD> G;
+  constexpr int NW = G::NW, NKCH = G::NKCH, PLANE = G::PLANE, ND = HD / 16;
+  extern __shared__ __attribute__((aligned(16))) char smem[];
+  char* kimg = smem;
+  char* vimg = smem + 2 * PLANE;
+  float* part = reinterpret_cast<float*>(smem + 4 * PLANE);
+  const int n = map.n_tok;
+  const int tid = threadIdx.x, lane = tid & 63, wave = __builtin_amdgcn_readfirstlane(tid >> 6);
+  const size_t ld = (size_t)6 * C, rs = (size_t)map.tok_stride * ld;
+  const float sq = __uint_as_float(train_presplit_scale(bound_qkv[0]).scale_bits);
+  constexpr float scale = TAHead<HD>::SCALE;
+  float am = 0.f;
+  if (op) {
+    if (blockIdx.x == 0 && tid == 0) { op_unscale[0] = 1.0f / sq; if (amax_out) amax_out[0] = bound_qkv[0]; }
+    const size_t n8 = (size_t)(Tp - T) * C / 4;
+    uint4* z = reinterpret_cast<uint4*>(op + (size_t)T * 2 * C);
+    for (size_t i = (size_t)blockIdx.x * (NW * 64) + tid; i < n8; i += (size_t)gridDim.x * (NW * 64)) z[i] = make_uint4(0u, 0u, 0u, 0u);
+  }
+  for (int unit = blockIdx.x; unit < n_work; unit += gridDim.x) {
+    const int prob = unit / groups, group = unit % groups;
+    const int seq = prob / heads, head = prob % heads;
+    const int base = ta_seq_base(map, seq);
+    const f16* pkh = pk + (size_t)base * ld + (size_t)head * HD;
+    const int qt = group * NW + wave;
+    const bool active = qt * 16 < n;
+    const int fi = lane & 15, fg = lane >> 4;
+    const int q = qt * 16 + fi;
+    const size_t tok = (size_t)(base + min(q, n - 1) * map.tok_stride);
+    if (unit != (int)blockIdx.x) __syncthreads();
+    ta_pre_issue<NKT, HD>(pkh, rs, C, 0, n, 0, kimg, vimg, wave, lane);
+    typename TAHead<HD>::frag qh[TAHead<HD>::NQ], ql[TAHead<HD>::NQ];
+    if (active) ta_pre_row_op<HD>(pk + tok * ld + head * HD, C, fg, qh, ql);
+    const TAFragT<HD> fk = ta_frag<HD>(kimg, lane), fv = ta_frag<HD>(vimg, lane);
+    const float cexp = scale * kLog2e / (sq * sq);
+    float mrun = -INFINITY, lrun = 0.f;
+    f32x4 o[ND];
+#pragma unroll
+    for (int dn = 0; dn < ND; ++dn) o[dn] = (f32x4){0.f, 0.f, 0.f, 0.f};
+    auto chunk = [&](const int kc, auto bufc) {
+      constexpr int buf = decltype(bufc)::value;
+      asm volatile("s_waitcnt vmcnt(0)" ::: "memory");
+      __syncthreads();
+      if (kc + NKCH < NKT && 16 * (kc + NKCH) < n) ta_pre_issue<NKT, HD>(pkh, rs, C, 16 * (kc + NKCH), n, buf ^ 1, kimg, vimg, wave, lane);
+      if (active) {
+        constexpr int t0 = buf * NKCH;
+#pragma unroll
+        for (int t = 0; t < NKCH; t += 2) {
+          if (16 * (kc + t) >= n) break;
+          f32x4 a, b;
+          ta_rows_pair<PLANE, HD, 3>(fk, t0 + t, qh, ql, a, b);
+          float s[8];
+#pragma unroll
+          for (int r = 0; r < 4; ++r) { s[r] = a[r] * cexp; s[4 + r] = b[r] * cexp; }
+          if (16 * (kc + t + 2) > n) {
+#pragma unroll
+            for (int r = 0; r < 4; ++r) {
+              if (16 * (kc + t) + 4 * fg + r >= n) s[r] = -INFINITY;
+              if (16 * (kc + t + 1) + 4 * fg + r >= n) s[4 + r] = -INFINITY;
+            }
+          }
+          float mx = s[0];
+#pragma unroll
+          for (int e = 1; e < 8; ++e) mx = fmaxf(mx, s[e]);
+          mx = fmaxf(mx, __shfl_xor(mx, 16, 64));
+          mx = fmaxf(mx, __shfl_xor(mx, 32, 64));
+          const float mnew = fmaxf(mrun, mx);
+          const float alpha = __builtin_amdgcn_exp2f(mrun - mnew);
+          mrun = mnew;
+          float psum = 0.f;
+          f16x8 ph, pl;
+#pragma unroll
+          for (int e = 0; e < 8; ++e) {
+            const float y = __builtin_amdgcn_exp2f(s[e] - mnew + 10.0f);
+            psum += y;
+            const f16 hh = (f16)y;
+            ph[e] = hh;
+            pl[e] = (f16)fmaf(y, 1.0f, -(float)hh);
+          }
+          psum += __shfl_xor(psum, 16, 64);
+          psum += __shfl_xor(psum, 32, 64);
+          lrun = fmaf(lrun, alpha, psum);
+#pragma unroll
+          for (int dn = 0; dn < ND; ++dn) o[dn] *= alpha;
+          ta_tr_chunk<PLANE, HD, 3>(fv, (t0 + t) >> 1, ph, pl, o);
+        }
+      }
+    };
+#pragma unroll 1
+    for (int kc = 0; kc < NKT && 16 * kc < n; kc += 2 * NKCH) {
+      chunk(kc, std::integral_constant<int, 0>{});
+      if (kc + NKCH < NKT && 16 * (kc + NKCH) < n) chunk(kc + NKCH, std::integral_constant<int, 1>{});
+    }
+    if (active) {
+      const float inv = 1.0f / (sq * lrun);
+      if (q < n) {
+        float* dst = out + tok * C + head * HD + fg * 4;
+#pragma unroll
+        for (int dn = 0; dn < ND; ++dn) {
+          const float4 r4 = make_float4(o[dn][0] * inv, o[dn][1] * inv, o[dn][2] * inv, o[dn][3] * inv);
+          am = fmaxf(am, fmaxf(fmaxf(fabsf(r4.x), fabsf(r4.y)), fmaxf(fabsf(r4.z), fabsf(r4.w))));
+          *reinterpret_cast<float4*>(dst + dn * 16) = r4;
+          if (op) {
+            const float y[4] = {ta_opaque(r4.x * sq), ta_opaque(r4.y * sq), ta_opaque(r4.z * sq), ta_opaque(r4.w * sq)};
+            f16x4 hi, lo;
+#pragma unroll
+            for (int e = 0; e < 4; ++e) { const f16 hh = (f16)y[e]; hi[e] = hh; lo[e] = (f16)(y[e] - (float)hh); }
+            f16* d = op + tok * 2 * C + h2i_col(head * HD + dn * 16 + fg * 4);
+            *reinterpret_cast<f16x4*>(d) = hi;
+            *reinterpret_cast<f16x4*>(d + kH2iLo) = lo;
+          }
+        }
+        if (fg == 0) stats[(size_t)prob * n + q].L = mrun + __builtin_amdgcn_logf(lrun) - 10.0f;
+      }
+    }
+  }
+  if (amax_out && !op) ta_block_amax<NW>(am, amax_out, part);
+}
+
+template <int NKT, int HD>
+__global__ __launch_bounds__((TAPre<NKT, HD>::NW * 64), 4) void tattn_bwd_q_pre_kernel(const f16* __restrict__ pk, const float* __restrict__ o,
+                                                                                 const float* __restrict__ dout, float* __restrict__ dqkv,
+                                                                                 TAStat* __restrict__ stats, SeqMap map, int C, int heads,
+                                                                                 int groups, int n_work, const unsigned* __restrict__ bound_qkv,
+                                                                                 const unsigned* __restrict__ amax_do, unsigned* __restrict__ amax_out) {
+  typedef TAPre<NKT, HD> G;
+  constexpr int NW = G::NW, NKCH = G::NKCH, PLANE = G::PLANE, ND = HD / 16;
+  extern __shared__ __attribute__((aligned(16))) char smem[];
+  char* kimg = smem;
+  char* vimg = smem + 2 * PLANE;
+  float* part = reinterpret_cast<float*>(smem + 4 * PLANE);
+  const int n = map.n_tok;
+  const int tid = threadIdx.x, lane = tid & 63, wave = __builtin_amdgcn_readfirstlane(tid >> 6);
+  const size_t ld = (size_t)6 * C, rs = (size_t)map.tok_stride * ld;
+  const size_t ldq = (size_t)3 * C;
+  const float sq = __uint_as_float(train_presplit_scale(bound_qkv[0]).scale_bits), sg = ta_scale(amax_do);
+  constexpr float scale = TAHead<HD>::SCALE;
+  float am = 0.f;
+  for (int unit = blockIdx.x; unit < n_work; unit += gridDim.x) {
+    const int prob = unit / groups, group = unit % groups;
+    const int seq = prob / heads, head = prob % heads;
+    const int base = ta_seq_base(map, seq);
+    const f16* pkh = pk + (size_t)base * ld + (size_t)head * HD;
+    const int qt = group * NW + wave;
+    const bool active = qt * 16 < n;
+    const int fi = lane & 15, fg = lane >> 4;
+    const int q = qt * 16 + fi;
+    const size_t tok = (size_t)(base + min(q, n - 1) * map.tok_stride);
+    if (unit != (int)blockIdx.x) __syncthreads();
+    ta_pre_issue<NKT, HD>(pkh, rs, C, 0, n, 0, kimg, vimg, wave, lane);
+    typename TAHead<HD>::frag qh[TAHead<HD>::NQ], ql[TAHead<HD>::NQ], gh[TAHead<HD>::NQ], gl[TAHead<HD>::NQ];
+    float D = 0.f, L = 0.f;
+    if (active) {
+      ta_pre_row_op<HD>(pk + tok * ld + head * HD, C, fg, qh, ql);
+      ta_load_row_op<HD, false, 3>(dout + tok * C + head * HD, fg, sg, gh, gl, HD);
+      {
+        const float* gs = dout + tok * C + head * HD;
+        const float* os = o + tok * C + head * HD;
+        constexpr int W = HD == 16 ? 4 : 8;
+#pragma unroll
+        for (int half = 0; half < TAHead<HD>::NQ; ++half)
+#pragma unroll
+          for (int c4 = 0; c4 < W / 4; ++c4) {
+            const float4 g = *reinterpret_cast<const float4*>(gs + half * 32 + fg * W + c4 * 4);
+            const float4 ov = *reinterpret_cast<const float4*>(os + half * 32 + fg * W + c4 * 4);
+            D = fmaf(g.x, ov.x, D); D = fmaf(g.y, ov.y, D); D = fmaf(g.z, ov.z, D); D = fmaf(g.w, ov.w, D);
+          }
+        D += __shfl_xor(D, 16, 64);
+        D += __shfl_xor(D, 32, 64);
+      }
+      L = stats[(size_t)prob * n + min(q, n - 1)].L;
+    }
+    const TAFragT<HD> fk = ta_frag<HD>(kimg, lane), fv = ta_frag<HD>(vimg, lane);
+    const float cexp = scale * kLog2e / (sq * sq);
+    const float cdp = 1.0f / (sq * sg);
+    int eb = 20;
+    f32x4 dq[ND];
+#pragma unroll
+    for (int dn = 0; dn < ND; ++dn) dq[dn] = (f32x4){0.f, 0.f, 0.f, 0.f};
+    auto chunk = [&](const int kc, auto bufc) {
+      constexpr int buf = decltype(bufc)::value;
+      asm volatile("s_waitcnt vmcnt(0)" ::: "memory");
+      __syncthreads();
+      if (kc + NKCH < NKT && 16 * (kc + NKCH) < n) ta_pre_issue<NKT, HD>(pkh, rs, C, 16 * (kc + NKCH), n, buf ^ 1, kimg, vimg, wave, lane);
+      if (active) {
+        constexpr int t0 = buf * NKCH;
+#pragma unroll
+        for (int t = 0; t < NKCH; t += 2) {
+          if (16 * (kc + t) >= n) break;
+          f32x4 a, b, c, d;
+          ta_rows_pair<PLANE, HD, 3>(fk, t0 + t, qh, ql, a, b);
+          ta_rows_pair<PLANE, HD, 3>(fv, t0 + t, gh, gl, c, d);
+          float ds[8];
+#pragma unroll
+          for (int r = 0; r < 4; ++r) {
+            const float pa = __builtin_amdgcn_exp2f(fmaf(a[r], cexp, -L)), pb = __builtin_amdgcn_exp2f(fmaf(b[r], cexp, -L));
+            ds[r] = pa * (fmaf(c[r], cdp, -D)) * scale;
+            ds[4 + r] = pb * (fmaf(d[r], cdp, -D)) * scale;
+          }
+          if (16 * (kc + t + 2) > n) {
+#pragma unroll
+            for (int r = 0; r < 4; ++r) {
+              if (16 * (kc + t) + 4 * fg + r >= n) ds[r] = 0.f;
+              if (16 * (kc + t + 1) + 4 * fg + r >= n) ds[4 + r] = 0.f;
+            }
+          }
+          const int en = max(eb, ta_exp_of_max(ds));
+          if (en != eb) {
+#pragma unroll
+            for (int dn = 0; dn < ND; ++dn)
+#pragma unroll
+              for (int i = 0; i < 4; ++i) dq[dn][i] = ldexpf(dq[dn][i], eb - en);
+            eb = en;
+          }
+          f16x8 sh, sl;
+          ta_split_run<3>(ds, eb, sh, sl);
+          ta_tr_chunk<PLANE, HD, 3>(fk, (t0 + t) >> 1, sh, sl, dq);
+        }
+      }
+    };
+#pragma unroll 1
+    for (int kc = 0; kc < NKT && 16 * kc < n; kc += 2 * NKCH) {
+      chunk(kc, std::integral_constant<int, 0>{});
+      if (kc + NKCH < NKT && 16 * (kc + NKCH) < n) chunk(kc + NKCH, std::integral_constant<int, 1>{});
+    }
+    if (active) {
+      if (q < n) {
+        const float un = 1.0f / sq;
+        float* dst = dqkv + tok * ldq + head * HD + fg * 4;
+#pragma unroll
+        for (int dn = 0; dn < ND; ++dn) {
+          const float4 r4 = make_float4(ldexpf(dq[dn][0], eb - 140) * un, ldexpf(dq[dn][1], eb - 140) * un,
+                                        ldexpf(dq[dn][2], eb - 140) * un, ldexpf(dq[dn][3], eb - 140) * un);
+          am = fmaxf(am, fmaxf(fmaxf(fabsf(r4.x), fabsf(r4.y)), fmaxf(fabsf(r4.z), fabsf(r4.w))));
+          *reinterpret_cast<float4*>(dst + dn * 16) = r4;
+        }
+        if (fg == 0) stats[(size_t)prob * n + q].D = D;
+      }
+    }
+  }
+  if (amax_out) ta_block_amax<NW>(am, amax_out, part);
+}
+
+template <int NK, int NT, int HD>
+__device__ __forceinline__ void ta_stage_pk(const f16* __restrict__ src, size_t rs, int C, int n, char* img, int tid) {
+  constexpr int ROWB = 2 * HD, SL = HD / 8, LS = HD == 64 ? 3 : HD == 32 ? 2 : 1;
+  constexpr int PLANE = NK * ROWB, ITEMS = NK * SL;
+  for (int i0 = 0; i0 < ITEMS; i0 += 4 * NT) {
+    uint4 a[4], b[4];
+#pragma unroll
+    for (int u = 0; u < 4; ++u) {
+      const int idx = i0 + u * NT + tid, row = idx >> LS, slot = idx & (SL - 1);
+      a[u] = make_uint4(0u, 0u, 0u, 0u); b[u] = a[u];
+      if (idx < ITEMS && row < n) {
+        const f16* p = src + (size_t)row * rs + slot * 8;
+        a[u] = *reinterpret_cast<const uint4*>(p);
+        b[u] = *reinterpret_cast<const uint4*>(p + C);
+      }
+    }
+#pragma unroll
+    for (int u = 0; u < 4; ++u) {
+      const int idx = i0 + u * NT + tid, row = idx >> LS, slot = idx & (SL - 1);
+      if (idx < ITEMS) {
+        const int off = row * ROWB + ((slot ^ ta_sw<HD>(row)) << 4);
+        *reinterpret_cast<uint4*>(img + off) = a[u];
+        *reinterpret_cast<uint4*>(img + PLANE + off) = b[u];
+      }
+    }
+  }
+}
+
+template <int NKT, int NW, int NKC, int WPE, int HD>
+__global__ __launch_bounds__(NW * 64, WPE) void tattn_bwd_kv_pre_kernel(const f16* __restrict__ pk, const float* __restrict__ dout,
+                                                              float* __restrict__ dqkv, const TAStat* __restrict__ stats,
+                                                              SeqMap map, int C, int heads, int groups, int n_work,
+                                                              const unsigned* __restrict__ amax_qkv,
+                                                              const unsigned* __restrict__ amax_do, unsigned* __restrict__ amax_out) {
+  constexpr int NK = 16 * NKC, PLANE = NK * 2 * HD, ND = HD / 16, NPL = 2, PASSES = 3;
+  constexpr bool PAD = false;
+  extern __shared__ __attribute__((aligned(16))) char smem[];
+  char* qimg = smem;
+  char* gimg = smem + NPL * PLANE;
+  float2* st = reinterpret_cast<float2*>(smem + 2 * NPL * PLANE);
+  float* part = reinterpret_cast<float*>(smem + 2 * NPL * PLANE + NK * 8);
+  const int n = map.n_tok;
+  const int tid = threadIdx.x, lane = tid & 63, wave = tid >> 6;
+  const size_t ld = (size_t)3 * C, ldp = (size_t)6 * C, rsp = (size_t)map.tok_stride * ldp;
+  const float sq = __uint_as_float(train_presplit_scale(amax_qkv[0]).scale_bits), sg = ta_scale(amax_do);
+  constexpr int hd = HD;
+  constexpr float scale = TAHead<HD>::SCALE;
+  float am = 0.f;
+  for (int unit = blockIdx.x; unit < n_work; unit += gridDim.x) {
+  const int prob = unit / groups, group = unit % groups;
+  const int seq = prob / heads, head = prob % heads;
+  const int base = ta_seq_base(map, seq);
+  const int kt = group * NW + wave;
+  const bool active = kt * 16 < n;
+  const int fi = lane & 15, fg = lane >> 4;
+  const int key = kt * 16 + fi;
+  const bool live = key < n;
+  const size_t tok = (size_t)(base + min(key, n - 1) * map.tok_stride);
+  typename TAHead<HD>::frag kh[TAHead<HD>::NQ], kl[TAHead<HD>::NQ], vh[TAHead<HD>::NQ], vl[TAHead<HD>::NQ];
+  if (active) {
+    ta_pre_row_op<HD>(pk + tok * ldp + 2 * C + head * hd, C, fg, kh, kl);
+    ta_pre_row_op<HD>(pk + tok * ldp + 4 * C + head * hd, C, fg, vh, vl);
+  }
+  const TAFragT<HD> fq = ta_frag<HD>(qimg, lane), fgr = ta_frag<HD>(gimg, lane);
+  const float cexp = scale * kLog2e / (sq * sq);
+  const float cdp = 1.0f / (sq * sg);
+  int eb = 20;
+  f32x4 dk[ND], dv[ND];
+#pragma unroll
+  for (int dn = 0; dn < ND; ++dn) { dk[dn] = (f32x4){0.f, 0.f, 0.f, 0.f}; dv[dn] = dk[dn]; }
+#pragma unroll 1
+  for (int qc = 0; qc < NKT && 16 * qc < n; qc += NKC) {
+  if (unit != (int)blockIdx.x || qc != 0) __syncthreads();
+  ta_stage_pk<NK, NW * 64, HD>(pk + (size_t)base * ldp + (size_t)head * hd + (size_t)qc * 16 * rsp, rsp, C, n - 16 * qc, qimg, tid);
+  ta_stage<NK, NW * 64, HD, PAD, PASSES>(dout + (size_t)base * C + (size_t)head * hd + (size_t)qc * 16 * map.tok_stride * C, (size_t)map.tok_stride * C,
+                        n - 16 * qc, sg, gimg, tid, hd);
+  for (int i = tid; i < NK; i += NW * 64) {
+    float2 v = make_float2(1.0e30f, 0.f);
+    if (16 * qc + i < n) { const TAStat s = stats[(size_t)prob * n + 16 * qc + i]; v = make_float2(s.L, s.D); }
+    st[i] = v;
+  }
+  __syncthreads();
+  if (active) {
+#pragma unroll
+    for (int t = 0; t < NKC; t += 2) {
+      if (16 * (qc + t) >= n) break;
+      f32x4 a, b, c, d;
+      ta_rows_pair<PLANE, HD, PASSES>(fq, t, kh, kl, a, b);
+      ta_rows_pair<PLANE, HD, PASSES>(fgr, t, vh, vl, c, d);
+      float ds[8];
+      f16x8 ph, pl;
+#pragma unroll
+      for (int r = 0; r < 4; ++r) {
+        const float2 sa = st[16 * t + 4 * fg + r], sb = st[16 * (t + 1) + 4 * fg + r];
+        float pa = __builtin_amdgcn_exp2f(fmaf(a[r], cexp, -sa.x)), pb = __builtin_amdgcn_exp2f(fmaf(b[r], cexp, -sb.x));
+        if (!live) { pa = 0.f; pb = 0.f; }
+        ds[r] = pa * (fmaf(c[r], cdp, -sa.y)) * scale;
+        ds[4 + r] = pb * (fmaf(d[r], cdp, -sb.y)) * scale;
+        if constexpr (PASSES == 1) {
+          ph[r] = (f16)(pa * 1024.0f); ph[4 + r] = (f16)(pb * 1024.0f);
+        } else {
+        const float ya = ta_opaque(pa * 1024.0f), yb = ta_opaque(pb * 1024.0f);
+        const f16 ha = (f16)ya, hb = (f16)yb;
+        ph[r] = ha; pl[r] = (f16)(ya - (float)ha);
+        ph[4 + r] = hb; pl[4 + r] = (f16)(yb - (float)hb);
+        }
+      }
+      ta_tr_chunk<PLANE, HD, PASSES>(fgr, t >> 1, ph, PASSES == 1 ? ph : pl, dv);
+      const int en = max(eb, ta_exp_of_max(ds));
+      if (en != eb) {
+#pragma unroll
+        for (int dn = 0; dn < ND; ++dn)
+#pragma unroll
+          for (int i = 0; i < 4; ++i) dk[dn][i] = ldexpf(dk[dn][i], eb - en);
+        eb = en;
+      }
+      f16x8 sh, sl;
+      ta_split_run<PASSES>(ds, eb, sh, sl);
+      ta_tr_chunk<PLANE, HD, PASSES>(fq, t >> 1, sh, sl, dk);
+    }
+  }
+  }
+  if (active) {
+    if (live) {
+      const float uk = 1.0f / sq, uv = 1.0f / (sg * 1024.0f);
+      float* dst = dqkv + tok * ld + C + head * hd + fg * 4;
+#pragma unroll
+      for (int dn = 0; dn < ND; ++dn) {
+        if constexpr (PAD) { if (dn * 16 + fg * 4 >= hd) continue; }
+        const float4 k4 = make_float4(ldexpf(dk[dn][0], eb - 140) * uk, ldexpf(dk[dn][1], eb - 140) * uk,
+                                      ldexpf(dk[dn][2], eb - 140) * uk, ldexpf(dk[dn][3], eb - 140) * uk);
+        const float4 v4 = make_float4(dv[dn][0] * uv, dv[dn][1] * uv, dv[dn][2] * uv, dv[dn][3] * uv);
+        am = fmaxf(am, fmaxf(fmaxf(fabsf(k4.x), fabsf(k4.y)), fmaxf(fabsf(k4.z), fabsf(k4.w))));
+        am = fmaxf(am, fmaxf(fmaxf(fabsf(v4.x), fabsf(v4.y)), fmaxf(fabsf(v4.z), fabsf(v4.w))));
+        *reinterpret_cast<float4*>(dst + dn * 16) = k4;
+        *reinterpret_cast<float4*>(dst + C + dn * 16) = v4;
+      }
+    }
+  }
+  }
+  if (amax_out) ta_block_amax<NW>(am, amax_out, part);
+}
+
+template <int NKT, int HD>
+int ta_launch_pre(int which, const f16* pk, const float* o, const float* dout, float* out, float* dqkv, void* stats, int n_seq, SeqMap map,
+                  int C, int heads, const unsigned* bound_qkv, const unsigned* amax_do, unsigned* amax_out, hipStream_t st, TAOperand po) {
+  typedef TAPre<NKT, HD> G;
+  constexpr int NKC_KV = (NKT > 16 || (HD < 64 && NKT > 8)) ? 8 : NKT, WPE_KV = HD < 64 ? 4 : 2;
+  const size_t lds_kv = (size_t)2 * 2 * NKC_KV * 16 * (2 * HD) + NKC_KV * 16 * 8 + 64;
+  static PerDeviceOnce once;
+  if (once.get([&](int) {
+        return d3dp_lds_opt_in(reinterpret_cast<const void*>(tattn_fwd_pre_kernel<NKT, HD>), 160 * 1024) < 0 ? -3
+               : d3dp_lds_opt_in(reinterpret_cast<const void*>(tattn_bwd_q_pre_kernel<NKT, HD>), 160 * 1024) < 0 ? -3
+               : d3dp_lds_opt_in(reinterpret_cast<const void*>(tattn_bwd_kv_pre_kernel<NKT, G::NW, NKC_KV, WPE_KV, HD>), 160 * 1024);
+      }) < 0) return -3;
+  const int tiles = (map.n_tok + 15) / 16, groups = (tiles + G::NW - 1) / G::NW;
+  const int n_work = n_seq * heads * groups;
+  const dim3 grid(n_work < 2048 ? n_work : 2048), blk(G::NW * 64);
+  TAStat* s = reinterpret_cast<TAStat*>(stats);
+  if (which == 0)
+    hipLaunchKernelGGL((tattn_fwd_pre_kernel<NKT, HD>), grid, blk, G::LDS, st, pk, out, s, map, C, heads, groups, n_work, bound_qkv, amax_out, po.op,
+                       po.T, po.Tp, po.unscale);
+  else {
+    if (which != 3)
+      hipLaunchKernelGGL((tattn_bwd_q_pre_kernel<NKT, HD>), grid, blk, G::LDS, st, pk, o, dout, dqkv, s, map, C, heads, groups, n_work, bound_qkv,
+                         amax_do, amax_out);
+    if (which != 2)
+      hipLaunchKernelGGL((tattn_bwd_kv_pre_kernel<NKT, G::NW, NKC_KV, WPE_KV, HD>), grid, blk, lds_kv, st, pk, dout, dqkv, (const TAStat*)s, map, C, heads,
+                         groups, n_work, bound_qkv, amax_do, amax_out);
+  }
+  return 0;
+}
+
+}
+
+int d3dp_train_attn_x2_pre(int which, const void* pk, const float* o, const float* dout, float* out, float* dqkv, void* stats,
+                           int n_seq, SeqMap map, int C, int heads, const unsigned* bound_qkv, const unsigned* amax_do,
+                           unsigned* amax_out, hipStream_t st, void* op, int T, int Tp, float* op_unscale) {
+  const int n = map.n_tok, hd = heads > 0 ? C / heads : 0;
+  if (which < 0 || which > 3 || (which != 0 && n <= 32)) return -1;
+  if (heads < 1 || hd * heads != C || n < 1 || n > 1024 || !pk || !bound_qkv || !stats || n_seq < 1) return -2;
+  if (which == 0 ? !out : (!o || !dout || !dqkv || !amax_do)) return -1;
+  if (op && (Tp < T || !op_unscale || C % 32 != 0)) return -1;
+  const TAOperand po{(f16*)op, T, Tp, op_unscale};
+  const f16* p = (const f16*)pk;
+#define TA_PRE_CASE(NKT_, HD_) return ta_launch_pre<NKT_, HD_>(which, p, o, dout, out, dqkv, stats, n_seq, map, C, heads, bound_qkv, amax_do, amax_out, st, po);
+#define TA_PRE_LENGTHS(HD_)              \
+  if (n <= 32) { TA_PRE_CASE(2, HD_) }   \
+  if (n <= 64) { TA_PRE_CASE(4, HD_) }   \
+  if (n <= 128) { TA_PRE_CASE(8, HD_) }  \
+  if (n <= 256) { TA_PRE_CASE(16, HD_) } \
+  if (n <= 512) { TA_PRE_CASE(32, HD_) } \
+  TA_PRE_CASE(64, HD_)
+  if (hd == 64) { TA_PRE_LENGTHS(64) }
+  if (hd == 32) { TA_PRE_LENGTHS(32) }
+  if (hd == 16) { TA_PRE_LENGTHS(16) }
+#undef TA_PRE_LENGTHS
+#undef TA_PRE_CASE
+  return -2;
+}
diff --git a/d3dp_amd/csrc/train_plan.h b/d3dp_amd/csrc/train_plan.h
--- a/d3dp_amd/csrc/train_plan.h
+++ b/d3dp_amd/csrc/train_plan.h
@@ -15,11 +15,27 @@
 inline size_t d3dp_train_attn_x2_stats_bytes(int n_seq, int n_tok, int heads) { return (size_t)n_seq * heads * n_tok * D3DP_TRAIN_ATTN_X2_STAT_BYTES; }
 
 constexpr int kTrainSlots = 8192, kTrainBwdSlot0 = 4096, kTrainQkvSlot0 = 2048, kTrainPmaxSlot0 = 3072;
+constexpr int kTrainQkvBoundSlot0 = 2560;
+
+#if defined(__HIPCC__)
+#define D3DP_PLAN_HD __host__ __device__
+#else
+#define D3DP_PLAN_HD
+#endif
+struct PresplitScale { unsigned scale_bits; bool ok; };
+D3DP_PLAN_HD inline PresplitScale train_presplit_scale(unsigned bound_bits) {
+  const unsigned ex = bound_bits >> 23;
+  if (ex == 0 || ex >= 255) return {0x3f800000u, false};
+  const unsigned sx = 267u - ex;
+  if (sx > 254u) return {0x3f800000u, false};
+  return {sx << 23, true};
+}
 
 struct TrainLayout {
   size_t T, Tpad, C, Hd, unit;
   size_t temb, x_final, saved0, saved_stride;
   size_t o_xin, o_qkv, o_att, o_xmid, o_hpre, o_xout;
+  size_t o_qkv_pk;
   size_t xn, y, hid, dA, dB, dC, dqkv, dh, z, At, Xt, Wt, dtemb, stats;
   size_t op_a, op_w, op_at, part, part_rem, slots;
   size_t dy_set_floats;
@@ -52,7 +68,8 @@
   L.x_final = take(L.unit);
   L.o_xin = 0; L.o_qkv = L.unit; L.o_att = 4 * L.unit; L.o_xmid = 5 * L.unit; L.o_hpre = 6 * L.unit;
   L.o_xout = 6 * L.unit + L.T * L.Hd;
-  L.saved_stride = (7 * L.unit + L.T * L.Hd + 63) / 64 * 64;
+  L.o_qkv_pk = 7 * L.unit + L.T * L.Hd;
+  L.saved_stride = (10 * L.unit + L.T * L.Hd + 63) / 64 * 64;
   L.saved0 = take(L.saved_stride * 2 * g.depth);
   L.xn = take(L.unit); L.y = take(L.unit); L.hid = take(L.T * L.Hd);
   L.dA = take(L.unit); L.dB = take(L.unit); L.dC = take(L.unit);
@@ -166,6 +183,9 @@
   bool batched;
   bool merged;
   int mZ, mTp;
+  bool qkv_presplit;
+  bool presplit(int blk) const { return qkv_presplit && (blk & 1); }
+  bool qkv_planes_only;
   bool rows_fit;
   bool parts_fit;
 
@@ -233,5 +253,12 @@
     P.parts_fit = P.parts_fit && (size_t)p.Tp <= L.Tp_max && (size_t)p.Z * p.N * p.K <= L.part_floats;
   }
   P.qkv_src0 = P.ln_fused ? TrainOperand::LN_INPUT : P.lin[kQkv].src;
+  {
+    const int hd = g.channels / g.heads;
+    P.qkv_presplit = c.train_qkv_presplit && P.path.attn_x2_t && (hd == 64 || hd == 32 || hd == 16) && hd * g.heads == g.channels &&
+                     P.attn_passes == 3 && P.passes == 3 && !P.rows_hi && P.batched && g.depth <= D3DP_QKV_BOUND_MAX &&
+                     P.lin[kQkv].fwd_tail.form != TrainTailForm::SPLIT_REM && g.channels <= 2048;
+    P.qkv_planes_only = P.qkv_presplit && g.frames > 32;
+  }
   return P;
 }
```

After: 51.73. No clear change (-0.0%).
